# TencentARC/SEED-Story

Measured on AMD Instinct MI355X. Metric: story-steps/sec (text + 1024x1024 image), higher is better.
Workload: dtype bf16

## Files before the change

include/seedstory_hip.h:

```cpp
#ifndef SEEDSTORY_HIP_H_
#define SEEDSTORY_HIP_H_

#include <stddef.h>
#include <stdint.h>

#ifdef __cplusplus
extern "C" {
#endif

#define SS_ABI_VERSION 1

enum { SS_F32 = 0, SS_BF16 = 1, SS_F16 = 2 };
enum { SS_OK = 0, SS_EINVAL = -1, SS_EHIP = -2, SS_ENOMEM = -3, SS_ESTATE = -4 };

enum {
    SS_EPI_NONE = 0,
    SS_EPI_BIAS = 1,
    SS_EPI_GELU = 2,
    SS_EPI_RESIDUAL = 4,
    SS_EPI_SILU_MUL = 8,
    SS_EPI_GEGLU_PAIR = 16
};

const char* ss_last_error(void);
// ... 137 lines not shown
    const void *wqkv, *wo, *wgu, *wdown, *ln1, *ln2;
} ss_llama_layer_weights;

typedef struct ss_llama_weights {
    const void* embed;
    const void* lm_head;
    const void* final_norm;
    const void* rope_cos;
    const void* rope_sin;
    const ss_llama_layer_weights* layers;
} ss_llama_weights;

size_t ss_llama_workspace_bytes(const ss_llama_config* cfg, int64_t max_prefill_rows);
int ss_llama_create(const ss_llama_config* cfg, const ss_llama_weights* w, void* workspace,
                    size_t workspace_bytes, int64_t max_prefill_rows, const int32_t* host_img_ids,
                    ss_llama** out);
void ss_llama_destroy(ss_llama* h);

int ss_llama_select(ss_llama* h, int32_t seq);
int ss_llama_set_stop_id(ss_llama* h, int32_t token_id);

int ss_llama_set_attn_capture(ss_llama* h, void* maps, int64_t n_rows, int64_t ld, int64_t row0, int32_t head,
                              int32_t row_calls);

void* ss_llama_buffer(ss_llama* h, int which);

int ss_llama_set_lengths(ss_llama* h, int64_t kv_len, int64_t pos, void* stream);
int ss_llama_get_lengths(ss_llama* h, int64_t* kv_len, int64_t* pos);
int ss_llama_kv_gather(ss_llama* h, const int32_t* keep_idx_dev, int64_t n_keep, void* stream);

int ss_llama_prefill(ss_llama* h, const void* embeds, int64_t M, const int32_t* pos_ids, void* hidden_out,
                     void* stream);
int ss_llama_prefill_batch(ss_llama* h, const void* embeds, const int64_t* host_rows, void* hidden_out, void* stream);

int ss_llama_generate(ss_llama* h, int64_t n_steps, int32_t last_prompt_id, const int32_t* host_forced,
                      int64_t n_forced, int64_t* host_n_generated, void* stream);

int ss_llama_generate_batch(ss_llama* h, int64_t n_steps, const int32_t* last_prompt_ids,
                            const int32_t* host_forced, int64_t forced_ld, const int64_t* n_forced,
                            const int32_t* active, int64_t* host_n_generated, void* stream);

int ss_llama_profile_decode(ss_llama* h, int64_t n_tokens, float out_ms[8], double out_bytes[4],
                            void* stream);

typedef struct ss_resampler_weights {
    const void* q_in;
    const void* pos_kv;
    const void* kv_proj;
    const void *ln_kv_w, *ln_kv_b;
    const void *in_w, *in_b;
    const void *out_w, *out_b;
    int32_t nq, embed, n_heads, kv_dim, l_kv;
    float ln_eps;
} ss_resampler_weights;
size_t ss_resampler_workspace_bytes(const ss_resampler_weights* w, int64_t batch, int dtype);
int ss_resampler_forward(const ss_resampler_weights* w, const void* x, void* y, int64_t batch, void* workspace,
                         size_t workspace_bytes, int dtype, void* stream);

typedef struct ss_vit_layer_weights {
    const void *ln1_w, *ln1_b, *ln2_w, *ln2_b;
    const void *in_w, *in_b;
    const void *out_w, *out_b;
    const void *fc_w, *fc_b, *proj_w, *proj_b;
} ss_vit_layer_weights;
typedef struct ss_vit_weights {
    const void* conv_w;
    const void* pos;
    const void *ln_pre_w, *ln_pre_b;
    const ss_vit_layer_weights* layers;
    int32_t width, n_layers, n_heads, mlp_width, patch, image, kpad;
    float ln_eps;
} ss_vit_weights;
size_t ss_vit_workspace_bytes(const ss_vit_weights* w, int64_t batch, int dtype);
int ss_vit_forward(const ss_vit_weights* w, const void* img, void* out, int64_t batch, void* workspace,
                   size_t workspace_bytes, int dtype, void* stream);

int ss_vit_blocks(const ss_vit_weights* w, void* x, int64_t batch, int64_t tokens, int64_t layer0, int64_t n_layers,
                  void* workspace, size_t workspace_bytes, int dtype, void* stream);


int ss_conv3x3(const void* x, const void* w, void* y, int64_t batch, int64_t H, int64_t W, int64_t Cin,
               int64_t Cout, int64_t stride, int64_t upsample2x, const void* bias, const void* rowvec,
               int64_t rowvec_stride, const void* residual, int dtype, void* stream);

size_t ss_groupnorm_workspace_bytes(int64_t batch, int64_t hw, int64_t channels, int64_t groups, int dtype);
int ss_groupnorm(const void* x, const void* gamma, const void* beta, void* y, void* stats_ws, int64_t batch,
                 int64_t hw, int64_t channels, int64_t groups, float eps, int fuse_silu, int dtype, void* stream);

size_t ss_loss_workspace_bytes(int64_t n);
int ss_cross_entropy_rows(const void* logits, int64_t ld, const int64_t* labels, int64_t rows, int64_t vocab,
                          int64_t ignore_index, float* row_loss, float* row_valid, int dtype, void* stream);
int ss_cosine_rows(const void* rec, const void* target, int64_t rows, int64_t dim, float* row_val, int dtype, void* stream);
int ss_masked_mean(const float* vals, const float* mask, int64_t n, void* workspace, float* out2, void* stream);
int ss_mse(const void* a, const void* b, int64_t n, void* workspace, float* out2, int dtype, void* stream);

int ss_geglu(const void* in, void* out, int64_t rows, int64_t d, int dtype, void* stream);
int ss_unary(const void* x, void* y, int64_t n, int op, int dtype, void* stream);
int ss_softmax_rows(void* scores, int64_t rows, int64_t cols, float scale, int dtype, void* stream);
int ss_transpose(const void* in, void* out, int64_t rows, int64_t cols, int dtype, void* stream);
int ss_concat_channels(const void* a, const void* b, void* out, int64_t rows, int64_t c1, int64_t c2, int dtype,
                       void* stream);
int ss_layout_nchw_nhwc(const void* in, void* out, int64_t batch, int64_t channels, int64_t hw, int64_t cpad,
                        int to_nhwc, int dtype, void* stream);
int ss_euler_scale_dup(const void* x, void* xin, int64_t n, float sigma, int dtype, void* stream);
int ss_euler_cfg_step(void* x, const void* eps, int64_t n, float guidance, float sigma, float sigma_next,
                      int dtype, void* stream);
#define SS_FILTER_BILINEAR 0
#define SS_FILTER_BICUBIC 1
int ss_resample_ksize(int64_t in_size, int64_t out_size, int filter);
int ss_resample_coeffs(int64_t in_size, int64_t out_size, int filter, int32_t* coef, int32_t* bounds);
int ss_image_preprocess(const void* src_u8_hwc, int64_t H, int64_t W, void* dst_chw, void* dst_u8_hwc, int64_t OH, int64_t OW,
                        int64_t crop_top, int64_t crop_left, int64_t CH, int64_t CW, const int32_t* coef_h,
                        const int32_t* bounds_h, int ksize_h, const int32_t* coef_v, const int32_t* bounds_v, int ksize_v,
                        int64_t first_row, int64_t n_rows, void* tmp_u8, const float mean[3], const float std[3], int dtype,
                        void* stream);
int ss_image_to_u8(const void* in, void* out_u8, int64_t pixels, int64_t cpad, int dtype, void* stream);

int ss_debug_tr_probe(const void* src, void* dst, const void* lane_off, void* stream);

#ifdef __cplusplus
}
#endif
#endif
```

seed-story_amd/csrc/ss_diffusion.hip:

```cpp
#include "ss_common.h"

namespace ss {

__device__ __forceinline__ float silu_d(float g) { return g / (1.0f + expf(-g)); }
__device__ __forceinline__ float gelu_d(float v) { return 0.5f * v * (1.0f + erff(v * 0.70710678118654752440f)); }

__device__ __forceinline__ float silu_fast(float g) {
    return g * __builtin_amdgcn_rcpf(1.0f + __builtin_amdgcn_exp2f(-1.4426950408889634f * g));
}

template <typename T>
__global__ __launch_bounds__(256) void groupnorm_stats_kernel(const T* __restrict__ x, double* __restrict__ part,
                                                              int HW, int C, int G, int rows_per_block) {
    constexpr int V = Tr<T>::kVec;
    extern __shared__ __attribute__((aligned(16))) char smem_raw[];
    float* red = reinterpret_cast<float*>(smem_raw);
    float* chs = red + 256 * 2 * V;
    const int b = blockIdx.y;
    const int cg = C / G, ppr = C / V;
    const int r0 = blockIdx.x * rows_per_block;
    const int r1 = min(HW, r0 + rows_per_block);
    const T* xb = x + ((int64_t)b * HW) * C;
    for (int pc = 0; pc < ppr; pc += 256) {
        const int cw = min(256, ppr - pc);
// ... 9 lines not shown
            for (; r + 3 * rip < r1; r += 4 * rip) {
                uint4 u[4];
#pragma unroll
                for (int q = 0; q < 4; ++q) u[q] = ld16(xp + (int64_t)(r + q * rip) * C);
#pragma unroll
                for (int q = 0; q < 4; ++q) {
                    float f[V];
                    unpack<T>(u[q], f);
#pragma unroll
                    for (int j = 0; j < V; ++j) { s1[j] += f[j]; s2[j] = fmaf(f[j], f[j], s2[j]); }
                }
            }
            for (; r + rip < r1; r += 2 * rip) {
                float f[V], h[V];
                const uint4 u0 = ld16(xp + (int64_t)r * C), u1 = ld16(xp + (int64_t)(r + rip) * C);
                unpack<T>(u0, f);
                unpack<T>(u1, h);
#pragma unroll
                for (int j = 0; j < V; ++j) {
                    s1[j] += f[j]; s2[j] = fmaf(f[j], f[j], s2[j]);
                    s1[j] += h[j]; s2[j] = fmaf(h[j], h[j], s2[j]);
                }
            }
            if (r < r1) {
                float f[V];
                unpack<T>(ld16(xp + (int64_t)r * C), f);
#pragma unroll
                for (int j = 0; j < V; ++j) { s1[j] += f[j]; s2[j] = fmaf(f[j], f[j], s2[j]); }
            }
#pragma unroll
            for (int j = 0; j < V; ++j) { red[threadIdx.x * 2 * V + 2 * j] = s1[j]; red[threadIdx.x * 2 * V + 2 * j + 1] = s2[j]; }
        }
        __syncthreads();
        if (active && ry == 0) {
            for (int k = 1; k < rip; ++k) {
                const float* o = red + (k * cw + (int)threadIdx.x) * 2 * V;
#pragma unroll
                for (int j = 0; j < V; ++j) { s1[j] += o[2 * j]; s2[j] += o[2 * j + 1]; }
            }
#pragma unroll
            for (int j = 0; j < V; ++j) { chs[(p * V + j) * 2] = s1[j]; chs[(p * V + j) * 2 + 1] = s2[j]; }
        }
        __syncthreads();
    }
    double* out = part + (((int64_t)b * gridDim.x + blockIdx.x) * G) * 2;
    for (int g = threadIdx.x; g < G; g += 256) {
        double a1 = 0.0, a2 = 0.0;
        for (int c = g * cg; c < (g + 1) * cg; ++c) { a1 += (double)chs[2 * c]; a2 += (double)chs[2 * c + 1]; }
        out[2 * g] = a1;
        out[2 * g + 1] = a2;
    }
}

__global__ __launch_bounds__(256) void groupnorm_finalize_kernel(const double* __restrict__ part, double* __restrict__ stats,
                                                                 int nblk, int G) {
    __shared__ double sl[256 * 2];
    const int b = blockIdx.x;
    const int gw = G < 256 ? G : 256;
    const int ns = 256 / gw;
    for (int g0 = 0; g0 < G; g0 += gw) {
        const int g = g0 + (int)threadIdx.x % gw, sidx = (int)threadIdx.x / gw;
        double a1 = 0.0, a2 = 0.0;
        if (sidx < ns && g < G) {
            const int per = (nblk + ns - 1) / ns;
            const int k0 = sidx * per, k1 = min(nblk, k0 + per);
            const double2* pp = reinterpret_cast<const double2*>(part) + (int64_t)b * nblk * G + g;
            for (int kb = k0; kb < k1; kb += 8) {
                double2 t[8];
#pragma unroll
                for (int k = 0; k < 8; ++k) t[k] = (kb + k < k1) ? pp[(int64_t)(kb + k) * G] : make_double2(0.0, 0.0);
#pragma unroll
                for (int k = 0; k < 8; ++k) { a1 += t[k].x; a2 += t[k].y; }
            }
        }
        sl[threadIdx.x * 2] = a1;
        sl[threadIdx.x * 2 + 1] = a2;
        __syncthreads();
        if (sidx == 0 && g < G) {
            for (int k = 1; k < ns; ++k) { a1 += sl[(k * gw + (int)threadIdx.x) * 2]; a2 += sl[(k * gw + (int)threadIdx.x) * 2 + 1]; }
            stats[((int64_t)b * G + g) * 2] = a1;
            stats[((int64_t)b * G + g) * 2 + 1] = a2;
        }
        __syncthreads();
    }
}

template <typename T>
__global__ __launch_bounds__(256) void groupnorm_apply_kernel(const T* __restrict__ x, const double* __restrict__ stats,
                                                              const T* __restrict__ gamma, const T* __restrict__ beta,
                                                              T* __restrict__ y, int HW, int C, int G, float eps,
                                                              int silu, int rows_per_block) {
    constexpr int V = Tr<T>::kVec;
    const int b = blockIdx.y;
    const int cg = C / G, ppr = C / V;
    const int r0 = blockIdx.x * rows_per_block;
    const int r1 = min(HW, r0 + rows_per_block);
    const float inv_n = 1.0f / ((float)HW * (float)cg);
    const T* xb = x + ((int64_t)b * HW) * C;
    T* yb = y + ((int64_t)b * HW) * C;
    for (int pc = 0; pc < ppr; pc += 256) {
        const int cw = min(256, ppr - pc);
        const int rip = 256 / cw;
        const int ry = threadIdx.x / cw, p = pc + threadIdx.x % cw;
        if (ry >= rip) continue;
        float sc[V], sh[V], ga[V], be[V];
        unpack<T>(ld16(gamma + p * V), ga);
        unpack<T>(ld16(beta + p * V), be);
#pragma unroll
        for (int j = 0; j < V; ++j) {
            const int g = (p * V + j) / cg;
            const double md = stats[((int64_t)b * G + g) * 2] * (double)inv_n;
            const float mean = (float)md;
            const float var = (float)fmax(stats[((int64_t)b * G + g) * 2 + 1] * (double)inv_n - md * md, 0.0);
            const float rstd = 1.0f / sqrtf(var + eps);
            sc[j] = rstd * ga[j];
            sh[j] = be[j] - mean * sc[j];
        }
        const T* xp = xb + (int64_t)p * V;
        T* yp = yb + (int64_t)p * V;
        auto one = [&](const uint4& u, int r) {
            float f[V];
            unpack<T>(u, f);
#pragma unroll
            for (int j = 0; j < V; ++j) {
                float v = fmaf(f[j], sc[j], sh[j]);
                if (silu) v = silu_fast(Tr<T>::rnd(v));
                f[j] = v;
            }
            st16(yp + (int64_t)r * C, pack<T>(f));
        };
        int r = r0 + ry;
        for (; r + 3 * rip < r1; r += 4 * rip) {
            uint4 u[4];
#pragma unroll
            for (int q = 0; q < 4; ++q) u[q] = ld16(xp + (int64_t)(r + q * rip) * C);
#pragma unroll
            for (int q = 0; q < 4; ++q) one(u[q], r + q * rip);
        }
        for (; r + rip < r1; r += 2 * rip) {
            const uint4 u0 = ld16(xp + (int64_t)r * C), u1 = ld16(xp + (int64_t)(r + rip) * C);
            one(u0, r);
            one(u1, r + rip);
        }
        if (r < r1) one(ld16(xp + (int64_t)r * C), r);
    }
}

static int groupnorm_rows_per_block(int64_t B, int64_t HW, int64_t C, size_t elem) {
    int rows_per_block = (int)((128 * 1024) / (C * elem));
    if (rows_per_block < 16) rows_per_block = 16;
    while (rows_per_block > 16 && B * cdiv(HW, rows_per_block) < 2048) rows_per_block /= 2;
    if (rows_per_block > HW) rows_per_block = (int)HW;
    return rows_per_block;
}

size_t groupnorm_workspace_bytes(int64_t B, int64_t HW, int64_t C, int64_t G, int dtype) {
    if (B * HW == 0) return 0;
    const int rpb = groupnorm_rows_per_block(B, HW, C, dtype_size(dtype));
    return (size_t)B * G * 2 * sizeof(double) * (1 + (size_t)cdiv(HW, rpb));
}

template <typename T>
int groupnorm_launch(const void* x, const void* gamma, const void* beta, void* y, double* ws, int64_t B, int64_t HW,
                     int64_t C, int64_t G, float eps, int silu, hipStream_t s) {
    constexpr int V = Tr<T>::kVec;
    SS_REQUIRE(C % G == 0 && C % V == 0, "groupnorm: C=%lld G=%lld unsupported", (long long)C, (long long)G);
    if (B * HW == 0) return SS_OK;
    const int rows_per_block = groupnorm_rows_per_block(B, HW, C, sizeof(T));
    dim3 grid((unsigned)cdiv(HW, rows_per_block), (unsigned)B);
    double* stats = ws;
    double* part = ws + (size_t)B * G * 2;
    const size_t lds = (size_t)256 * 2 * V * sizeof(float) + (size_t)C * 2 * sizeof(float);
    SS_REQUIRE(lds <= 64 * 1024, "groupnorm: C=%lld too wide", (long long)C);
    hipLaunchKernelGGL(groupnorm_stats_kernel<T>, grid, dim3(256), lds, s, (const T*)x, part, (int)HW, (int)C, (int)G,
                       rows_per_block);
    SS_LAUNCH_CHECK("groupnorm_stats");
    hipLaunchKernelGGL(groupnorm_finalize_kernel, dim3((unsigned)B), dim3(256), 0, s, (const double*)part, stats, (int)grid.x, (int)G);
    SS_LAUNCH_CHECK("groupnorm_finalize");
    hipLaunchKernelGGL(groupnorm_apply_kernel<T>, grid, dim3(256), 0, s, (const T*)x, stats, (const T*)gamma,
                       (const T*)beta, (T*)y, (int)HW, (int)C, (int)G, eps, silu, rows_per_block);
    SS_LAUNCH_CHECK("groupnorm_apply");
    return SS_OK;
}

template <typename T>
__global__ __launch_bounds__(256) void geglu_kernel(const T* __restrict__ in, T* __restrict__ out, int64_t rows, int D) {
    constexpr int V = Tr<T>::kVec;
    const int ppr = D / V;
    const int64_t total = rows * ppr;
    for (int64_t i = blockIdx.x * (int64_t)blockDim.x + threadIdx.x; i < total; i += (int64_t)gridDim.x * blockDim.x) {
        const int64_t r = i / ppr;
        const int p = (int)(i % ppr);
        float a[V], g[V];
        unpack<T>(ld16(in + r * 2 * D + (int64_t)p * V), a);
        unpack<T>(ld16(in + r * 2 * D + D + (int64_t)p * V), g);
#pragma unroll
        for (int j = 0; j < V; ++j) a[j] = a[j] * Tr<T>::rnd(gelu_d(g[j]));
        st16(out + r * D + (int64_t)p * V, pack<T>(a));
    }
}

template <typename T>
__global__ __launch_bounds__(256) void softmax_rows_kernel(T* __restrict__ s, int cols, float scale) {
    constexpr int V = Tr<T>::kVec;
    __shared__ float red[16];
    T* row = s + (int64_t)blockIdx.x * cols;
    const int npack = cols / V;
    float mx = -1e30f;
    for (int p = threadIdx.x; p < npack; p += 256) {
        float f[V];
        unpack<T>(ld16(row + (int64_t)p * V), f);
#pragma unroll
        for (int j = 0; j < V; ++j) mx = fmaxf(mx, f[j] * scale);
    }
    mx = block_max(mx, red);
    float sum = 0.f;
    for (int p = threadIdx.x; p < npack; p += 256) {
        float f[V];
        unpack<T>(ld16(row + (int64_t)p * V), f);
#pragma unroll
        for (int j = 0; j < V; ++j) sum += expf(f[j] * scale - mx);
    }
    sum = block_sum(sum, red);
    const float inv = 1.0f / sum;
    for (int p = threadIdx.x; p < npack; p += 256) {
        float f[V];
        unpack<T>(ld16(row + (int64_t)p * V), f);
#pragma unroll
        for (int j = 0; j < V; ++j) f[j] = expf(f[j] * scale - mx) * inv;
        st16(row + (int64_t)p * V, pack<T>(f));
    }
}

template <typename T>
__global__ __launch_bounds__(256) void transpose_kernel(const T* __restrict__ in, T* __restrict__ out, int R, int Cc) {
    __shared__ T tile[32][33];
    const int c0 = blockIdx.x * 32, r0 = blockIdx.y * 32;
    const int tx = threadIdx.x & 31, ty = threadIdx.x >> 5;
    for (int j = ty; j < 32; j += 8)
        if (r0 + j < R && c0 + tx < Cc) tile[j][tx] = in[(int64_t)(r0 + j) * Cc + c0 + tx];
    __syncthreads();
    for (int j = ty; j < 32; j += 8)
        if (c0 + j < Cc && r0 + tx < R) out[(int64_t)(c0 + j) * R + r0 + tx] = tile[tx][j];
}

template <typename T>
__global__ __launch_bounds__(256) void concat_channels_kernel(const T* __restrict__ a, const T* __restrict__ b,
                                                              T* __restrict__ out, int64_t rows, int C1, int C2) {
    constexpr int V = Tr<T>::kVec;
    const int ppr = (C1 + C2) / V, p1 = C1 / V;
    const int64_t total = rows * ppr;
    for (int64_t i = blockIdx.x * (int64_t)blockDim.x + threadIdx.x; i < total; i += (int64_t)gridDim.x * blockDim.x) {
        const int64_t r = i / ppr;
        const int p = (int)(i % ppr);
        const uint4 v = p < p1 ? ld16(a + r * C1 + (int64_t)p * V) : ld16(b + r * C2 + (int64_t)(p - p1) * V);
        st16(out + r * (C1 + C2) + (int64_t)p * V, v);
    }
}

template <typename T>
__global__ void nchw_to_nhwc_kernel(const T* __restrict__ in, T* __restrict__ out, int64_t B, int C, int HW, int Cpad) {
    const int64_t total = B * HW * Cpad;
    for (int64_t i = blockIdx.x * (int64_t)blockDim.x + threadIdx.x; i < total; i += (int64_t)gridDim.x * blockDim.x) {
        const int c = (int)(i % Cpad);
        const int64_t r = i / Cpad;
        const int64_t b = r / HW, px = r % HW;
        T v;
// ... 64 lines not shown
    SS_LAUNCH_CHECK("geglu");
    return SS_OK;
}
template <typename T>
int unary_launch(const void* x, void* y, int64_t n, int op, hipStream_t s) {
    if (n == 0) return SS_OK;
    hipLaunchKernelGGL(unary_kernel<T>, dim3(egrid(n)), dim3(256), 0, s, (const T*)x, (T*)y, n, op);
    SS_LAUNCH_CHECK("unary");
    return SS_OK;
}
template <typename T>
int softmax_rows_launch(void* sc, int64_t rows, int64_t cols, float scale, hipStream_t s) {
    SS_REQUIRE(cols % Tr<T>::kVec == 0, "softmax_rows: cols %% %d != 0", Tr<T>::kVec);
    if (rows == 0) return SS_OK;
    hipLaunchKernelGGL(softmax_rows_kernel<T>, dim3((unsigned)rows), dim3(256), 0, s, (T*)sc, (int)cols, scale);
    SS_LAUNCH_CHECK("softmax_rows");
    return SS_OK;
}
template <typename T>
int transpose_launch(const void* in, void* out, int64_t R, int64_t Cc, hipStream_t s) {
    if (R * Cc == 0) return SS_OK;
    hipLaunchKernelGGL(transpose_kernel<T>, dim3((unsigned)cdiv(Cc, 32), (unsigned)cdiv(R, 32)), dim3(256), 0, s,
                       (const T*)in, (T*)out, (int)R, (int)Cc);
    SS_LAUNCH_CHECK("transpose");
    return SS_OK;
}
template <typename T>
int concat_channels_launch(const void* a, const void* b, void* out, int64_t rows, int64_t C1, int64_t C2, hipStream_t s) {
    SS_REQUIRE(C1 % Tr<T>::kVec == 0 && C2 % Tr<T>::kVec == 0, "concat_channels: channels %% %d != 0", Tr<T>::kVec);
    if (rows == 0) return SS_OK;
    hipLaunchKernelGGL(concat_channels_kernel<T>, dim3(egrid(rows * (C1 + C2) / Tr<T>::kVec)), dim3(256), 0, s,
                       (const T*)a, (const T*)b, (T*)out, rows, (int)C1, (int)C2);
    SS_LAUNCH_CHECK("concat_channels");
    return SS_OK;
}
template <typename T>
int layout_launch(const void* in, void* out, int64_t B, int64_t C, int64_t HW, int64_t Cpad, int to_nhwc, hipStream_t s) {
    if (B * HW == 0) return SS_OK;
    if (to_nhwc)
        hipLaunchKernelGGL(nchw_to_nhwc_kernel<T>, dim3(egrid(B * HW * Cpad)), dim3(256), 0, s, (const T*)in, (T*)out, B,
                           (int)C, (int)HW, (int)Cpad);
    else
        hipLaunchKernelGGL(nhwc_to_nchw_kernel<T>, dim3(egrid(B * C * HW)), dim3(256), 0, s, (const T*)in, (T*)out, B,
                           (int)C, (int)HW, (int)Cpad);
    SS_LAUNCH_CHECK("layout");
    return SS_OK;
}
template <typename T>
int euler_scale_dup_launch(const void* x, void* xin, int64_t n, float sigma, hipStream_t s) {
    hipLaunchKernelGGL(euler_scale_dup_kernel<T>, dim3(egrid(n)), dim3(256), 0, s, (const T*)x, (T*)xin, n,
                       1.0f / sqrtf(sigma * sigma + 1.0f));
    SS_LAUNCH_CHECK("euler_scale_dup");
    return SS_OK;
}
template <typename T>
int euler_cfg_step_launch(void* x, const void* eps, int64_t n, float guidance, float sigma, float sigma_next, hipStream_t s) {
    hipLaunchKernelGGL(euler_cfg_step_kernel<T>, dim3(egrid(n)), dim3(256), 0, s, (T*)x, (const T*)eps, n, guidance,
                       sigma_next - sigma);
    SS_LAUNCH_CHECK("euler_cfg_step");
    return SS_OK;
}
template <typename T>
int image_to_u8_launch(const void* in, void* out, int64_t pixels, int64_t Cpad, hipStream_t s) {
    hipLaunchKernelGGL(image_to_u8_kernel<T>, dim3(egrid(pixels * 3)), dim3(256), 0, s, (const T*)in, (uint8_t*)out, pixels,
                       (int)Cpad);
    SS_LAUNCH_CHECK("image_to_u8");
    return SS_OK;
}

}

using namespace ss;

extern "C" {

size_t ss_groupnorm_workspace_bytes(int64_t batch, int64_t hw, int64_t channels, int64_t groups, int dtype) {
    return ss::groupnorm_workspace_bytes(batch, hw, channels, groups, dtype);
}

int ss_groupnorm(const void* x, const void* gamma, const void* beta, void* y, void* stats_ws, int64_t batch, int64_t hw,
                 int64_t channels, int64_t groups, float eps, int fuse_silu, int dtype, void* stream) {
    return SS_DISPATCH(dtype, groupnorm_launch, x, gamma, beta, y, (double*)stats_ws, batch, hw, channels, groups, eps,
                       fuse_silu, (hipStream_t)stream);
}
int ss_geglu(const void* in, void* out, int64_t rows, int64_t d, int dtype, void* stream) {
    return SS_DISPATCH(dtype, geglu_launch, in, out, rows, d, (hipStream_t)stream);
}
int ss_unary(const void* x, void* y, int64_t n, int op, int dtype, void* stream) {
    return SS_DISPATCH(dtype, unary_launch, x, y, n, op, (hipStream_t)stream);
}
int ss_softmax_rows(void* scores, int64_t rows, int64_t cols, float scale, int dtype, void* stream) {
    return SS_DISPATCH(dtype, softmax_rows_launch, scores, rows, cols, scale, (hipStream_t)stream);
}
int ss_transpose(const void* in, void* out, int64_t rows, int64_t cols, int dtype, void* stream) {
    return SS_DISPATCH(dtype, transpose_launch, in, out, rows, cols, (hipStream_t)stream);
}
int ss_concat_channels(const void* a, const void* b, void* out, int64_t rows, int64_t c1, int64_t c2, int dtype,
                       void* stream) {
    return SS_DISPATCH(dtype, concat_channels_launch, a, b, out, rows, c1, c2, (hipStream_t)stream);
}
int ss_layout_nchw_nhwc(const void* in, void* out, int64_t batch, int64_t channels, int64_t hw, int64_t cpad,
                        int to_nhwc, int dtype, void* stream) {
    return SS_DISPATCH(dtype, layout_launch, in, out, batch, channels, hw, cpad, to_nhwc, (hipStream_t)stream);
}
int ss_euler_scale_dup(const void* x, void* xin, int64_t n, float sigma, int dtype, void* stream) {
    return SS_DISPATCH(dtype, euler_scale_dup_launch, x, xin, n, sigma, (hipStream_t)stream);
}
int ss_euler_cfg_step(void* x, const void* eps, int64_t n, float guidance, float sigma, float sigma_next, int dtype,
                      void* stream) {
    return SS_DISPATCH(dtype, euler_cfg_step_launch, x, eps, n, guidance, sigma, sigma_next, (hipStream_t)stream);
}
int ss_image_to_u8(const void* in, void* out_u8, int64_t pixels, int64_t cpad, int dtype, void* stream) {
    return SS_DISPATCH(dtype, image_to_u8_launch, in, out_u8, pixels, cpad, (hipStream_t)stream);
}

}

namespace ss {
typedef short v4s_t __attribute__((ext_vector_type(4)));
typedef __attribute__((address_space(3))) v4s_t lds_v4s_t;
__global__ void tr_probe_kernel(const uint16_t* src, uint16_t* dst, const int* lane_off) {
    __shared__ __attribute__((aligned(16))) uint16_t sm[4096];
    for (int i = threadIdx.x; i < 4096; i += 64) sm[i] = src[i];
    __syncthreads();
    const int off = lane_off[threadIdx.x];
    v4s_t r = __builtin_amdgcn_ds_read_tr16_b64_v4i16((lds_v4s_t*)(sm + off));
    for (int j = 0; j < 4; ++j) dst[threadIdx.x * 4 + j] = (uint16_t)r[j];
}
}
extern "C" int ss_debug_tr_probe(const void* src, void* dst, const void* lane_off, void* stream) {
    hipLaunchKernelGGL(ss::tr_probe_kernel, dim3(1), dim3(64), 0, (hipStream_t)stream, (const uint16_t*)src,
                       (uint16_t*)dst, (const int*)lane_off);
    SS_LAUNCH_CHECK("tr_probe");
    return SS_OK;
}
```

seed-story_amd/csrc/ss_gemm.hip:

```cpp
#include <stdio.h>

#include <map>
#include <mutex>

#include "ss_gemm_common.h"

namespace ss {

__device__ __attribute__((aligned(16))) unsigned int g_zero_page[64];

template <typename T, int BM, int BN, int WM, int WN, int KT, bool CONV, bool SPLIT = false>
__global__ __launch_bounds__(64 * WM * WN) void gemm_kernel(const GemmArgs g) {
    static_assert(!SPLIT || Tr<T>::kVec == 4, "SPLIT: fp32 operands");
    constexpr int V = Tr<T>::kVec;
    constexpr int NT = 64 * WM * WN;
    constexpr int PPR = 8 * KT;
    constexpr int BK = PPR * V;
    constexpr int LS = BK + V;
    constexpr int TM = BM / WM, TN = BN / WN;
    constexpr int FM = TM / 16, FN = TN / 16;
    constexpr int PA = (BM * PPR + NT - 1) / NT, PW = (BN * PPR + NT - 1) / NT;
    static_assert(TM % 16 == 0 && TN % 16 == 0, "wave tile must be MFMA-shaped");

    extern __shared__ __attribute__((aligned(16))) char smem_raw[];
// ... 587 lines not shown
                                                               float* __restrict__ part, int part_ld, int tn) {
    const int m = blockIdx.x * 4 + (threadIdx.x >> 6), lane = threadIdx.x & 63;
    if (m >= M) return;
    const T* row = C + (int64_t)m * ldc;
    double t1 = 0.0, t2 = 0.0;
    for (int n0 = 0, strip = 0; n0 < N; n0 += tn, ++strip) {
        float s1 = 0.f, s2 = 0.f;
        const int n1 = n0 + tn < N ? n0 + tn : N;
        for (int n = n0 + lane; n < n1; n += 64) {
            const float v = Tr<T>::ld(row + n);
            s1 += v;
            s2 = fmaf(v, v, s2);
        }
        s1 = wave_sum(s1);
        s2 = wave_sum(s2);
        if (part && lane == 0 && strip < part_ld) {
            part[((int64_t)m * part_ld + strip) * 2] = s1;
            part[((int64_t)m * part_ld + strip) * 2 + 1] = s2;
        }
        t1 += (double)s1;
        t2 += (double)s2;
    }
    if (stat && lane == 0) {
        stat[(int64_t)m * 2] += t1;
        stat[(int64_t)m * 2 + 1] += t2;
    }
}

template <typename T>
int gemm_launch(const void* A, const void* W, void* C, int64_t M, int64_t N, int64_t K, int64_t lda, int64_t ldw,
                int64_t ldc, const void* bias, const void* residual, int64_t ldr, int epi, hipStream_t s,
                double* rowstat_out = nullptr, float* rowpart = nullptr) {
    constexpr int V = Tr<T>::kVec;
    SS_REQUIRE(K % V == 0 && lda % V == 0 && ldw % V == 0, "gemm: K/lda/ldw must be multiples of %d (K=%lld)", V,
               (long long)K);
    SS_REQUIRE(!(epi & SS_EPI_SILU_MUL), "gemm: SILU_MUL is a GEMV epilogue (use ss_silu_mul)");
    SS_REQUIRE(!(epi & SS_EPI_GEGLU_PAIR) || (!(epi & (SS_EPI_GELU | SS_EPI_RESIDUAL)) && N % 2 == 0),
               "gemm: GEGLU_PAIR cannot be combined with GELU/RESIDUAL and needs an even N");
    SS_REQUIRE(!(epi & SS_EPI_BIAS) || bias, "gemm: bias epilogue without bias");
    SS_REQUIRE(!(epi & SS_EPI_RESIDUAL) || residual, "gemm: residual epilogue without residual");
    if (M == 0 || N == 0) return SS_OK;
    GemmArgs g = gemm_args(A, W, C, M, N, K, lda, ldw, ldc, epi, bias, residual, ldr);
    g.swz = knob(K_gemm_xcd_swizzle);
    if (knob(K_gemm_epi_generic)) g.epi |= SS_EPI_INTERNAL_GENERIC;
    if (rowstat_out || rowpart) {
        if constexpr (Tr<T>::kVec != 8) {
            set_error("ss_gemm_rowstat: 16-bit dtypes only");
            return SS_EINVAL;
        } else {
            SS_REQUIRE(K % 64 == 0 && N % 8 == 0 && M > 128, "ss_gemm_rowstat: needs K %% 64 == 0, N %% 8 == 0, M > 128 (M=%lld N=%lld K=%lld)",
                       (long long)M, (long long)N, (long long)K);
            g.rowstat_out = rowstat_out;
            int bn = 0, tn = 0;
            const int cfg = rowstat_cfg<T>(g, &bn, &tn);
            if (rowpart) {
                constexpr size_t A16 = 15;
                SS_REQUIRE(N % bn == 0 && (((size_t)C | (size_t)residual | (size_t)bias) & A16) == 0 && ((ldc | ldr) & 7) == 0,
                           "ss_gemm_rowpart: N %% %d != 0 or operands not 16-byte aligned (N=%lld)", bn, (long long)N);
                g.rowpart = rowpart;
                g.rowpart_ld = (int)(N / tn);
            }
            const bool force_fb = knob(K_gemm_rowstat_fallback) != 0;
            int rc = force_fb ? 1 : gemm_sp_dispatch<T>(cfg + 200, g, s);
            if (rc == 1 && !rowpart && !force_fb) rc = gemm_sp_dispatch<T>(265, g, s);
            if (rc == 1) {
                g.rowstat_out = nullptr;
                g.rowpart = nullptr;
                rc = gemm_dispatch_cfg<T>(lookup_cfg<T>(g), g, s);
                if (rc) return rc;
                hipLaunchKernelGGL(rowstat_fallback_kernel<T>, dim3((unsigned)((M + 3) / 4)), dim3(256), 0, s, (const T*)C, ldc, (int)M,
                                   (int)N, rowstat_out, rowpart, rowpart ? (int)(N / tn) : 0, tn > 0 ? tn : (int)N);
                SS_LAUNCH_CHECK("rowstat_fallback");
                return SS_OK;
            }
            return rc;
        }
    }
    return gemm_dispatch_cfg<T>(lookup_cfg<T>(g), g, s);
}

template <typename T>
int conv3x3_launch(const void* x, const void* w, void* y, int64_t B, int64_t H, int64_t Wd, int64_t Cin, int64_t Cout,
                   int64_t stride, int64_t up, const void* bias, const void* rowvec, int64_t rowvec_ld,
                   const void* residual, int epi, hipStream_t s) {
    constexpr int V = Tr<T>::kVec;
    SS_REQUIRE(Cin % V == 0, "conv3x3: Cin=%lld must be a multiple of %d (pad the channels)", (long long)Cin, V);
    SS_REQUIRE((stride == 1 || stride == 2) && !(up && stride != 1), "conv3x3: unsupported stride/upsample");
    GemmArgs g;
    conv_geometry(g, B, H, Wd, Cin, Cout, stride, up);
    g.A = x; g.W = w; g.C = y; g.bias = bias; g.residual = residual; g.epi = epi;
    g.rowvec = rowvec; g.rowvec_ld = rowvec_ld > 0 ? rowvec_ld : Cout;
    g.swz = knob(K_gemm_xcd_swizzle);
    if (g.M == 0) return SS_OK;
    return gemm_dispatch_cfg<T>(lookup_cfg<T>(g), g, s);
}

template <typename T>
int gemm_tune_launch(int64_t M, int64_t N, int64_t K, int epi, void* ws, size_t ws_bytes, hipStream_t s, float* us) {
    const GemmArgs g = gemm_args(nullptr, nullptr, nullptr, (M + 127) / 128 * 128, N, K, K, K, N, epi, nullptr, nullptr, N);
    return tune_shape<T>(g, ws, ws_bytes, (size_t)g.M * K, s, us);
}
template <typename T>
int conv_tune_launch(int64_t B, int64_t H, int64_t Wd, int64_t Cin, int64_t Cout, int64_t stride, int64_t up, void* ws,
                     size_t ws_bytes, hipStream_t s, float* us) {
    GemmArgs g;
    conv_geometry(g, B, H, Wd, Cin, Cout, stride, up);
    return tune_shape<T>(g, ws, ws_bytes, (size_t)B * H * Wd * Cin, s, us);
}

template <typename T>
int gemm_lnfold_launch(const void* A, const void* Wg, void* C, int64_t M, int64_t N, int64_t K, int64_t ldc, const float* rstd,
                       const float* shift, const float* colsum, const void* bias, int epi, hipStream_t s,
                       const float* ln_part = nullptr, int64_t ln_nstrip = 0, int64_t ln_width = 0, float ln_eps = 0.f) {
    if constexpr (Tr<T>::kVec != 8) {
        set_error("ss_gemm_lnfold: 16-bit dtypes only");
        return SS_EINVAL;
    } else {
        SS_REQUIRE(K % 64 == 0 && N % 16 == 0, "ss_gemm_lnfold: K %% 64 and N %% 16 must be 0 (K=%lld N=%lld)", (long long)K, (long long)N);
        SS_REQUIRE(!(epi & ~(SS_EPI_BIAS | SS_EPI_GELU | SS_EPI_GEGLU_PAIR)), "ss_gemm_lnfold: unsupported epilogue %d", epi);
        SS_REQUIRE(!(epi & SS_EPI_BIAS) || bias, "ss_gemm_lnfold: bias epilogue without bias");
        SS_REQUIRE(((rstd && shift) || (ln_part && ln_nstrip > 0 && ln_width > 0)) && colsum && (((size_t)colsum) & 15) == 0 &&
                   (((size_t)ln_part) & 7) == 0, "ss_gemm_lnfold: row statistics / column vector missing or misaligned");
        if (M == 0 || N == 0) return SS_OK;
        GemmArgs g = gemm_args(A, Wg, C, M, N, K, K, K, ldc, epi, bias);
        g.swz = knob(K_gemm_xcd_swizzle);
        g.scale_a = rstd; g.shift_a = shift; g.scale_w = colsum;
        g.ln_part = ln_part; g.ln_nstrip = (int)ln_nstrip; g.ln_inv_width = ln_width > 0 ? 1.0f / (float)ln_width : 0.f; g.ln_eps = ln_eps;
        int cfg = lookup_cfg<T>(g);
        if (cfg < 60 || cfg > 72) cfg = N % 160 == 0 ? (M >= 2048 ? 62 : 61) : (M * N >= 128 * 128 * 256 ? 65 : 70);
        if (const GemmTile t = sp_tile(cfg); t.WM * t.WN == 4 && !knob(K_lnfold_w4))
            cfg = (t.BN == 160 || N % 160 == 0) ? 62 : 66;
        const int rc = gemm_sp_dispatch<T>(cfg + 100, g, s);
        if (rc == 1) {
            set_error("ss_gemm_lnfold: no kernel for cfg %d / shape [%lld, %lld, %lld]", cfg + 100, (long long)M, (long long)N, (long long)K);
            return SS_EINVAL;
        }
        return rc;
    }
}

template <typename T>
__global__ __launch_bounds__(256) void rowstats_kernel(const T* __restrict__ x, int64_t ld, int rows, int cols, float eps,
                                                       float* __restrict__ rstd, float* __restrict__ shift) {
    constexpr int V = Tr<T>::kVec;
    constexpr int MAXP = 4;
    const int lane = threadIdx.x & 63;
    const int row = blockIdx.x * 4 + (threadIdx.x >> 6);
    if (row >= rows) return;
    const int npack = cols / V;
    const T* xr = x + (int64_t)row * ld;
    uint4 px[MAXP];
    float s1 = 0.f;
#pragma unroll
    for (int i = 0; i < MAXP; ++i) {
        const int p = lane + i * 64;
        if (p < npack) {
            px[i] = *reinterpret_cast<const uint4*>(xr + (int64_t)p * V);
            float f[V];
            unpack<T>(px[i], f);
#pragma unroll
            for (int j = 0; j < V; ++j) s1 += f[j];
        }
    }
    const float mean = wave_sum(s1) / (float)cols;
    float s2 = 0.f;
#pragma unroll
    for (int i = 0; i < MAXP; ++i) {
        const int p = lane + i * 64;
        if (p < npack) {
            float f[V];
            unpack<T>(px[i], f);
#pragma unroll
            for (int j = 0; j < V; ++j) { const float d = f[j] - mean; s2 = fmaf(d, d, s2); }
        }
    }
    const float r = 1.0f / sqrtf(wave_sum(s2) / (float)cols + eps);
    if (lane == 0) { rstd[row] = r; shift[row] = -mean * r; }
// ... 40 lines not shown
    }
    float v[4] = {a.x, a.y, a.z, a.w};
#pragma unroll
    for (int r = 0; r < 4; ++r) {
        if (bias) v[r] += Tr<T>::ld(bias + n + r);
        v[r] = Tr<T>::rnd(v[r]);
        if (res) v[r] += Tr<T>::ld(res + (int64_t)m * ldr + n + r);
        Tr<T>::st(C + (int64_t)m * ldc + n + r, v[r]);
    }
}

static void splitk_plan(int64_t M, int64_t N, int64_t K, int* cfg, int* S) {
    *cfg = 0; *S = 0;
    if (M <= 128 || M > 512 || N % 64 || K % 64 || K < 1024) return;
    const int mt = cdiv(M, 128);
    if (mt * cdiv(N, 128) >= 256) return;
    int c = 301, base = mt * cdiv(N, 64);
    int s = cdiv(2 * 256, base);
    const int kt = (int)(K / 64);
    if (s > kt / 8) s = kt / 8;
    if (s > 8) s = 8;
    if (s < 2) return;
    while (s > 2 && (s - 1) * cdiv(kt, s) >= kt) --s;
    *cfg = c; *S = s;
}

size_t gemm_splitk_workspace_bytes(int64_t M, int64_t N, int64_t K) {
    int cfg, S;
    splitk_plan(M, N, K, &cfg, &S);
    return S ? (size_t)S * M * N * sizeof(float) : 0;
}

template <typename T>
int gemm_splitk_launch(const void* A, const void* W, void* C, int64_t M, int64_t N, int64_t K, const void* bias,
                       const void* residual, void* ws, size_t ws_bytes, hipStream_t s) {
    int cfg = 0, S = 0;
    if constexpr (Tr<T>::kVec == 8) {
        if (knob(K_gemm_splitk)) splitk_plan(M, N, K, &cfg, &S);
    }
    const int force = knob(K_gemm_splitk_s);
    if (S && force >= 2 && force <= 8 && (size_t)force * M * N * sizeof(float) > ws_bytes) S = 0;
    if (!S || !ws || ws_bytes < (size_t)S * M * N * sizeof(float))
        return gemm_launch<T>(A, W, C, M, N, K, K, K, N, bias, residual, N, (bias ? SS_EPI_BIAS : 0) | (residual ? SS_EPI_RESIDUAL : 0), s);
    if constexpr (Tr<T>::kVec == 8) {
        GemmArgs g = gemm_args(A, W, ws, M, N, K, K, K, N, 0, nullptr, nullptr, N);
        g.swz = knob(K_gemm_splitk_swz);
        g.ksplit = S;
        if (force >= 2 && force <= 8 && force <= (int)(K / 64) / 2) g.ksplit = S = force;
        const int rc = gemm_sp_dispatch<T>(cfg, g, s);
        if (rc) {
            if (rc == 1) set_error("gemm_splitk: no kernel for cfg %d", cfg);
            return rc == 1 ? SS_EINVAL : rc;
        }
        const int64_t quads = M * N / 4;
        hipLaunchKernelGGL(splitk_reduce_kernel<T>, dim3((unsigned)((quads + 255) / 256)), dim3(256), 0, s, (const float*)ws, S, (int)M,
                           (int)N, (T*)C, N, (const T*)bias, (const T*)residual, N);
        SS_LAUNCH_CHECK("splitk_reduce");
    }
    return SS_OK;
}

int gemm_splitk_dev(const void* A, const void* W, void* C, int64_t M, int64_t N, int64_t K, const void* bias,
                    const void* residual, void* ws, size_t ws_bytes, int dtype, hipStream_t s) {
    return SS_DISPATCH(dtype, gemm_splitk_launch, A, W, C, M, N, K, bias, residual, ws, ws_bytes, s);
}

int gemm_dev(const void* A, const void* W, void* C, int64_t M, int64_t N, int64_t K, int64_t lda, int64_t ldw,
             int64_t ldc, const void* bias, const void* residual, int64_t ldr, int epi, int dtype, hipStream_t s) {
    return SS_DISPATCH(dtype, gemm_launch, A, W, C, M, N, K, lda, ldw, ldc, bias, residual, ldr, epi, s);
}

}

extern "C" {

int ss_conv3x3(const void* x, const void* w, void* y, int64_t batch, int64_t H, int64_t W_, int64_t Cin,
               int64_t Cout, int64_t stride, int64_t upsample2x, const void* bias, const void* rowvec,
               int64_t rowvec_stride, const void* residual, int dtype, void* stream) {
    const int epi = (bias ? SS_EPI_BIAS : 0) | (residual ? SS_EPI_RESIDUAL : 0);
    return SS_DISPATCH(dtype, ss::conv3x3_launch, x, w, y, batch, H, W_, Cin, Cout, stride, upsample2x, bias, rowvec,
                       rowvec_stride, residual, epi, (hipStream_t)stream);
}

int ss_gemm(const void* A, const void* W, void* C, int64_t M, int64_t N, int64_t K, int64_t lda,
            int64_t ldw, int64_t ldc, const void* bias, const void* residual, int64_t ldr, int epilogue,
            int dtype, void* stream) {
    return ss::gemm_dev(A, W, C, M, N, K, lda, ldw, ldc, bias, residual, ldr, epilogue, dtype, (hipStream_t)stream);
}

int ss_gemm_rowstat(const void* A, const void* W, void* C, int64_t M, int64_t N, int64_t K, int64_t lda, int64_t ldw,
                    int64_t ldc, const void* bias, const void* residual, int64_t ldr, int epilogue, double* rowstat_accum,
                    int dtype, void* stream) {
    SS_REQUIRE(rowstat_accum && (((size_t)rowstat_accum) & 15) == 0, "ss_gemm_rowstat: rowstat_accum missing or not 16-byte aligned");
    SS_REQUIRE(!(epilogue & SS_EPI_GEGLU_PAIR), "ss_gemm_rowstat: not defined for the GEGLU epilogue");
    return SS_DISPATCH(dtype, ss::gemm_launch, A, W, C, M, N, K, lda, ldw, ldc, bias, residual, ldr, epilogue,
                       (hipStream_t)stream, rowstat_accum);
}

size_t ss_gemm_splitk_workspace_bytes(int64_t M, int64_t N, int64_t K) { return ss::gemm_splitk_workspace_bytes(M, N, K); }

int ss_gemm_splitk(const void* A, const void* W, void* C, int64_t M, int64_t N, int64_t K, const void* bias, const void* residual,
                   void* workspace, size_t workspace_bytes, int dtype, void* stream) {
    SS_REQUIRE(A && W && C && M > 0 && N > 0 && K > 0, "ss_gemm_splitk: bad arguments");
    return ss::gemm_splitk_dev(A, W, C, M, N, K, bias, residual, workspace, workspace_bytes, dtype, (hipStream_t)stream);
}

int ss_rowstat_finalize(double* rowstat, int64_t M, int64_t width, float eps, float* rstd_out, float* shift_out, void* stream) {
    SS_REQUIRE(rowstat && rstd_out && shift_out && M > 0 && width > 0 && (((size_t)rowstat) & 15) == 0, "ss_rowstat_finalize: bad arguments");
    hipLaunchKernelGGL(ss::rowstat_finalize_kernel, dim3((unsigned)((M + 255) / 256)), dim3(256), 0, (hipStream_t)stream, rowstat,
                       (int)M, 1.0 / (double)width, eps, rstd_out, shift_out);
    SS_LAUNCH_CHECK("rowstat_finalize");
    return SS_OK;
}

int ss_rowstats(const void* x, int64_t ld, int64_t M, int64_t K, float eps, float* rstd_out, float* shift_out, int dtype, void* stream) {
    SS_REQUIRE(x && rstd_out && shift_out && M > 0 && K > 0 && ld >= K, "ss_rowstats: bad arguments");
    return SS_DISPATCH(dtype, ss::rowstats_launch, x, ld, M, K, eps, rstd_out, shift_out, (hipStream_t)stream);
}

int64_t ss_gemm_rowpart_strips(int64_t M, int64_t N, int64_t K, int dtype) {
    if (dtype != SS_BF16 && dtype != SS_F16) return 0;
    ss::GemmArgs g;
    g.M = (int)M; g.N = (int)N; g.K = (int)K;
    int bn = 0, tn = 0;
    if (dtype == SS_BF16) ss::rowstat_cfg<ss::bf16_t>(g, &bn, &tn); else ss::rowstat_cfg<ss::f16_t>(g, &bn, &tn);
    return (N % bn == 0) ? N / tn : 0;
}

int ss_gemm_rowpart(const void* A, const void* W, void* C, int64_t M, int64_t N, int64_t K, int64_t lda, int64_t ldw,
                    int64_t ldc, const void* bias, const void* residual, int64_t ldr, int epilogue, float* rowpart,
                    int dtype, void* stream) {
    SS_REQUIRE(rowpart && (((size_t)rowpart) & 7) == 0, "ss_gemm_rowpart: rowpart missing or not 8-byte aligned");
    SS_REQUIRE(!(epilogue & SS_EPI_GEGLU_PAIR), "ss_gemm_rowpart: not defined for the GEGLU epilogue");
    return SS_DISPATCH(dtype, ss::gemm_launch, A, W, C, M, N, K, lda, ldw, ldc, bias, residual, ldr, epilogue,
                       (hipStream_t)stream, nullptr, rowpart);
}

int ss_gemm_lnfold_part(const void* A, const void* Wg, void* C, int64_t M, int64_t N, int64_t K, int64_t ldc, const float* rowpart,
                        int64_t strips, int64_t width, float eps, const float* colsum, const void* bias, int epilogue, int dtype,
                        void* stream) {
    SS_REQUIRE(A && Wg && C && rowpart && strips > 0 && width > 0, "ss_gemm_lnfold_part: bad arguments");
    return SS_DISPATCH(dtype, ss::gemm_lnfold_launch, A, Wg, C, M, N, K, ldc, nullptr, nullptr, colsum, bias, epilogue, (hipStream_t)stream,
                       rowpart, strips, width, eps);
}

int ss_gemm_lnfold(const void* A, const void* Wg, void* C, int64_t M, int64_t N, int64_t K, int64_t ldc, const float* rstd,
                   const float* shift, const float* colsum, const void* bias, int epilogue, int dtype, void* stream) {
    SS_REQUIRE(A && Wg && C, "ss_gemm_lnfold: NULL argument");
    return SS_DISPATCH(dtype, ss::gemm_lnfold_launch, A, Wg, C, M, N, K, ldc, rstd, shift, colsum, bias, epilogue, (hipStream_t)stream);
}

size_t ss_gemm_tune_workspace_bytes(int64_t M, int64_t N, int64_t K, int dtype) {
    const size_t e = ss::dtype_size(dtype);
    const size_t Mk = (size_t)((M + 127) / 128 * 128);
    return (Mk * K + Mk * N) * e + ss::tune_rot_bytes((size_t)N * K * e) + 1024;
}

int ss_gemm_tune(int64_t M, int64_t N, int64_t K, int epilogue, int dtype, void* workspace, size_t workspace_bytes,
                 void* stream, float* best_us_host) {
    SS_REQUIRE(M > 0 && N > 0 && K > 0 && K % 8 == 0, "gemm_tune: bad shape");
    return SS_DISPATCH(dtype, ss::gemm_tune_launch, M, N, K, epilogue, workspace, workspace_bytes, (hipStream_t)stream,
                       best_us_host);
}

size_t ss_conv3x3_tune_workspace_bytes(int64_t batch, int64_t H, int64_t W_, int64_t Cin, int64_t Cout, int64_t stride,
                                       int64_t upsample2x, int dtype) {
// ... 63 lines not shown
```

seed-story_amd/csrc/ss_gemm_common.h:

```cpp
#pragma once
#include <type_traits>
#include <utility>

#include "ss_common.h"

namespace ss {

typedef __attribute__((ext_vector_type(4))) uint32_t u32x4_t;
typedef __attribute__((ext_vector_type(8))) uint32_t u32x8_t;
template <int NV> struct Frag { uint4 v[NV]; };
template <typename T> struct OutT { using type = T; };
template <> struct OutT<fp8_t> { using type = bf16_t; };
template <typename T> struct Mma;
template <> struct Mma<bf16_t> {
    static constexpr int kK = 32;
    static constexpr int kEB = 2;
    static constexpr int kNV = 1;
    static __device__ __forceinline__ f32x4_t run(const uint4& a, const uint4& b, f32x4_t c) {
        return __builtin_amdgcn_mfma_f32_16x16x32_bf16(__builtin_bit_cast(bf16x8_t, a),
                                                       __builtin_bit_cast(bf16x8_t, b), c, 0, 0, 0);
    }
    static __device__ __forceinline__ void run_inplace(const uint4& a, const uint4& b, f32x4_t& c) {
        asm volatile("v_mfma_f32_16x16x32_bf16 %0, %1, %2, %0"
                     : "+v"(c)
// ... 383 lines not shown
                    if constexpr (EM == 1) t *= sa * swv[i][r];
                    if constexpr (EM == 2) t = fmaf(t, sa, sh * swv[i][r]);
                    t += bv[i][r];
                    if (do_gelu) t = gelu_for<T>(Tr<T>::rnd(t));
                    v[r] = Tr<T>::rnd(t);
                    if (do_rowvec) v[r] = Tr<T>::rnd(v[r] + rv[i][r]);
                }
                if (geglu) {
                    const float o0 = v[0] * Tr<T>::rnd(gelu_for<T>(v[1])), o1 = v[2] * Tr<T>::rnd(gelu_for<T>(v[3]));
                    float pk[8] = {o0, o1, 0.f, 0.f, 0.f, 0.f, 0.f, 0.f};
                    *reinterpret_cast<uint32_t*>(rowp + (i * 8 + grp * 2) * 2) = pack<T>(pk).x;
                } else {
                    float pk[8] = {v[0], v[1], v[2], v[3], 0.f, 0.f, 0.f, 0.f};
                    const uint4 u = pack<T>(pk);
                    *reinterpret_cast<uint2*>(rowp + (i * 16 + grp * 4) * 2) = make_uint2(u.x, u.y);
                }
            }
        }
        auto readback = [&](auto lpr_tag) {
            constexpr int LPR = decltype(lpr_tag)::value;
            const int n_out0 = geglu ? (n_base >> 1) : n_base;
#pragma unroll
            for (int k = 0; k < (CR * LPR + 63) / 64; ++k) {
                const int idx = lane + k * 64;
                const int row = idx / LPR, c16 = idx - row * LPR;
                const int m = m_base + c * CR + row;
                if (idx < CR * LPR && m < M) {
                    uint4 u = *reinterpret_cast<const uint4*>(stg + row * RS + c16 * 16);
                    if (g.epi & SS_EPI_RESIDUAL) {
                        const uint4 rr = *reinterpret_cast<const uint4*>(res + (int64_t)m * g.ldr + n_base + c16 * 8);
                        float a[8], b[8];
                        unpack<T>(u, a);
                        unpack<T>(rr, b);
#pragma unroll
                        for (int e = 0; e < 8; ++e) a[e] += b[e];
                        u = pack<T>(a);
                    }
                    *reinterpret_cast<uint4*>(C + (int64_t)m * g.ldc + n_out0 + c16 * 8) = u;
                    if constexpr (RSTAT) {
                        if (g.rowstat_out || g.rowpart) {
                            float a[8];
                            unpack<T>(u, a);
                            float sv = 0.f, qv = 0.f;
#pragma unroll
                            for (int e = 0; e < 8; ++e) { sv += a[e]; qv = fmaf(a[e], a[e], qv); }
                            *reinterpret_cast<float2*>(stg + row * RS + c16 * 16) = make_float2(sv, qv);
                        }
                    }
                }
            }
            if constexpr (RSTAT) {
                if (g.rowstat_out || g.rowpart) {
                    const int m = m_base + c * CR + lane;
                    if (lane < CR && m < M) {
                        float sv = 0.f, qv = 0.f;
#pragma unroll
                        for (int q = 0; q < LPR; ++q) {
                            const float2 t = *reinterpret_cast<const float2*>(stg + lane * RS + q * 16);
                            sv += t.x; qv += t.y;
                        }
                        if (g.rowpart) {
                            *reinterpret_cast<float2*>(g.rowpart + ((int64_t)m * g.rowpart_ld + n_base / TN) * 2) = make_float2(sv, qv);
                        } else {
                            unsafeAtomicAdd(g.rowstat_out + 2 * (int64_t)m, (double)sv);
                            unsafeAtomicAdd(g.rowstat_out + 2 * (int64_t)m + 1, (double)qv);
                        }
                    }
                }
            }
        };
        if (geglu) readback(std::integral_constant<int, TN / 16>{});
        else readback(std::integral_constant<int, TN / 8>{});
    }
}

template <typename T> __device__ __forceinline__ uint32_t pack2(float a, float b) {
    if constexpr (std::is_same<T, bf16_t>::value) return f32x2_to_bf16x2_bits(a, b);
    else return f32_to_f16_bits(a) | (f32_to_f16_bits(b) << 16);
}
template <typename T> __device__ __forceinline__ void unpack2(uint32_t w, float& lo, float& hi) {
    if constexpr (std::is_same<T, bf16_t>::value) { lo = __uint_as_float(w << 16); hi = __uint_as_float(w & 0xffff0000u); }
    else { lo = f16_bits_to_f32(w & 0xffffu); hi = f16_bits_to_f32(w >> 16); }
}
template <typename T, int FM, int FN, int EV, bool RES, bool WHOLE>
__device__ __forceinline__ void gemm_epilogue_staged_pipe(const GemmArgs& g, f32x4_t (&acc)[FN][FM], int m_base, int n_base,
                                                          int lane, char* stg) {
    static_assert(Tr<T>::kVec == 8, "16-bit outputs only");
    static_assert(EV >= 1 && EV <= 4, "compile-time variants only");
    constexpr int TN = FN * 16, RS = TN * 2 + 16;
    constexpr bool GEGLU = EV == 4;
    constexpr int LPR = GEGLU ? TN / 16 : TN / 8;
    constexpr int NPC = 16 * LPR;
    constexpr int NP = (NPC + 63) / 64;
    const int l15 = lane & 15, grp = lane >> 4;
    const int M = g.M;
    constexpr bool has_res = RES;
    const T* bias = (const T*)g.bias;

    float bv[FN][4];
    {
        uint2 braw[FN];
        const bool hb = (g.epi & SS_EPI_BIAS) != 0;
#pragma unroll
        for (int i = 0; i < FN; ++i) braw[i] = hb ? *reinterpret_cast<const uint2*>(bias + n_base + i * 16 + grp * 4) : make_uint2(0u, 0u);
#pragma unroll
        for (int i = 0; i < FN; ++i) {
            float f[8];
            unpack<T>(make_uint4(braw[i].x, braw[i].y, 0u, 0u), f);
            bv[i][0] = f[0]; bv[i][1] = f[1]; bv[i][2] = f[2]; bv[i][3] = f[3];
        }
    }
    uint2 rvp[EV == 3 ? FN : 1];
    int rv_b = -1;
    auto load_rv = [&](int c) {
        if constexpr (EV == 3) {
            const int bidx = (m_base + c * 16) / g.rows_per_batch;
            if (bidx != rv_b) {
                rv_b = bidx;
                const T* rp = (const T*)g.rowvec + (int64_t)bidx * g.rowvec_ld + n_base + grp * 4;
#pragma unroll
                for (int i = 0; i < FN; ++i) rvp[i] = *reinterpret_cast<const uint2*>(rp + i * 16);
            }
        }
    };

    uint32_t loff[NP], goff[NP], roff[NP];
    bool pv[NP];
    int prow[NP];
#pragma unroll
    for (int k = 0; k < NP; ++k) {
        const int idx = lane + k * 64;
        const int row = idx / LPR, c16 = idx - row * LPR;
        pv[k] = (NPC % 64 == 0 || k + 1 < NP) ? true : idx < NPC;
        prow[k] = row;
        loff[k] = pv[k] ? (uint32_t)(row * RS + c16 * 16) : 0u;
        goff[k] = (uint32_t)row * (uint32_t)(g.ldc * 2) + (uint32_t)(c16 * 16);
        roff[k] = pv[k] ? (uint32_t)row * (uint32_t)(g.ldr * 2) + (uint32_t)(c16 * 16) : 0u;
    }
    const int n_out0 = GEGLU ? (n_base >> 1) : n_base;
    char* Cb = reinterpret_cast<char*>((T*)g.C + (int64_t)m_base * g.ldc + n_out0);
    const char* Rb = reinterpret_cast<const char*>((const T*)g.residual + (int64_t)m_base * g.ldr + n_base);
    const int64_t cstep = 32 * g.ldc, rstep = 32 * g.ldr;
    char* wrow = stg + l15 * RS + (GEGLU ? grp * 4 : grp * 8);

    auto stage = [&](int c) {
        load_rv(c);
#pragma unroll
        for (int i = 0; i < FN; ++i) {
            float t[4];
#pragma unroll
            for (int r = 0; r < 4; ++r) t[r] = acc[i][c][r] + bv[i][r];
            if constexpr (EV == 2) {
#pragma unroll
                for (int r = 0; r < 4; ++r) t[r] = gelu_for<T>(Tr<T>::rnd(t[r]));
            }
            if constexpr (EV == 3) {
                float rv[8];
                asm volatile("" : "+v"(rvp[i].x), "+v"(rvp[i].y));
                unpack<T>(make_uint4(rvp[i].x, rvp[i].y, 0u, 0u), rv);
#pragma unroll
                for (int r = 0; r < 4; ++r) t[r] = Tr<T>::rnd(t[r]) + rv[r];
            }
            if constexpr (GEGLU) {
                float v0, v1, v2, v3;
                unpack2<T>(pack2<T>(t[0], t[1]), v0, v1);
                unpack2<T>(pack2<T>(t[2], t[3]), v2, v3);
                const float o0 = v0 * Tr<T>::rnd(gelu_for<T>(v1)), o1 = v2 * Tr<T>::rnd(gelu_for<T>(v3));
                *reinterpret_cast<uint32_t*>(wrow + i * 16) = pack2<T>(o0, o1);
            } else {
                *reinterpret_cast<uint2*>(wrow + i * 32) = make_uint2(pack2<T>(t[0], t[1]), pack2<T>(t[2], t[3]));
            }
        }
    };
    uint4 u[NP];
    auto readback = [&]() {
#pragma unroll
        for (int k = 0; k < NP; ++k) u[k] = *reinterpret_cast<const uint4*>(stg + loff[k]);
    };

    constexpr int RD = 2;
    uint4 rr[FM][NP];
    auto row_ok = [&](int c, int k) { return pv[k] && (WHOLE || m_base + c * 16 + prow[k] < M); };
    auto load_res = [&](int c) {
        const gmem_char_t* Rc = uniform_gptr(Rb + c * rstep);
#pragma unroll
        for (int k = 0; k < NP; ++k) {
            if constexpr (WHOLE) rr[c][k] = gmem_ld16(Rc + roff[k]);
            else rr[c][k] = row_ok(c, k) ? gmem_ld16(Rc + roff[k]) : make_uint4(0u, 0u, 0u, 0u);
        }
    };
    load_rv(0);
    if (has_res) {
#pragma unroll
        for (int c = 0; c < RD && c < FM; ++c) load_res(c);
    }
    __builtin_amdgcn_sched_barrier(0);
    stage(0);
    __builtin_amdgcn_sched_barrier(0);
    readback();
#pragma unroll
    for (int c = 0; c < FM; ++c) {
        if (has_res && c + RD < FM) load_res(c + RD);
        __builtin_amdgcn_sched_barrier(0);
        if (c + 1 < FM) stage(c + 1);
        __builtin_amdgcn_sched_barrier(0);
        gmem_char_t* Cc = uniform_gptr(Cb + c * cstep);
#pragma unroll
        for (int k = 0; k < NP; ++k) {
            uint4 o = u[k];
            if (has_res) {
                float a[8], b[8];
                unpack<T>(o, a);
                unpack<T>(rr[c][k], b);
#pragma unroll
                for (int e = 0; e < 8; ++e) a[e] += b[e];
                o = pack<T>(a);
            }
            if (row_ok(c, k)) gmem_st16(Cc + goff[k], o);
        }
        __builtin_amdgcn_sched_barrier(0);
        if (c + 1 < FM) readback();
    }
}

#define SS_SP_TILES(X) \
    X(20, 128, 128, 2, 2, 1, 2,  0, 0) \
    X(21, 128,  64, 2, 2, 1, 2,  0, 0) \
    X(22,  64,  64, 2, 2, 1, 2,  0, 0) \
    X(23, 256, 128, 4, 2, 1, 2,  0, 0) \
    X(24, 256, 256, 2, 4, 2, 2,  0, 0)    \
    X(26, 128, 160, 2, 2, 1, 2,  0, 0)    \
    X(28, 128, 320, 2, 4, 1, 2,  0, 0)    \
    X(29,  64, 160, 2, 2, 1, 2,  0, 0)    \
    X(30, 256, 160, 4, 2, 1, 2,  0, 0)    \
    X(31, 256, 160, 4, 2, 1, 3,  0, 0)    \
    X(32, 256, 160, 4, 2, 1, 3,  1, 0)    \
    X(33, 256, 160, 4, 2, 1, 3,  3, 0)    \
    X(34, 256, 256, 2, 4, 2, 2,  1, 0)    \
    X(35, 256, 256, 2, 4, 2, 2,  2, 0)    \
    X(36, 256, 256, 2, 4, 2, 2,  3, 0)    \
    X(37, 128, 160, 2, 2, 1, 2,  1, 0)    \
    X(38, 256, 160, 4, 2, 1, 2,  2, 0)    \
    X(39, 128, 320, 2, 4, 1, 2,  2, 0)    \
    X(40, 256, 256, 2, 4, 2, 2,  6, 0)    \
    X(41, 128, 160, 2, 2, 1, 2,  4, 0)    \
    X(42, 256, 160, 4, 2, 1, 3,  4, 0)    \
    X(43, 256, 160, 4, 2, 1, 2,  6, 0)    \
    X(44, 128, 320, 2, 4, 1, 2,  4, 0)    \
    X(45, 256, 128, 4, 2, 1, 2,  4, 0)    \
    X(46, 128, 128, 2, 2, 1, 2,  4, 0)    \
    X(60, 256, 256, 2, 4, 2, 2, 11, 1)    \
    X(61, 128, 160, 2, 2, 1, 2,  8, 3)    \
    X(62, 256, 160, 4, 2, 1, 3, 12, 3)    \
    X(63, 128, 320, 2, 4, 1, 2,  8, 3)    \
    X(64, 256, 160, 4, 2, 1, 2, 10, 3)    \
    X(65, 128, 128, 2, 2, 1, 2,  8, 3)    \
    X(66, 256, 128, 4, 2, 1, 2,  8, 1)    \
    X(67,  64, 160, 2, 2, 1, 2,  8, 3)    \
    X(68, 128,  64, 2, 2, 1, 2,  8, 1)    \
    X(69, 256, 256, 2, 4, 2, 2,  8, 1)    \
    X(70,  64,  64, 2, 2, 1, 2,  8, 1)    \
    X(71, 256, 160, 4, 2, 1, 2,  8, 3)    \
    X(72, 128, 320, 2, 4, 1, 2, 10, 3)
#define SS_SP_SPLITK_TILES(X) \
    X(300, 128, 128, 2, 2, 1, 2, 64, 0) \
    X(301, 128,  64, 2, 2, 1, 2, 64, 0)
#define SS_SP_FP8_TILES(X) \
    X(80, 128, 128, 2, 2, 2, 2, 8, 0)     \
    X(81, 128, 160, 2, 2, 2, 2, 8, 0)     \
    X(82, 256, 160, 4, 2, 2, 2, 8, 0)     \
    X(85,  64, 160, 2, 2, 1, 2, 8, 0)     \
    X(86,  64,  64, 2, 2, 1, 2, 8, 0) \
    X(88, 128, 160, 2, 2, 2, 2, 0, 0)
#define SS_W4_FP8_TILES(X) \
    X(95, 256, 256, 2, 2, 16, 0, 2, 0)    \
    X(96, 256, 256, 2, 2, 16, 0, 0, 0)

struct GemmTile { int id, BM, BN, WM, WN, NH, NS, FLAGS, variants; };
#define SS_TILE_ROW(id, BM, BN, WM, WN, NH, NS, FLAGS, VAR) {id, BM, BN, WM, WN, NH, NS, FLAGS, VAR},
constexpr GemmTile kSpTiles[] = {SS_SP_TILES(SS_TILE_ROW)};
constexpr GemmTile kFp8Tiles[] = {SS_SP_FP8_TILES(SS_TILE_ROW) SS_W4_FP8_TILES(SS_TILE_ROW)};
template <int N> constexpr GemmTile find_tile(const GemmTile (&t)[N], int id) {
    for (int i = 0; i < N; ++i) if (t[i].id == id) return t[i];
    return GemmTile{};
}
constexpr GemmTile sp_tile(int id) { return find_tile(kSpTiles, id); }
constexpr GemmTile fp8_tile(int id) { return find_tile(kFp8Tiles, id); }

template <int N> constexpr bool tiles_well_formed(const GemmTile (&t)[N]) {
    for (int i = 0; i < N; ++i) {
        for (int j = 0; j < i; ++j) if (t[j].id == t[i].id) return false;
        if (t[i].id < 1 || t[i].id >= 100 || (t[i].variants && !(t[i].FLAGS & 8))) return false;
    }
    return true;
}
static_assert(tiles_well_formed(kSpTiles) && tiles_well_formed(kFp8Tiles),
              "tile lists: duplicate id, base id outside 1 .. 99, or a variant on a tile without the staged epilogue");

template <typename T> int gemm_sp_dispatch(int cfg, const GemmArgs& g, hipStream_t s);
template <typename T> int gemm_sp_dispatch_conv(int cfg, const GemmArgs& g, hipStream_t s);
template <typename T> int gemm_pp_dispatch(int cfg, const GemmArgs& g, hipStream_t s);
template <typename T> int gemm_pp_dispatch_conv(int cfg, const GemmArgs& g, hipStream_t s);
template <typename T> int gemm_w4_dispatch(int cfg, const GemmArgs& g, hipStream_t s);
template <typename T> int gemm_w4_dispatch_conv(int cfg, const GemmArgs& g, hipStream_t s);
int gemm_sp_dispatch_fp8(int cfg, const GemmArgs& g, hipStream_t s);
int gemm_w4_dispatch_fp8(int cfg, const GemmArgs& g, hipStream_t s);
template <typename T> static int gemm_sp_run(int cfg, const GemmArgs& g, hipStream_t s) {
    return g.conv_Cin > 0 ? gemm_sp_dispatch_conv<T>(cfg, g, s) : gemm_sp_dispatch<T>(cfg, g, s);
}
template <typename T> static int gemm_pp_run(int cfg, const GemmArgs& g, hipStream_t s) {
    return g.conv_Cin > 0 ? gemm_pp_dispatch_conv<T>(cfg, g, s) : gemm_pp_dispatch<T>(cfg, g, s);
}
template <typename T> static int gemm_w4_run(int cfg, const GemmArgs& g, hipStream_t s) {
    return g.conv_Cin > 0 ? gemm_w4_dispatch_conv<T>(cfg, g, s) : gemm_w4_dispatch<T>(cfg, g, s);
}

static inline int num_cus() {
    static int n = 0;
    if (!n) {
        int dev = 0;
        hipDeviceProp_t p;
        if (hipGetDevice(&dev) == hipSuccess && hipGetDeviceProperties(&p, dev) == hipSuccess) n = p.multiProcessorCount;
        if (n <= 0) n = 256;
    }
    return n;
}
template <auto KERN> static int launch_tiles(const char* name, const GemmArgs& g, int total, int cap, int threads, size_t lds, hipStream_t s) {
    const int grid = cap > 0 && total > cap ? cap : total;
    if (lds > 64 * 1024) SS_DYN_LDS(KERN, lds);
    hipLaunchKernelGGL(KERN, dim3((unsigned)grid, (unsigned)g.ksplit), dim3(threads), lds, s, g, total);
    SS_LAUNCH_CHECK(name);
    return SS_OK;
}

}
```

seed-story_amd/csrc/ss_gemm_pp.inc:

```

namespace ss {

template <int BN, int FLAGS>
struct PpLds {
    static constexpr int FN = BN / 64, FN0 = (FN + 1) / 2, FN1 = FN / 2, TN = FN * 16;
    static constexpr int HA = 128 * 128, HB0 = 4 * FN0 * 16 * 128, HB1 = 4 * FN1 * 16 * 128;
    static constexpr int BUF = 2 * HA + HB0 + HB1;
    static constexpr int STG_CR = 16, STG_WAVE = STG_CR * (TN * 2 + 16);
    static constexpr bool STG_IN_RING = 2 * BUF + 8 * STG_WAVE > 163840;
    static constexpr int BYTES = 2 * BUF + ((FLAGS & 8) != 0 && !STG_IN_RING ? 8 * STG_WAVE : 0);
};

static __device__ __attribute__((aligned(4096))) unsigned int g_pp_zero_page[1024];

__device__ __forceinline__ void dma16v(const char* gsrc, uint32_t lds_base) {
    asm volatile(
        "s_mov_b32 m0, %1\n\t"
        "s_nop 0\n\t"
        "global_load_lds_dwordx4 %0, off"
        :
        : "v"(gsrc), "s"(lds_base)
        : "memory");
}

template <typename T, int BN, int FLAGS, bool CONV>
__global__ __launch_bounds__(512) void gemm_pp_kernel(const GemmArgs g, const int total_tiles) {
    using Lds = PpLds<BN, FLAGS>;
    constexpr int BM = 256, FN = Lds::FN, FN0 = Lds::FN0, FN1 = Lds::FN1, TM = 128, TN = Lds::TN, FM = 8;
    static_assert(BN == 256 || BN == 320, "tile widths");
    constexpr bool EXACT = BN == 320 || CONV;
    constexpr bool PRIO = (FLAGS & 1) != 0, PERSIST = (FLAGS & 2) != 0, TWO = (FLAGS & 4) != 0, STAGED = (FLAGS & 8) != 0, RSTAT = (FLAGS & 32) != 0;
    constexpr int EM = ((FLAGS & 16) != 0) ? 2 : 0;
    constexpr int HA = Lds::HA, HB0 = Lds::HB0, HB1 = Lds::HB1, BUF = Lds::BUF;
    constexpr int OFF_A0 = 0, OFF_A1 = HA, OFF_B0 = 2 * HA, OFF_B1 = 2 * HA + HB0;
    constexpr int NP0 = FN0, NP1 = FN1;
    constexpr int FLY = NP0 + 2 + NP1;
    constexpr int STG_CR = Lds::STG_CR, STG_WAVE = Lds::STG_WAVE;
    constexpr bool STG_IN_RING = Lds::STG_IN_RING;
    static_assert(!(PERSIST && STG_IN_RING), "persistent tiles prefetch under the epilogue: the strips need their own LDS");
    static_assert(Mma<T>::kEB == 2, "16-bit operands");
    using TO = T;
    extern __shared__ __attribute__((aligned(16))) char smem_raw[];

    const int tid = threadIdx.x, lane = tid & 63;
    const int wid = __builtin_amdgcn_readfirstlane(tid >> 6);
    const int wm = wid >> 2, wn = wid & 3;
    const int l15 = lane & 15, grp = lane >> 4;
    const int M = g.M, N = g.N;
    const int MT = (M + BM - 1) / BM, NT = (N + BN - 1) / BN;
    const int ntiles = g.K / 64;
    const int tpt = CONV ? g.conv_Cin / 64 : 1;
    const uint32_t tpt_inv = CONV ? (65536u + (uint32_t)tpt - 1u) / (uint32_t)tpt : 0u;
    const int lw = CONV ? __builtin_ctz((unsigned)g.conv_W) : 0;
    const uint32_t lds0 = __builtin_amdgcn_readfirstlane((uint32_t)(size_t)(lds_void_t*)smem_raw);

    const int srow = lane >> 3;
    const int schunk = (lane & 7) ^ srow;
    auto b_col = [&](int h, int i) {
        const int RH = (h ? FN1 : FN0) * 16;
        const int r8 = (wid + 8 * i) * 8;
        return (r8 / RH) * TN + (h ? FN0 * 16 : 0) + r8 % RH + srow;
    };
    int m_blk = 0, n_blk = 0;
    uint32_t voffA[EXACT ? 1 : 2][EXACT ? 1 : 2], voffW[EXACT ? 1 : 2][EXACT ? 1 : 3];
    const char* sbaseA = nullptr;
    const char* sbaseW = nullptr;
    auto setup_tile = [&](int vid) {
        int mt_, nt_;
        xcd_tile_id(g.swz, MT, NT, vid, mt_, nt_);
        m_blk = mt_ * BM; n_blk = nt_ * BN;
        if constexpr (CONV) {
            voffA[0][0] = (uint32_t)(srow * g.conv_Cin * 2 + schunk * 16);
            voffW[0][0] = (uint32_t)((int64_t)srow * g.ldw * 2 + schunk * 16);
        } else if constexpr (EXACT) {
            voffA[0][0] = (uint32_t)((int64_t)srow * g.lda * 2 + schunk * 16);
            voffW[0][0] = (uint32_t)((int64_t)srow * g.ldw * 2 + schunk * 16);
        } else {
#pragma unroll
            for (int h = 0; h < 2; ++h) {
#pragma unroll
                for (int i = 0; i < 2; ++i) {
                    int m = m_blk + i * 128 + h * 64 + wid * 8 + srow;
                    m = m < M ? m : M - 1;
                    voffA[h][i] = (uint32_t)((int64_t)(m - m_blk) * g.lda * 2 + schunk * 16);
                }
#pragma unroll
                for (int i = 0; i < (h ? NP1 : NP0); ++i) {
                    int n = n_blk + b_col(h, i);
                    n = n < N ? n : N - 1;
                    voffW[h][i] = (uint32_t)((int64_t)(n - n_blk) * g.ldw * 2 + schunk * 16);
                }
            }
        }
        sbaseA = uniform_ptr((const char*)g.A + (CONV ? (int64_t)0 : (int64_t)m_blk * g.lda * 2));
        sbaseW = uniform_ptr((const char*)g.W + (int64_t)n_blk * g.ldw * 2);
    };
    struct Cur { const char* src; int dy, dx, c, tap; };
    auto cur_set_tap = [&](Cur& k) {
        const int t3 = (k.tap * 11) >> 5;
        k.dy = t3 - 1; k.dx = k.tap - 3 * t3 - 1;
        k.src = (const char*)g.A + ((int64_t)(k.dy * g.conv_W + k.dx) * g.conv_Cin + k.c * 64) * 2;
    };
    auto cur_make = [&](int t) {
        Cur k;
        k.tap = (int)(((uint32_t)t * tpt_inv) >> 16);
        k.c = t - k.tap * tpt;
        cur_set_tap(k);
        return k;
    };
    auto cur_next = [&](Cur& k) {
        k.c += 1; k.src += 128;
        if (k.c == tpt) { k.c = 0; k.tap += 1; cur_set_tap(k); }
    };
    auto stage_conv = [&](const Cur& k, int b, int h) {
        const uint32_t keep = m0_save();
// ... 156 lines not shown
            asm volatile("s_waitcnt lgkmcnt(0)" ::: "memory");
            pin();
            mma(1, H1);
            pin();
            bar();
            if (s2) { stage(t + 2, b, 3); wait_vmcnt<FLY>(); } else { wait_vmcnt<0>(); }
            bar();
            pin();
            mma(1, H0);
            pin();
            bar();
            if constexpr (CONV) { P1 = P2; cur_next(P2); }
        };
        auto tile2 = [&](int t, auto btag) {
            constexpr int b = decltype(btag)::value;
            const char* L = smem_raw + b * BUF;
            const bool s1 = t + 1 < ntiles, s2 = t + 2 < ntiles;
            read_w0(L + OFF_B0);
            read_w1(L + OFF_B1);
            read_a(L + OFF_A0);
            pin();
            if (s1) {
                stage(t + 1, b ^ 1, 3);
                if constexpr (CONV) stage_conv(P1, b ^ 1, 1); else stage(t + 1, b ^ 1, 1);
                wait_vmcnt<4 + NP0 + NP1>();
            } else {
                wait_vmcnt<0>();
            }
            asm volatile("s_waitcnt lgkmcnt(0)" ::: "memory");
            bar();
            pin();
            mma(0, H0);
            mma(0, H1);
            pin();
            bar();
            read_a(L + OFF_A1);
            pin();
            if (s2) {
                if constexpr (CONV) stage_conv(P2, b, 0); else stage(t + 2, b, 0);
                stage(t + 2, b, 2);
                wait_vmcnt<4 + NP0>();
            } else if (s1) {
                wait_vmcnt<2>();
            } else {
                wait_vmcnt<0>();
            }
            asm volatile("s_waitcnt lgkmcnt(0)" ::: "memory");
            bar();
            pin();
            mma(1, H1);
            mma(1, H0);
            pin();
            bar();
            if constexpr (CONV) { P1 = P2; cur_next(P2); }
        };
        int t = 0;
        for (; t + 1 < ntiles; t += 2) {
            if constexpr (TWO) { tile2(t, std::integral_constant<int, 0>{}); tile2(t + 1, std::integral_constant<int, 1>{}); }
            else { tile(t, std::integral_constant<int, 0>{}); tile(t + 1, std::integral_constant<int, 1>{}); }
        }
        if (t < ntiles) { if constexpr (TWO) tile2(t, std::integral_constant<int, 0>{}); else tile(t, std::integral_constant<int, 0>{}); }
        if (wm == 0) bar();

        if (has_next) {
            setup_tile(vnext);
            prologue();
        }
        asm volatile("s_nop 15\n\ts_nop 15" ::: "memory");
#pragma unroll
        for (int i = 0; i < FN; ++i)
#pragma unroll
            for (int j = 0; j < FM; ++j) asm volatile("" : "+v"(acc[i][j]));

        bool staged = false;
        if constexpr (STAGED) {
            constexpr size_t A16 = 15;
            staged = (n_cur + wn * TN + TN <= N) && (((size_t)g.C | (size_t)g.residual | (size_t)g.bias | (size_t)g.rowvec) & A16) == 0 &&
                     ((g.ldc | g.ldr | g.rowvec_ld) & 7) == 0 && (EM == 0 || ((size_t)g.scale_w & A16) == 0);
            if (staged) {
                char* strip = smem_raw + (STG_IN_RING ? 0 : 2 * BUF) + wid * STG_WAVE;
                const int mb = m_cur + wm * TM, nb = n_cur + wn * TN;
                const bool o_gelu = (g.epi & SS_EPI_GELU) != 0, o_geglu = (g.epi & SS_EPI_GEGLU_PAIR) != 0;
                const bool o_rv = g.rowvec != nullptr || (!CONV && (g.epi & SS_EPI_INTERNAL_GENERIC) != 0);
                if constexpr (EM == 0 && !RSTAT) {
                    const bool o_res = (g.epi & SS_EPI_RESIDUAL) != 0;
                    if (!o_gelu && !o_geglu && !o_rv && !o_res) gemm_epilogue_staged_pipe<TO, FM, FN, 1, false, EXACT>(g, acc, mb, nb, lane, strip);
                    else if (!o_gelu && !o_geglu && !o_rv) gemm_epilogue_staged_pipe<TO, FM, FN, 1, true, EXACT>(g, acc, mb, nb, lane, strip);
                    else if (CONV && !o_gelu && !o_geglu && !o_res && (g.rows_per_batch & 15) == 0) gemm_epilogue_staged_pipe<TO, FM, FN, 3, false, EXACT>(g, acc, mb, nb, lane, strip);
                    else if (!CONV && o_geglu && !o_gelu && !o_rv && !o_res) gemm_epilogue_staged_pipe<TO, FM, FN, 4, false, EXACT>(g, acc, mb, nb, lane, strip);
                    else if (!CONV && o_gelu && !o_geglu && !o_rv && !o_res) gemm_epilogue_staged_pipe<TO, FM, FN, 2, false, EXACT>(g, acc, mb, nb, lane, strip);
                    else gemm_epilogue_staged<TO, FM, FN, STG_CR, EM, RSTAT, 0>(g, acc, mb, nb, lane, strip);
                } else {
                if (!o_gelu && !o_geglu && !o_rv) gemm_epilogue_staged<TO, FM, FN, STG_CR, EM, RSTAT, 1>(g, acc, mb, nb, lane, strip);
                else if constexpr (CONV) gemm_epilogue_staged<TO, FM, FN, STG_CR, EM, RSTAT, 3>(g, acc, mb, nb, lane, strip);
                else if (o_geglu && !o_gelu && !o_rv) gemm_epilogue_staged<TO, FM, FN, STG_CR, EM, RSTAT, 4>(g, acc, mb, nb, lane, strip);
                else if (o_gelu && !o_geglu && !o_rv) gemm_epilogue_staged<TO, FM, FN, STG_CR, EM, RSTAT, 2>(g, acc, mb, nb, lane, strip);
                else gemm_epilogue_staged<TO, FM, FN, STG_CR, EM, RSTAT, 0>(g, acc, mb, nb, lane, strip);
                }
            }
        }
        if (!staged) gemm_epilogue<TO, FM, FN, EM, RSTAT>(g, acc, m_cur + wm * TM, n_cur + wn * TN, l15, grp);
        if (!has_next) break;
        vid = vnext;
        asm volatile("" : "+s"(vid));
        setup_tile(vid);
    }
}

template <typename T, int BN, int FLAGS>
static int pp_launch(const GemmArgs& g, hipStream_t s) {
    constexpr bool CONV = SS_PP_CONV != 0;
    const bool conv = g.conv_Cin > 0;
    if (conv != CONV || g.ksplit > 1) return 1;
    bool ok = (g.K % 64 == 0) && g.K >= 64 && (int64_t)BN * g.ldw * 2 < (1ll << 31);
    if (conv) {
        ok = ok && g.conv_stride == 1 && !g.conv_up && g.conv_Cin % 64 == 0 && g.conv_Cin <= 4096 && g.conv_W >= 8 &&
             (g.conv_W & (g.conv_W - 1)) == 0 && (g.conv_H & (g.conv_H - 1)) == 0 && g.M % 256 == 0 && g.N % BN == 0 &&
             (int64_t)g.M * g.conv_Cin * 2 < (1ll << 31);
    } else {
        ok = ok && (int64_t)256 * g.lda * 2 < (1ll << 31);
        if (BN == 320 && (g.M % 256 != 0 || g.N % 320 != 0)) ok = false;
    }
    if (!ok) return 1;
    if ((g.rowstat_out || g.rowpart) && !(FLAGS & 32)) return 1;
    return launch_tiles<gemm_pp_kernel<T, BN, FLAGS, CONV>>("gemm_pp", g, cdiv(g.M, 256) * cdiv(g.N, BN), (FLAGS & 2) ? num_cus() : 0, 512,
                                                            PpLds<BN, FLAGS>::BYTES, s);
}

#if SS_PP_CONV
template <typename T> int gemm_pp_dispatch_conv(int cfg, const GemmArgs& g, hipStream_t s) {
#else
template <typename T> int gemm_pp_dispatch(int cfg, const GemmArgs& g, hipStream_t s) {
#endif
    switch (cfg) {
        case 54: return pp_launch<T, 256, 8>(g, s);
        case 55: return pp_launch<T, 256, 10>(g, s);
        case 56: return pp_launch<T, 320, 8>(g, s);
        case 57: return pp_launch<T, 256, 12>(g, s);
#if !SS_PP_CONV
        case 58: return pp_launch<T, 320, 12>(g, s);
#endif
        default: return 1;
    }
}
#if SS_PP_CONV
template int gemm_pp_dispatch_conv<SS_PP_T>(int, const GemmArgs&, hipStream_t);
#else
template int gemm_pp_dispatch<SS_PP_T>(int, const GemmArgs&, hipStream_t);
#endif

}
```

seed-story_amd/seedstory/_lib.py:

```python
import ctypes as C
import os

_HERE = os.path.dirname(os.path.abspath(__file__))
LIB_PATH = os.environ.get("SEEDSTORY_HIP_LIB", os.path.join(os.path.dirname(_HERE), "lib", "libseedstory_hip.so"))

SS_F32, SS_BF16, SS_F16 = 0, 1, 2
SS_FILTER_BILINEAR, SS_FILTER_BICUBIC = 0, 1
EPI_NONE, EPI_BIAS, EPI_GELU, EPI_RESIDUAL, EPI_SILU_MUL, EPI_GEGLU_PAIR = 0, 1, 2, 4, 8, 16

vp, i64, i32, f32, sz = C.c_void_p, C.c_int64, C.c_int32, C.c_float, C.c_size_t
i32p = C.POINTER(C.c_int32)


class SSError(RuntimeError):
    pass


class LlamaConfig(C.Structure):
    _fields_ = [("hidden", i32), ("n_heads", i32), ("n_layers", i32), ("inter", i32), ("vocab", i32),
                ("max_pos", i32), ("rms_eps", f32), ("dtype", i32), ("cache_cap", i32), ("max_new", i32),
                ("n_img_ids", i32), ("eos_id", i32), ("n_seq", i32)]


class LlamaLayerWeights(C.Structure):
# ... 17 lines not shown


class VitWeights(C.Structure):
    _fields_ = [("conv_w", vp), ("pos", vp), ("ln_pre_w", vp), ("ln_pre_b", vp),
                ("layers", C.POINTER(VitLayerWeights)), ("width", i32), ("n_layers", i32), ("n_heads", i32),
                ("mlp_width", i32), ("patch", i32), ("image", i32), ("kpad", i32), ("ln_eps", f32)]


PROTOTYPES = {
    "ss_last_error": (C.c_char_p, []),
    "ss_abi_version": (C.c_int, []),
    "ss_device_info": (C.c_int, [i32p]),
    "ss_rowstats": (C.c_int, [vp, i64, i64, i64, f32, vp, vp, C.c_int, vp]),
    "ss_gemm_lnfold": (C.c_int, [vp, vp, vp, i64, i64, i64, i64, vp, vp, vp, vp, C.c_int, C.c_int, vp]),
    "ss_gemm_rowstat": (C.c_int, [vp, vp, vp, i64, i64, i64, i64, i64, i64, vp, vp, i64, C.c_int, vp, C.c_int, vp]),
    "ss_gemm_rowpart_strips": (i64, [i64, i64, i64, C.c_int]),
    "ss_gemm_rowpart": (C.c_int, [vp, vp, vp, i64, i64, i64, i64, i64, i64, vp, vp, i64, C.c_int, vp, C.c_int, vp]),
    "ss_gemm_lnfold_part": (C.c_int, [vp, vp, vp, i64, i64, i64, i64, vp, i64, i64, f32, vp, vp, C.c_int, C.c_int, vp]),
    "ss_rowstat_finalize": (C.c_int, [vp, i64, i64, f32, vp, vp, vp]),
    "ss_gemm_splitk_workspace_bytes": (C.c_size_t, [i64, i64, i64]),
    "ss_gemm_splitk": (C.c_int, [vp, vp, vp, i64, i64, i64, vp, vp, vp, C.c_size_t, C.c_int, vp]),
    "ss_quantize_rows_fp8": (C.c_int, [vp, i64, i64, i64, vp, vp, vp, vp, f32, C.c_int, vp]),
    "ss_gemm_fp8": (C.c_int, [vp, vp, vp, vp, vp, i64, i64, i64, i64, vp, vp, i64, C.c_int, vp]),
    "ss_create": (C.c_int, [C.c_int, C.POINTER(vp)]),
    "ss_context_info": (C.c_int, [vp, C.POINTER(i64)]),
    "ss_destroy": (None, [vp]),
    "ss_rccl_unique_id": (C.c_int, [vp]),
    "ss_rccl_init": (C.c_int, [vp, C.c_int, C.c_int, C.POINTER(vp)]),
    "ss_rccl_destroy": (None, [vp]),
    "ss_rccl_send": (C.c_int, [vp, vp, i64, C.c_int, C.c_int, vp]),
    "ss_rccl_recv": (C.c_int, [vp, vp, i64, C.c_int, C.c_int, vp]),
    "ss_rccl_bcast": (C.c_int, [vp, vp, i64, C.c_int, C.c_int, vp]),
    "ss_set_tuning": (C.c_int, [C.c_char_p, C.c_int]),
    "ss_get_tuning": (C.c_int, [C.c_char_p, C.c_int]),
    "ss_rmsnorm": (C.c_int, [vp, vp, vp, i64, i64, f32, C.c_int, vp]),
    "ss_layernorm": (C.c_int, [vp, vp, vp, vp, i64, i64, f32, C.c_int, vp]),
    "ss_add_bcast": (C.c_int, [vp, vp, vp, i64, i64, i64, i64, C.c_int, vp]),
    "ss_silu_mul": (C.c_int, [vp, vp, i64, i64, C.c_int, vp]),
    "ss_gather_rows": (C.c_int, [vp, vp, vp, i64, i64, C.c_int, vp]),
    "ss_scatter_rows": (C.c_int, [vp, vp, vp, i64, i64, C.c_int, vp]),
    "ss_im2col_patch": (C.c_int, [vp, vp, i64, i64, i64, i64, C.c_int, vp]),
    "ss_l2normalize_dim1": (C.c_int, [vp, vp, i64, i64, i64, C.c_int, vp]),
    "ss_rope_kv_append": (C.c_int, [vp, vp, vp, vp, vp, vp, vp, i64, i64, i64, i64, i64, i64, C.c_int, vp]),
    "ss_attention": (C.c_int, [vp, vp, vp, vp] + [i64] * 17 + [f32, C.c_int, C.c_int, vp]),
    "ss_attention_ragged": (C.c_int, [vp, vp, vp, vp] + [i64] * 3 + [vp] + [i64] * 13 + [f32, C.c_int, C.c_int, vp]),
    "ss_attn_decode_workspace_bytes": (sz, [i64, i64]),
    "ss_attn_decode": (C.c_int, [vp, vp, vp, vp, vp, vp, i64, i64, i64, C.c_int, vp]),
    "ss_attn_scores": (C.c_int, [vp, i64, vp, i64, vp, i64, i64, i64, i64, C.c_int, C.c_int, vp]),
    "ss_gemm": (C.c_int, [vp, vp, vp, i64, i64, i64, i64, i64, i64, vp, vp, i64, C.c_int, C.c_int, vp]),
    "ss_gemm_tune_workspace_bytes": (sz, [i64, i64, i64, C.c_int]),
    "ss_gemm_tune": (C.c_int, [i64, i64, i64, C.c_int, C.c_int, vp, sz, vp, C.POINTER(f32)]),
    "ss_conv3x3_tune_workspace_bytes": (sz, [i64, i64, i64, i64, i64, i64, i64, C.c_int]),
    "ss_conv3x3_tune": (C.c_int, [i64, i64, i64, i64, i64, i64, i64, C.c_int, vp, sz, vp, C.POINTER(f32)]),
    "ss_tune_lookup": (C.c_int, [i64, i64, i64, i64, i64, i64, i64, i64, C.c_int, i32p]),
    "ss_tune_export": (i64, [i32p, i64]),
    "ss_tune_import": (C.c_int, [i32p, i64]),
    "ss_tune_clear": (C.c_int, []),
    "ss_gemv": (C.c_int, [vp, vp, vp, i64, i64, vp, f32, vp, vp, C.c_int, C.c_int, vp]),
    "ss_gemv_batched": (C.c_int, [vp, vp, vp, i64, i64, i64, vp, f32, vp, vp, C.c_int, C.c_int, vp]),
    "ss_gemv_plan": (C.c_int, [i64, i64, i64, C.c_int, C.c_int, C.c_int, C.c_int, i32p, i64]),
    "ss_imgproc_argmax": (C.c_int, [vp, i64, vp, vp, i64, vp, C.c_int, vp]),
    "ss_llama_workspace_bytes": (sz, [C.POINTER(LlamaConfig), i64]),
    "ss_llama_create": (C.c_int, [C.POINTER(LlamaConfig), C.POINTER(LlamaWeights), vp, sz, i64, i32p,
                                  C.POINTER(vp)]),
    "ss_llama_destroy": (None, [vp]),
    "ss_llama_select": (C.c_int, [vp, i32]),
    "ss_llama_set_stop_id": (C.c_int, [vp, i32]),
    "ss_llama_set_attn_capture": (C.c_int, [vp, vp, i64, i64, i64, i32, i32]),
    "ss_llama_buffer": (vp, [vp, C.c_int]),
    "ss_llama_set_lengths": (C.c_int, [vp, i64, i64, vp]),
    "ss_llama_get_lengths": (C.c_int, [vp, C.POINTER(i64), C.POINTER(i64)]),
    "ss_llama_kv_gather": (C.c_int, [vp, vp, i64, vp]),
    "ss_llama_prefill": (C.c_int, [vp, vp, i64, vp, vp, vp]),
    "ss_llama_prefill_batch": (C.c_int, [vp, vp, C.POINTER(i64), vp, vp]),
    "ss_llama_generate": (C.c_int, [vp, i64, i32, i32p, i64, C.POINTER(i64), vp]),
    "ss_llama_generate_batch": (C.c_int, [vp, i64, i32p, i32p, i64, C.POINTER(i64), i32p, C.POINTER(i64), vp]),
    "ss_llama_profile_decode": (C.c_int, [vp, i64, C.POINTER(f32), C.POINTER(C.c_double), vp]),
    "ss_resampler_workspace_bytes": (sz, [C.POINTER(ResamplerWeights), i64, C.c_int]),
    "ss_resampler_forward": (C.c_int, [C.POINTER(ResamplerWeights), vp, vp, i64, vp, sz, C.c_int, vp]),
    "ss_vit_workspace_bytes": (sz, [C.POINTER(VitWeights), i64, C.c_int]),
    "ss_vit_forward": (C.c_int, [C.POINTER(VitWeights), vp, vp, i64, vp, sz, C.c_int, vp]),
    "ss_vit_blocks": (C.c_int, [C.POINTER(VitWeights), vp, i64, i64, i64, i64, vp, sz, C.c_int, vp]),
    "ss_conv3x3": (C.c_int, [vp, vp, vp, i64, i64, i64, i64, i64, i64, i64, vp, vp, i64, vp, C.c_int, vp]),
    "ss_loss_workspace_bytes": (C.c_size_t, [i64]),
    "ss_cross_entropy_rows": (C.c_int, [vp, i64, vp, i64, i64, i64, vp, vp, C.c_int, vp]),
    "ss_cosine_rows": (C.c_int, [vp, vp, i64, i64, vp, C.c_int, vp]),
    "ss_masked_mean": (C.c_int, [vp, vp, i64, vp, vp, vp]),
    "ss_mse": (C.c_int, [vp, vp, i64, vp, vp, C.c_int, vp]),
    "ss_groupnorm_workspace_bytes": (C.c_size_t, [i64, i64, i64, i64, C.c_int]),
    "ss_groupnorm": (C.c_int, [vp, vp, vp, vp, vp, i64, i64, i64, i64, f32, C.c_int, C.c_int, vp]),
    "ss_geglu": (C.c_int, [vp, vp, i64, i64, C.c_int, vp]),
    "ss_unary": (C.c_int, [vp, vp, i64, C.c_int, C.c_int, vp]),
    "ss_softmax_rows": (C.c_int, [vp, i64, i64, f32, C.c_int, vp]),
    "ss_transpose": (C.c_int, [vp, vp, i64, i64, C.c_int, vp]),
    "ss_concat_channels": (C.c_int, [vp, vp, vp, i64, i64, i64, C.c_int, vp]),
    "ss_layout_nchw_nhwc": (C.c_int, [vp, vp, i64, i64, i64, i64, C.c_int, C.c_int, vp]),
    "ss_euler_scale_dup": (C.c_int, [vp, vp, i64, f32, C.c_int, vp]),
    "ss_euler_cfg_step": (C.c_int, [vp, vp, i64, f32, f32, f32, C.c_int, vp]),
    "ss_resample_ksize": (C.c_int, [i64, i64, C.c_int]),
    "ss_resample_coeffs": (C.c_int, [i64, i64, C.c_int, i32p, i32p]),
    "ss_image_preprocess": (C.c_int, [vp, i64, i64, vp, vp, i64, i64, i64, i64, i64, i64, vp, vp, C.c_int, vp, vp, C.c_int,
                                      i64, i64, vp, C.POINTER(f32), C.POINTER(f32), C.c_int, vp]),
    "ss_image_to_u8": (C.c_int, [vp, vp, i64, i64, C.c_int, vp]),
    "ss_debug_tr_probe": (C.c_int, [vp, vp, vp, vp]),
}

_lib = None


def lib():
    global _lib
    if _lib is None:
        if not os.path.exists(LIB_PATH):
            raise SSError("libseedstory_hip.so not found at %s — build it first (seed-story_amd/csrc/Makefile); "
                          "there is no CPU fallback" % LIB_PATH)
        import torch
        l = C.CDLL(LIB_PATH)
        for name, (res, args) in PROTOTYPES.items():
            fn = getattr(l, name)
            fn.restype = res
            fn.argtypes = args
        if l.ss_abi_version() != 1:
            raise SSError("ABI version mismatch")
        _lib = l
        from . import tune
        tune.load_default_table()
    return _lib


def check(rc, what=""):
    if rc != 0:
        msg = lib().ss_last_error()
        raise SSError("%s failed (%d): %s" % (what or "seedstory call", rc, msg.decode() if msg else "?"))


_tuning_gen = 0


def set_tuning(key: str, value: int):
    global _tuning_gen
    check(lib().ss_set_tuning(key.encode(), int(value)), "ss_set_tuning")
    _tuning_gen += 1


def tuning_generation() -> int:
    return _tuning_gen


def get_tuning(key: str, default: int = 0) -> int:
    return int(lib().ss_get_tuning(key.encode(), int(default)))
```

seed-story_amd/seedstory/diffusion.py:

```python
import json
import math
import os

import numpy as np
import torch
from torch import nn

from . import _lib, ops

SDXL_BASE_UNET = dict(in_channels=4, out_channels=4, block_out_channels=(320, 640, 1280), layers_per_block=2,
                      transformer_layers=(0, 2, 10), num_heads=(5, 10, 20), cross_attention_dim=2048,
                      addition_time_embed_dim=256, pooled_dim=1280, norm_groups=32)
SDXL_BASE_VAE = dict(latent_channels=4, out_channels=3, block_out_channels=(128, 256, 512, 512), layers_per_block=2,
                     norm_groups=32, scaling_factor=0.13025)



def _unet_shapes(c):
    s = {}
    boc = c["block_out_channels"]
    temb = boc[0] * 4
    xdim = c["cross_attention_dim"]

    def lin(n, o, i, bias=True):
# ... 175 lines not shown
    def config(self):
        return self.cfg

    @classmethod
    def from_pretrained(cls, path, subfolder=None, torch_dtype=None, **kw):
        folder = os.path.join(path, subfolder) if subfolder else path
        with open(os.path.join(folder, "config.json")) as f:
            jc = json.load(f)
        tl = jc.get("transformer_layers_per_block", 1)
        boc = tuple(jc["block_out_channels"])
        types = jc.get("down_block_types", ())
        tl = tuple(tl) if isinstance(tl, (list, tuple)) else (tl,) * len(boc)
        tl = tuple(t if "CrossAttn" in types[i] else 0 for i, t in enumerate(tl)) if types else tl
        heads = jc.get("attention_head_dim", 8)
        heads = tuple(heads) if isinstance(heads, (list, tuple)) else (heads,) * len(boc)
        cfg = dict(in_channels=jc.get("in_channels", 4), out_channels=jc.get("out_channels", 4), block_out_channels=boc,
                   layers_per_block=jc.get("layers_per_block", 2), transformer_layers=tl, num_heads=heads,
                   cross_attention_dim=jc.get("cross_attention_dim", 2048),
                   addition_time_embed_dim=jc.get("addition_time_embed_dim", 256),
                   pooled_dim=jc.get("projection_class_embeddings_input_dim", 2816) - 6 * jc.get("addition_time_embed_dim", 256),
                   norm_groups=jc.get("norm_num_groups", 32))
        m = cls(cfg)
        from safetensors.torch import load_file
        sd = {}
        for fn in sorted(os.listdir(folder)):
            if fn.endswith(".safetensors") and "fp16" not in fn or fn == "diffusion_pytorch_model.fp16.safetensors" and not sd:
                sd.update(load_file(os.path.join(folder, fn)))
        from . import ckpt as _ckpt
        _ckpt.load_checked(m, sd, "unet:")
        return m.to(torch_dtype) if torch_dtype is not None else m

    def init_synthetic(self, seed=0):
        _init_synthetic(self, seed)
        self._prep = None
        return self

    def _prepare(self):
        sig = _sig(self)
        if self._prep is not None and self._prep_sig == sig:
            return self._prep
        sd = {k: v.data for k, v in self.named_parameters()}
        P = {}
        for k, v in sd.items():
            if v.dim() == 4 and v.shape[-1] == 3:
                cpad = 8 if v.shape[1] < 8 else None
                P[k] = _conv_w(v, cpad)
            elif v.dim() == 4:
                P[k] = v.reshape(v.shape[0], v.shape[1]).contiguous()
            else:
                P[k] = v
        for k in list(sd.keys()):
            if k.endswith("attn1.to_q.weight"):
                b = k[:-len("to_q.weight")]
                P[b + "qkv"] = torch.cat([sd[b + "to_q.weight"], sd[b + "to_k.weight"], sd[b + "to_v.weight"]], 0).contiguous()
            if k.endswith("ff.net.0.proj.weight"):
                b = k[:-len("weight")]
                w, bb = sd[k], sd[b + "bias"]
                d = w.shape[0] // 2
                P[b + "pairs.weight"] = torch.stack([w[:d], w[d:]], dim=1).reshape(2 * d, w.shape[1]).contiguous()
                P[b + "pairs.bias"] = torch.stack([bb[:d], bb[d:]], dim=1).reshape(2 * d).contiguous()
            if k.endswith("attn2.to_k.weight"):
                b = k[:-len("to_k.weight")]
                P[b + "kv"] = torch.cat([sd[b + "to_k.weight"], sd[b + "to_v.weight"]], 0).contiguous()
        names = [k[:-len(".time_emb_proj.weight")] for k in sd if k.endswith(".time_emb_proj.weight")]
        if names:
            P["temb_all.weight"] = torch.cat([sd[n + ".time_emb_proj.weight"] for n in names], 0).contiguous()
            P["temb_all.bias"] = torch.cat([sd[n + ".time_emb_proj.bias"] for n in names], 0).contiguous()
            off = 0
            P["temb_all.offsets"] = {}
            for n in names:
                P["temb_all.offsets"][n] = off
                off += sd[n + ".time_emb_proj.weight"].shape[0]
        if getattr(self, "_lnfold", False) and sd[next(iter(sd))].dtype in (torch.bfloat16, torch.float16):
            self._prepare_lnfold(P)
        if getattr(self, "_fp8", False):
            if sd[next(iter(sd))].dtype != torch.bfloat16:
                raise _lib.SSError("the fp8 UNet path produces bf16 activations: move the module to bf16 first")
            self._prepare_fp8(P)
        self._prep, self._prep_sig = P, sig
        self._prep_gen = getattr(self, "_prep_gen", 0) + 1
        return P

    def _resnet(self, P, n, x, B, H, W, temb_act, groups, eps=1e-5):
        h = ops.groupnorm(x, P[n + ".norm1.weight"], P[n + ".norm1.bias"], B, groups, eps, silu=True)
        tp, tld = None, 0
        if temb_act is not None:
            off = P["temb_all.offsets"][n]
            tld = temb_act.shape[1]
            tp = temb_act[:, off:]
        h, _, _ = ops.conv3x3(h, P[n + ".conv1.weight"], B, H, W, bias=P[n + ".conv1.bias"], rowvec=tp, rowvec_stride=tld)
        h = ops.groupnorm(h, P[n + ".norm2.weight"], P[n + ".norm2.bias"], B, groups, eps, silu=True)
        sc = x
        if (n + ".conv_shortcut.weight") in P:
            sc = ops.gemm(x, P[n + ".conv_shortcut.weight"], bias=P[n + ".conv_shortcut.bias"])
        h, _, _ = ops.conv3x3(h, P[n + ".conv2.weight"], B, H, W, bias=P[n + ".conv2.bias"], residual=sc)
        return h

    def enable_fp8(self, on=True):
        if bool(on) != getattr(self, "_fp8", False):
            self._fp8 = bool(on)
            self._prep = None
        return self

    def enable_lnfold(self, on=True):
        if bool(on) != getattr(self, "_lnfold", False):
            self._lnfold = bool(on)
            self._prep = None
        return self

    def _prepare_lnfold(self, P):
        for k in list(P.keys()):
            if not k.endswith(".norm1.weight") or ".transformer_blocks." not in k:
                continue
            b = k[:-len(".norm1.weight")]
            for norm, wkey, bkey in ((".norm1", ".attn1.qkv", None), (".norm2", ".attn2.to_q.weight", None),
                                     (".norm3", ".ff.net.0.proj.pairs.weight", ".ff.net.0.proj.pairs.bias")):
                W = P[b + wkey]
                if W.shape[1] % 64 or W.shape[0] % 16:
                    continue
                gamma, beta = P[b + norm + ".weight"].float(), P[b + norm + ".bias"].float()
                wg = (W.float() * gamma[None, :]).to(W.dtype).contiguous()
                c = wg.float().sum(dim=1).contiguous()
                d = W.float() @ beta
                if bkey is not None:
                    d = d + P[b + bkey].float()
                P[b + wkey + ".lnf"] = (wg, c, d.to(W.dtype).contiguous())

    def _prepare_fp8(self, P):
        for k in list(P.keys()):
            v = P[k]
            if not (isinstance(v, torch.Tensor) and v.dim() == 2 and ".attentions." in k):
                continue
            if k.endswith(("attn1.qkv", "pairs.weight", "to_out.0.weight", "attn2.to_q.weight", "ff.net.2.weight",
                           "proj_in.weight", "proj_out.weight")) and v.shape[1] % 128 == 0:
                P[k + ".fp8"] = ops.quantize_rows_fp8(v.contiguous())

    def _lin(self, P, name, x, *, ln=None, bias=None, residual=None, geglu=False, rowstat=None):
        f8 = P.get(name + ".fp8") if getattr(self, "_fp8", False) else None
        if f8 is None:
            if ln is not None:
                x = ops.layernorm(x, ln[0], ln[1], ln[2])
            if geglu:
                return ops.gemm_geglu(x, P[name], bias)
            part = None
            if rowstat is not None:
                M, K = x.shape
                N = P[name].shape[0]
                strips = ops.rowpart_strips(M, N, K, x.dtype)
                part = rowstat["buf"][:M * strips * 2].view(M, strips, 2)
                rowstat["cur"] = part
            return ops.gemm(x, P[name], bias=bias, residual=residual, rowpart=part)
        assert rowstat is None
        x8, sx = ops.quantize_rows_fp8(x, ln=ln)
        return ops.gemm_fp8(x8, sx, f8[0], f8[1], bias=bias, residual=residual, geglu=geglu)

    def _lnfold_on(self):
        return getattr(self, "_lnfold", False) and not getattr(self, "_fp8", False)

    def _lin_ln(self, P, name, x, ln, bias=None, geglu=False, rowstat=None):
        lnf = P.get(name + ".lnf") if self._lnfold_on() else None
        if lnf is None:
            assert rowstat is None
            return self._lin(P, name, x, ln=ln, bias=bias, geglu=geglu)
        if rowstat is not None:
            return ops.gemm_lnfold_part(x, lnf[0], rowstat["cur"], x.shape[1], ln[2], lnf[1], bias_d=lnf[2], geglu=geglu)
        rstd, shift = ops.rowstats(x, ln[2])
        return ops.gemm_lnfold(x, lnf[0], rstd, shift, lnf[1], bias_d=lnf[2], geglu=geglu)

    def _rs_new(self, rows, width, device):
        bufs = self.__dict__.setdefault("_rs_bufs", {})
        key = (rows, width, str(device))
        b = bufs.get(key)
        if b is None:
            b = bufs[key] = torch.empty(rows * ((width + 63) // 64) * 2, dtype=torch.float32, device=device)
            self._kv_gen = getattr(self, "_kv_gen", 0) + 1
        return {"buf": b, "cur": None}

    def _transformer(self, P, n, x, B, HW, ctx2d, Lctx, heads, layers, groups):
        h = ops.groupnorm(x, P[n + ".norm.weight"], P[n + ".norm.bias"], B, groups, 1e-6, silu=False)
        rs = None
        if self._lnfold_on() and h.shape[0] > 128 and all(
                (n + ".transformer_blocks.%d%s.lnf" % (k, w)) in P for k in range(layers)
                for w in (".attn1.qkv", ".attn2.to_q.weight", ".ff.net.0.proj.pairs.weight")):
            width = P[n + ".proj_in.weight"].shape[0]
            if all(ops.rowpart_strips(h.shape[0], width, kk, h.dtype) > 0 for kk in (h.shape[1], width, 4 * width)):
                rs = self._rs_new(h.shape[0], width, h.device)
        h = self._lin(P, n + ".proj_in.weight", h, bias=P[n + ".proj_in.bias"], rowstat=rs)
        for k in range(layers):
            b = n + ".transformer_blocks.%d" % k
            qkv = self._lin_ln(P, b + ".attn1.qkv", h, (P[b + ".norm1.weight"], P[b + ".norm1.bias"], 1e-5), rowstat=rs)
            a = ops.attention_qkv_packed(qkv, B, HW, heads)
            h = self._lin(P, b + ".attn1.to_out.0.weight", a, bias=P[b + ".attn1.to_out.0.bias"], residual=h, rowstat=rs)
            q = self._lin_ln(P, b + ".attn2.to_q.weight", h, (P[b + ".norm2.weight"], P[b + ".norm2.bias"], 1e-5), rowstat=rs)
            kv = self._ctx_kv.get(b)
            if kv is None:
                w = P[b + ".attn2.kv"]
                buf = self._ctx_kv_buf.get(b) if hasattr(self, "_ctx_kv_buf") else None
                if buf is None or buf.shape != (ctx2d.shape[0], w.shape[0]) or buf.dtype != ctx2d.dtype:
                    if not hasattr(self, "_ctx_kv_buf"):
                        self._ctx_kv_buf = {}
                    buf = self._ctx_kv_buf[b] = torch.empty(ctx2d.shape[0], w.shape[0], dtype=ctx2d.dtype, device=ctx2d.device)
                    self._kv_gen = getattr(self, "_kv_gen", 0) + 1
                kv = self._ctx_kv[b] = ops.gemm(ctx2d, w, out=buf)
            a = ops.attention_q_kvpacked(q, kv, B, HW, Lctx, heads)
            h = self._lin(P, b + ".attn2.to_out.0.weight", a, bias=P[b + ".attn2.to_out.0.bias"], residual=h, rowstat=rs)
            u = self._lin_ln(P, b + ".ff.net.0.proj.pairs.weight", h, (P[b + ".norm3.weight"], P[b + ".norm3.bias"], 1e-5),
                             bias=P[b + ".ff.net.0.proj.pairs.bias"], geglu=True, rowstat=rs)
            h = self._lin(P, b + ".ff.net.2.weight", u, bias=P[b + ".ff.net.2.bias"], residual=h,
                          rowstat=rs if k + 1 < layers else None)
        return self._lin(P, n + ".proj_out.weight", h, bias=P[n + ".proj_out.bias"], residual=x)

    @torch.no_grad()
    def forward(self, sample, timestep, encoder_hidden_states, added_cond_kwargs=None, return_dict=True, **kw):
        c = self.cfg
        P = self._prepare()
        dt, dev = sample.dtype, sample.device
        B, _, H, W = sample.shape
        boc, G, L = c["block_out_channels"], c["norm_groups"], c["layers_per_block"]
        temb = kw.get("temb_in")
        if temb is None:
            t = torch.as_tensor(timestep, dtype=torch.float32).reshape(-1).expand(B)
            temb = timestep_embedding(t, boc[0]).to(device=dev, dtype=dt)
        emb = ops.gemm(ops.silu(ops.gemm(temb, P["time_embedding.linear_1.weight"], bias=P["time_embedding.linear_1.bias"])),
                       P["time_embedding.linear_2.weight"], bias=P["time_embedding.linear_2.bias"])
        tids = added_cond_kwargs["time_ids"]
        tkey = (tuple(tids.flatten().tolist()), dt, str(dev)) if tids.device.type == "cpu" else None
        tid = self._tid_cache.get(tkey) if tkey is not None and hasattr(self, "_tid_cache") else None
        if tid is None:
            tid = timestep_embedding(tids.flatten().cpu(), c["addition_time_embed_dim"]).reshape(B, -1).to(device=dev, dtype=dt)
            if tkey is not None:
                self._tid_cache = {tkey: tid}
        add = torch.cat([added_cond_kwargs["text_embeds"].to(dt), tid], dim=-1).contiguous()
        emb = ops.gemm(ops.silu(ops.gemm(add, P["add_embedding.linear_1.weight"], bias=P["add_embedding.linear_1.bias"])),
                       P["add_embedding.linear_2.weight"], bias=P["add_embedding.linear_2.bias"], residual=emb)
        temb_act = ops.silu(emb)
        temb_act = ops.gemm(temb_act, P["temb_all.weight"], bias=P["temb_all.bias"])
        ctx = encoder_hidden_states.to(dt).contiguous()
        Lctx = ctx.shape[1]
        ctx2d = ctx.view(B * Lctx, -1)
        ckey = (encoder_hidden_states.data_ptr(), encoder_hidden_states._version, tuple(ctx.shape), dt, id(P))
        if getattr(self, "_ctx_key", None) != ckey:
            self._ctx_key, self._ctx_kv = ckey, {}

        x = ops.nchw_to_nhwc(sample.contiguous(), 8)
        h, _, _ = ops.conv3x3(x, P["conv_in.weight"], B, H, W, bias=P["conv_in.bias"])
        skips = [(h, H, W)]
        for i in range(len(boc)):
            for j in range(L):
                h = self._resnet(P, "down_blocks.%d.resnets.%d" % (i, j), h, B, H, W, temb_act, G)
                if c["transformer_layers"][i]:
                    h = self._transformer(P, "down_blocks.%d.attentions.%d" % (i, j), h, B, H * W, ctx2d, Lctx,
                                          c["num_heads"][i], c["transformer_layers"][i], G)
                skips.append((h, H, W))
            if i < len(boc) - 1:
                n = "down_blocks.%d.downsamplers.0.conv" % i
                h, H, W = ops.conv3x3(h, P[n + ".weight"], B, H, W, stride=2, bias=P[n + ".bias"])
                skips.append((h, H, W))
        h = self._resnet(P, "mid_block.resnets.0", h, B, H, W, temb_act, G)
        h = self._transformer(P, "mid_block.attentions.0", h, B, H * W, ctx2d, Lctx, c["num_heads"][-1],
                              c["transformer_layers"][-1], G)
        h = self._resnet(P, "mid_block.resnets.1", h, B, H, W, temb_act, G)
        for i in range(len(boc)):
            ri = len(boc) - 1 - i
            for j in range(L + 1):
                sk, _, _ = skips.pop()
                h = ops.concat_channels(h, sk)
                h = self._resnet(P, "up_blocks.%d.resnets.%d" % (i, j), h, B, H, W, temb_act, G)
                if c["transformer_layers"][ri]:
                    h = self._transformer(P, "up_blocks.%d.attentions.%d" % (i, j), h, B, H * W, ctx2d, Lctx,
                                          c["num_heads"][ri], c["transformer_layers"][ri], G)
            if i < len(boc) - 1:
                n = "up_blocks.%d.upsamplers.0.conv" % i
                h, H, W = ops.conv3x3(h, P[n + ".weight"], B, H, W, upsample=True, bias=P[n + ".bias"])
        h = ops.groupnorm(h, P["conv_norm_out.weight"], P["conv_norm_out.bias"], B, G, 1e-5, silu=True)
        o, _, _ = ops.conv3x3(h, P["conv_out.weight"], B, H, W, bias=P["conv_out.bias"])
        out = ops.nhwc_to_nchw(o, B, c["out_channels"], H, W)
        return _Sample(out) if return_dict else (out,)



class _VaeConfig:
    def __init__(self, scaling_factor, force_upcast=False):
        self.scaling_factor = scaling_factor
        self.force_upcast = force_upcast


class AutoencoderKL(nn.Module):

    def __init__(self, config=None):
        super().__init__()
        self.cfg = dict(SDXL_BASE_VAE if config is None else config)
        _grow(self, _vae_shapes(self.cfg))
        self.config = _VaeConfig(self.cfg["scaling_factor"], bool(self.cfg.get("force_upcast", True)))
        self._prep = None
        self._prep_sig = None

    @classmethod
    def from_pretrained(cls, path, subfolder=None, torch_dtype=None, **kw):
        folder = os.path.join(path, subfolder) if subfolder else path
        with open(os.path.join(folder, "config.json")) as f:
            jc = json.load(f)
        cfg = dict(latent_channels=jc.get("latent_channels", 4), out_channels=jc.get("out_channels", 3),
                   block_out_channels=tuple(jc["block_out_channels"]), layers_per_block=jc.get("layers_per_block", 2),
                   norm_groups=jc.get("norm_num_groups", 32), scaling_factor=jc.get("scaling_factor", 0.13025),
                   force_upcast=jc.get("force_upcast", True))
        m = cls(cfg)
        from safetensors.torch import load_file
        sd = {}
        for fn in sorted(os.listdir(folder)):
            if fn.endswith(".safetensors") and not sd:
                sd.update(load_file(os.path.join(folder, fn)))
        ren = {".query.": ".to_q.", ".key.": ".to_k.", ".value.": ".to_v.", ".proj_attn.": ".to_out.0."}
        sd = {_rename(k, ren): v for k, v in sd.items()}
        from . import ckpt as _ckpt
        _ckpt.load_checked(m, sd, "vae:", expect_unexpected=("encoder.", "quant_conv."))
        return m.to(torch_dtype) if torch_dtype is not None else m

    def init_synthetic(self, seed=0):
        _init_synthetic(self, seed)
        self._prep = None
        return self

    def decode_dtype(self):
        p0 = next(self.parameters()).dtype
        if _lib.get_tuning("vae_fp32", 0):
            return torch.float32
        if p0 == torch.float16 and self.config.force_upcast:
            return torch.bfloat16 if _lib.get_tuning("vae_bf16", 0) else torch.float32
        return p0

    def _prepare(self, run_dtype=None):
        run_dtype = self.decode_dtype() if run_dtype is None else run_dtype
        sig = _sig(self) + (run_dtype,)
        if self._prep is not None and self._prep_sig == sig:
            return self._prep
        P = {}
        for k, v in self.named_parameters():
            v = v.data.to(run_dtype)
            if v.dim() == 4 and v.shape[-1] == 3:
                P[k] = _conv_w(v, 8 if v.shape[1] < 8 else None)
            elif v.dim() == 4:
                P[k] = v.reshape(v.shape[0], v.shape[1]).contiguous()
            else:
                P[k] = v
        w = P["post_quant_conv.weight"]
        wp = torch.zeros(8, 8, dtype=w.dtype, device=w.device)
        wp[:w.shape[0], :w.shape[1]] = w
        bp = torch.zeros(8, dtype=w.dtype, device=w.device)
        bp[:w.shape[0]] = P["post_quant_conv.bias"]
        P["post_quant_conv.weight"], P["post_quant_conv.bias"] = wp, bp
        self._prep, self._prep_sig = P, sig
        return P

    def _resnet(self, P, n, x, B, H, W, G):
        h = ops.groupnorm(x, P[n + ".norm1.weight"], P[n + ".norm1.bias"], B, G, 1e-6, silu=True)
        h, _, _ = ops.conv3x3(h, P[n + ".conv1.weight"], B, H, W, bias=P[n + ".conv1.bias"])
        h = ops.groupnorm(h, P[n + ".norm2.weight"], P[n + ".norm2.bias"], B, G, 1e-6, silu=True)
# ... 209 lines not shown
```

seed-story_amd/seedstory/ops.py:

```python
import math

import torch

from . import _lib, tune
from ._lib import EPI_BIAS, EPI_GELU, EPI_NONE, EPI_RESIDUAL, EPI_SILU_MUL, check, lib

_DT = {torch.float32: _lib.SS_F32, torch.bfloat16: _lib.SS_BF16, torch.float16: _lib.SS_F16}


def dt(t):
    try:
        return _DT[t.dtype if isinstance(t, torch.Tensor) else t]
    except KeyError:
        raise _lib.SSError("unsupported dtype %s" % (t.dtype if isinstance(t, torch.Tensor) else t))


def stream():
    return torch.cuda.current_stream().cuda_stream


def p(t):
    return None if t is None else t.data_ptr()


# ... 76 lines not shown
def l2normalize_dim1(x):
    _req(x)
    B, L, Cc = x.shape
    y = torch.empty_like(x)
    check(lib().ss_l2normalize_dim1(p(x), p(y), B, L, Cc, dt(x), stream()), "ss_l2normalize_dim1")
    return y


def rope_kv_append(qkv, kcache, vcache, cos, sin, n_heads, kv_start, pos_ids=None, pos_start=0):
    _req(qkv); _req(kcache); _req(vcache)
    M = qkv.shape[0]
    E = qkv.shape[1] // 3
    hd = E // n_heads
    q = torch.empty(M, E, dtype=qkv.dtype, device=qkv.device)
    pid = None if pos_ids is None else pos_ids.to(device=qkv.device, dtype=torch.int32).contiguous()
    check(lib().ss_rope_kv_append(p(qkv), p(q), p(kcache), p(vcache), p(cos), p(sin), p(pid), pos_start, M, n_heads,
                                  hd, kv_start, kcache.shape[1], dt(qkv), stream()), "ss_rope_kv_append")
    return q


def attention(q, k, v, n_heads, scale=None, causal_br=False, out=None):
    _req(q); _req(k); _req(v)
    B, Lq, E = q.shape
    Lk = k.shape[1]
    hd = E // n_heads
    out = _out(out, q.shape, q, "attention")
    scale = 1.0 / math.sqrt(hd) if scale is None else scale
    kb = 0 if k.shape[0] == 1 and B > 1 else Lk * E
    check(lib().ss_attention(p(q), p(k), p(v), p(out), B, n_heads, Lq, Lk, hd, Lq * E, hd, E, kb, hd, E, kb, hd, E,
                             Lq * E, hd, E, scale, int(causal_br), dt(q), stream()), "ss_attention")
    return out


def attention_cache(q, kcache, vcache, kv_len, causal_br=True, out=None):
    _req(q); _req(kcache)
    M, E = q.shape
    n_heads, cap, hd = kcache.shape
    out = _out(out, q.shape, q, "attention_cache")
    check(lib().ss_attention(p(q), p(kcache), p(vcache), p(out), 1, n_heads, M, kv_len, hd, 0, hd, E, 0, cap * hd, hd,
                             0, cap * hd, hd, 0, hd, E, 1.0 / math.sqrt(hd), int(causal_br), dt(q), stream()),
          "ss_attention")
    return out


def attention_cache_slots(q, kcache, vcache, kv_lens, causal_br=True, out=None):
    import ctypes
    _req(q); _req(kcache)
    S, n_heads, cap, hd = kcache.shape
    E = n_heads * hd
    M = q.shape[0] // S
    out = _out(out, q.shape, q, "attention_cache_slots")
    lens = (ctypes.c_int32 * S)(*[int(x) for x in kv_lens])
    check(lib().ss_attention_ragged(p(q), p(kcache), p(vcache), p(out), S, n_heads, M, ctypes.cast(lens, ctypes.c_void_p), hd,
                                    M * E, hd, E, n_heads * cap * hd, cap * hd, hd, n_heads * cap * hd, cap * hd, hd, M * E, hd, E,
                                    1.0 / math.sqrt(hd), int(causal_br), dt(q), stream()), "ss_attention_ragged")
    return out


def attn_decode(q, kcache, vcache, kv_len_dev, out=None):
    _req(q); _req(kcache)
    n_heads, cap, hd = kcache.shape
    ws = torch.empty(lib().ss_attn_decode_workspace_bytes(n_heads, hd), dtype=torch.uint8, device=q.device)
    out = _out(out, q.shape, q, "attn_decode")
    check(lib().ss_attn_decode(p(q), p(kcache), p(vcache), p(out), p(ws), p(kv_len_dev), n_heads, hd, cap, dt(q),
                               stream()), "ss_attn_decode")
    return out


def attn_scores(q, k, out, row_calls=False):
    for t, name in ((q, "q"), (k, "k"), (out, "out")):
        if not t.is_cuda:
            raise _lib.SSError("%s must live on the GPU (there is no CPU path)" % name)
        if t.dim() != 2 or t.stride(1) != 1 or t.dtype != q.dtype:
            raise _lib.SSError("%s must be a 2-D view with unit inner stride, in q's dtype" % name)
    M, hd = q.shape
    kv = k.shape[0]
    if k.shape[1] != hd or out.shape[0] != M or out.shape[1] < kv:
        raise _lib.SSError("attn_scores: q %s, k %s, out %s do not fit" % (tuple(q.shape), tuple(k.shape), tuple(out.shape)))
    check(lib().ss_attn_scores(p(q), q.stride(0), p(k), k.stride(0), p(out), out.stride(0), M, kv, hd, 1 if row_calls else 0,
                               dt(q), stream()), "ss_attn_scores")
    return out


def gemm(a, w, bias=None, residual=None, gelu=False, out=None, rowstat=None, rowpart=None):
    _req(a); _req(w)
    M, K = a.shape
    N = w.shape[0]
    out = _out(out, (M, N), a, "gemm")
    epi = (EPI_BIAS if bias is not None else 0) | (EPI_GELU if gelu else 0) | (EPI_RESIDUAL if residual is not None else 0)
    tune.ensure_gemm(M, N, K, dt(a), epi, a.device)
    if rowstat is not None:
        assert rowstat.dtype == torch.float64 and rowstat.is_contiguous() and rowstat.numel() == 2 * M
        check(lib().ss_gemm_rowstat(p(a), p(w), p(out), M, N, K, K, w.stride(0), N, p(bias), p(residual), N, epi, p(rowstat),
                                    dt(a), stream()), "ss_gemm_rowstat")
        return out
    if rowpart is not None:
        assert rowpart.dtype == torch.float32 and rowpart.is_contiguous() and rowpart.shape[0] == M
        if rowpart.shape[1] != rowpart_strips(M, N, K, a.dtype):
            raise _lib.SSError("gemm(rowpart=): buffer has %d strips, this shape's tile writes %d"
                               % (rowpart.shape[1], rowpart_strips(M, N, K, a.dtype)))
        check(lib().ss_gemm_rowpart(p(a), p(w), p(out), M, N, K, K, w.stride(0), N, p(bias), p(residual), N, epi, p(rowpart),
                                    dt(a), stream()), "ss_gemm_rowpart")
        return out
    check(lib().ss_gemm(p(a), p(w), p(out), M, N, K, K, w.stride(0), N, p(bias), p(residual), N, epi, dt(a), stream()),
          "ss_gemm")
    return out


def gemm_splitk(a, w, bias=None, residual=None, out=None):
    _req(a); _req(w)
    M, K = a.shape
    N = w.shape[0]
    out = _out(out, (M, N), a, "gemm_splitk")
    nbytes = lib().ss_gemm_splitk_workspace_bytes(M, N, K)
    ws = torch.empty(max(nbytes, 16), dtype=torch.uint8, device=a.device)
    check(lib().ss_gemm_splitk(p(a), p(w), p(out), M, N, K, p(bias), p(residual), p(ws), nbytes, dt(a), stream()), "ss_gemm_splitk")
    return out


def gemm_geglu(a, w_pairs, bias_pairs, out=None):
    _req(a); _req(w_pairs)
    M, K = a.shape
    N = w_pairs.shape[0]
    out = _out(out, (M, N // 2), a, "gemm_geglu")
    tune.ensure_gemm(M, N, K, dt(a), _lib.EPI_GEGLU_PAIR, a.device)
    check(lib().ss_gemm(p(a), p(w_pairs), p(out), M, N, K, K, K, N // 2, p(bias_pairs), None, 0,
                        _lib.EPI_BIAS | _lib.EPI_GEGLU_PAIR, dt(a), stream()), "ss_gemm(geglu)")
    return out


def rowstats(x, eps):
    _req(x)
    M, K = x.shape
    st = torch.empty(2, M, dtype=torch.float32, device=x.device)
    check(lib().ss_rowstats(p(x), x.stride(0), M, K, float(eps), p(st[0]), p(st[1]), dt(x), stream()), "ss_rowstats")
    return st[0], st[1]


def gemm_lnfold(x, wg, rstd, shift, colsum, bias_d=None, gelu=False, geglu=False):
    _req(x); _req(wg)
    M, K = x.shape
    N = wg.shape[0]
    No = N // 2 if geglu else N
    out = torch.empty(M, No, dtype=x.dtype, device=x.device)
    epi = (EPI_BIAS if bias_d is not None else 0) | (EPI_GELU if gelu else 0) | (_lib.EPI_GEGLU_PAIR if geglu else 0)
    tune.ensure_gemm(M, N, K, dt(x), epi, x.device)
    check(lib().ss_gemm_lnfold(p(x), p(wg), p(out), M, N, K, No, p(rstd), p(shift), p(colsum), p(bias_d), epi, dt(x), stream()),
          "ss_gemm_lnfold")
    return out


def rowpart_strips(M, N, K, dtype):
    tune.ensure_gemm(M, N, K, dt(dtype), 0, None)
    return int(lib().ss_gemm_rowpart_strips(M, N, K, dt(dtype)))


def gemm_lnfold_part(x, wg, rowpart, width, eps, colsum, bias_d=None, gelu=False, geglu=False):
    _req(x); _req(wg); _req(rowpart)
    M, K = x.shape
    N = wg.shape[0]
    No = N // 2 if geglu else N
    out = torch.empty(M, No, dtype=x.dtype, device=x.device)
    epi = (EPI_BIAS if bias_d is not None else 0) | (EPI_GELU if gelu else 0) | (_lib.EPI_GEGLU_PAIR if geglu else 0)
    tune.ensure_gemm(M, N, K, dt(x), epi, x.device)
    check(lib().ss_gemm_lnfold_part(p(x), p(wg), p(out), M, N, K, No, p(rowpart), rowpart.shape[1], int(width), float(eps),
                                    p(colsum), p(bias_d), epi, dt(x), stream()), "ss_gemm_lnfold_part")
    return out


def rowstat_finalize(rowstat, width, eps, out=None):
    M = rowstat.shape[0]
    st = torch.empty(2, M, dtype=torch.float32, device=rowstat.device) if out is None else out
    check(lib().ss_rowstat_finalize(p(rowstat), M, int(width), float(eps), p(st[0]), p(st[1]), stream()), "ss_rowstat_finalize")
    return st[0], st[1]


def quantize_rows_fp8(x, ln=None):
    _req(x)
    M, K = x.shape
    q = torch.empty(M, K, dtype=torch.uint8, device=x.device)
    sc = torch.empty(M, dtype=torch.float32, device=x.device)
    g, b, eps = ln if ln is not None else (None, None, 0.0)
    check(lib().ss_quantize_rows_fp8(p(x), x.stride(0), M, K, p(q), p(sc), p(g), p(b), float(eps), dt(x), stream()),
          "ss_quantize_rows_fp8")
    return q, sc


def gemm_fp8(a8, sa, w8, sw, bias=None, residual=None, gelu=False, geglu=False, out=None):
    M, K = a8.shape
    N = w8.shape[0]
    No = N // 2 if geglu else N
    if out is None:
        out = torch.empty(M, No, dtype=torch.bfloat16, device=a8.device)
    epi = (EPI_BIAS if bias is not None else 0) | (EPI_GELU if gelu else 0) | (EPI_RESIDUAL if residual is not None else 0) | \
        (_lib.EPI_GEGLU_PAIR if geglu else 0)
    check(lib().ss_gemm_fp8(p(a8), p(sa), p(w8), p(sw), p(out), M, N, K, No, p(bias), p(residual), No, epi, stream()), "ss_gemm_fp8")
    return out


def gemv(w, x, norm_w=None, eps=0.0, bias=None, residual=None, silu_mul=False, out=None):
    _req(w); _req(x)
    N, K = w.shape
    if silu_mul:
        N //= 2
    y = _out(out, (N,), x, "gemv")
    epi = (EPI_BIAS if bias is not None else 0) | (EPI_RESIDUAL if residual is not None else 0) | \
          (EPI_SILU_MUL if silu_mul else 0)
    check(lib().ss_gemv(p(w), p(x), p(y), N, K, p(norm_w), eps, p(bias), p(residual), epi, dt(x), stream()), "ss_gemv")
    return y


def gemv_batched(w, x, norm_w=None, eps=0.0, bias=None, residual=None, silu_mul=False, out=None):
    _req(w); _req(x)
    N, K = w.shape
    if silu_mul:
        N //= 2
    nb = x.shape[0]
    y = _out(out, (nb, N), x, "gemv_batched")
    epi = (EPI_BIAS if bias is not None else 0) | (EPI_RESIDUAL if residual is not None else 0) | \
          (EPI_SILU_MUL if silu_mul else 0)
    check(lib().ss_gemv_batched(p(w), p(x), p(y), N, K, nb, p(norm_w), eps, p(bias), p(residual), epi, dt(x),
                                stream()), "ss_gemv_batched")
    return y


def imgproc_argmax(logits, last_id, img_ids):
    _req(logits)
    dev = logits.device
    last = torch.tensor([last_id], dtype=torch.int32, device=dev)
    ids = torch.as_tensor(list(img_ids), dtype=torch.int32, device=dev)
    tok = torch.zeros(1, dtype=torch.int32, device=dev)
    check(lib().ss_imgproc_argmax(p(logits), logits.numel(), p(last), p(ids), ids.numel(), p(tok), dt(logits),
                                  stream()), "ss_imgproc_argmax")
    return tok


def conv3x3(x, w, B, H, W, stride=1, upsample=False, bias=None, rowvec=None, residual=None, rowvec_stride=0, out=None):
    _req(x); _req(w)
    Cin = x.shape[-1]
    Cout = w.shape[0]
    Hin, Win = (2 * H, 2 * W) if upsample else (H, W)
    Ho, Wo = (Hin + 2 - 3) // stride + 1, (Win + 2 - 3) // stride + 1
    y = _out(out, (B * Ho * Wo, Cout), x, "conv3x3")
    tune.ensure_conv(B, H, W, Cin, Cout, stride, upsample, dt(x), x.device)
    check(lib().ss_conv3x3(p(x), p(w), p(y), B, H, W, Cin, Cout, stride, int(upsample), p(bias), p(rowvec),
                           rowvec_stride, p(residual), dt(x), stream()), "ss_conv3x3")
    return y, Ho, Wo


def groupnorm(x, gamma, beta, B, groups, eps, silu=False):
    _req(x)
    C = x.shape[-1]
    HW = x.shape[0] // B
    y = torch.empty_like(x)
    nb = int(lib().ss_groupnorm_workspace_bytes(B, HW, C, groups, dt(x)))
    ws = torch.empty(max(nb // 8, 1), dtype=torch.float64, device=x.device)
    check(lib().ss_groupnorm(p(x), p(gamma), p(beta), p(y), p(ws), B, HW, C, groups, eps, int(silu), dt(x), stream()),
          "ss_groupnorm")
    return y


def _mean2(vals, mask):
    n = vals.numel()
    ws = torch.empty(max(int(lib().ss_loss_workspace_bytes(n)) // 8, 1), dtype=torch.float64, device=vals.device)
    out = torch.empty(2, dtype=torch.float32, device=vals.device)
    check(lib().ss_masked_mean(p(vals), p(mask) if mask is not None else None, n, p(ws), p(out), stream()), "ss_masked_mean")
    return out


def cross_entropy(logits, labels, ignore_index=-100):
    _req(logits)
    R, V = logits.shape
    labels = labels.to(device=logits.device, dtype=torch.int64).contiguous()
    assert labels.numel() == R and logits.stride(1) == 1
    row = torch.empty(R, dtype=torch.float32, device=logits.device)
    valid = torch.empty(R, dtype=torch.float32, device=logits.device)
    check(lib().ss_cross_entropy_rows(p(logits), logits.stride(0), p(labels), R, V, ignore_index, p(row), p(valid), dt(logits),
                                      stream()), "ss_cross_entropy_rows")
    out = _mean2(row, valid)
    return out[0], out[1]


def cosine_loss(rec, target):
    _req(rec)
    _req(target)
    assert rec.shape == target.shape and rec.dtype == target.dtype
    dim = rec.shape[-1]
    r2, t2 = rec.reshape(-1, dim).contiguous(), target.reshape(-1, dim).contiguous()
    val = torch.empty(r2.shape[0], dtype=torch.float32, device=rec.device)
    check(lib().ss_cosine_rows(p(r2), p(t2), r2.shape[0], dim, p(val), dt(rec), stream()), "ss_cosine_rows")
    return _mean2(val, None)[0]


def mse_loss(a, b):
    _req(a)
    _req(b)
    assert a.shape == b.shape and a.dtype == b.dtype
    a2, b2 = a.contiguous(), b.contiguous()
    n = a2.numel()
    ws = torch.empty(max(int(lib().ss_loss_workspace_bytes(n)) // 8, 1), dtype=torch.float64, device=a.device)
    out = torch.empty(2, dtype=torch.float32, device=a.device)
    check(lib().ss_mse(p(a2), p(b2), n, p(ws), p(out), dt(a), stream()), "ss_mse")
    return out[0]


def geglu(x):
    _req(x)
    rows, two_d = x.shape
    out = torch.empty(rows, two_d // 2, dtype=x.dtype, device=x.device)
    check(lib().ss_geglu(p(x), p(out), rows, two_d // 2, dt(x), stream()), "ss_geglu")
    return out


def silu(x):
    _req(x)
    y = torch.empty_like(x)
    check(lib().ss_unary(p(x), p(y), x.numel(), 0, dt(x), stream()), "ss_unary")
    return y


def attention_qkv_packed(qkv, B, L, n_heads, out=None):
    _req(qkv)
    E = qkv.shape[1] // 3
    hd = E // n_heads
    out = _out(out, (B * L, E), qkv, "attention_qkv_packed")
    esz = qkv.element_size()
    base = qkv.data_ptr()
    check(lib().ss_attention(base, base + E * esz, base + 2 * E * esz, p(out), B, n_heads, L, L, hd, L * 3 * E, hd, 3 * E,
                             L * 3 * E, hd, 3 * E, L * 3 * E, hd, 3 * E, L * E, hd, E, 1.0 / math.sqrt(hd), 0, dt(qkv),
                             stream()), "ss_attention")
    return out


def attention_q_kvpacked(q, kv, B, Lq, Lk, n_heads, out=None):
    _req(q); _req(kv)
    E = q.shape[1]
    hd = E // n_heads
    out = _out(out, q.shape, q, "attention_q_kvpacked")
    esz = q.element_size()
    kb = kv.data_ptr()
    check(lib().ss_attention(p(q), kb, kb + E * esz, p(out), B, n_heads, Lq, Lk, hd, Lq * E, hd, E, Lk * 2 * E, hd, 2 * E,
                             Lk * 2 * E, hd, 2 * E, Lq * E, hd, E, 1.0 / math.sqrt(hd), 0, dt(q), stream()), "ss_attention")
    return out


def softmax_rows_(s, scale):
    _req(s)
    check(lib().ss_softmax_rows(p(s), s.shape[0], s.shape[1], scale, dt(s), stream()), "ss_softmax_rows")
    return s


def transpose(x):
    _req(x)
    R, Cc = x.shape
    out = torch.empty(Cc, R, dtype=x.dtype, device=x.device)
    check(lib().ss_transpose(p(x), p(out), R, Cc, dt(x), stream()), "ss_transpose")
    return out


def concat_channels(a, b):
    _req(a); _req(b)
    rows = a.shape[0]
    out = torch.empty(rows, a.shape[1] + b.shape[1], dtype=a.dtype, device=a.device)
    check(lib().ss_concat_channels(p(a), p(b), p(out), rows, a.shape[1], b.shape[1], dt(a), stream()),
          "ss_concat_channels")
    return out


def nchw_to_nhwc(x, cpad):
    _req(x)
    B, Cc = x.shape[0], x.shape[1]
    HW = x[0, 0].numel()
    out = torch.empty(B * HW, cpad, dtype=x.dtype, device=x.device)
    check(lib().ss_layout_nchw_nhwc(p(x), p(out), B, Cc, HW, cpad, 1, dt(x), stream()), "ss_layout_nchw_nhwc")
    return out


def nhwc_to_nchw(x, B, C, H, W):
    _req(x)
    out = torch.empty(B, C, H, W, dtype=x.dtype, device=x.device)
    check(lib().ss_layout_nchw_nhwc(p(x), p(out), B, C, H * W, x.shape[-1], 0, dt(x), stream()), "ss_layout_nchw_nhwc")
    return out


def euler_scale_dup(x, sigma):
    _req(x)
    xin = torch.empty((2,) + tuple(x.shape), dtype=x.dtype, device=x.device)
    check(lib().ss_euler_scale_dup(p(x), p(xin), x.numel(), float(sigma), dt(x), stream()), "ss_euler_scale_dup")
    return xin


def euler_cfg_step_(x, eps, guidance, sigma, sigma_next):
    _req(x); _req(eps)
    check(lib().ss_euler_cfg_step(p(x), p(eps), x.numel(), float(guidance), float(sigma), float(sigma_next), dt(x),
                                  stream()), "ss_euler_cfg_step")
    return x


def image_to_u8(x, pixels):
    _req(x)
    out = torch.empty(pixels, 3, dtype=torch.uint8, device=x.device)
    check(lib().ss_image_to_u8(p(x), p(out), pixels, x.shape[-1], dt(x), stream()), "ss_image_to_u8")
    return out
```

Measured before the change: 2.325.

## Fuse GroupNorm statistics into conv/GEMM epilogues and skip-concat writes in UNet

Conv3x3 and GEMM epilogues now emit per-column partial sums into a colpart buffer, so the following GroupNorm only finalizes and applies instead of rereading the activation for statistics. Up-block outputs are written directly into the left half of the concat buffer via a leading dimension. A concat_skip kernel copies the skip half while accumulating its channel statistics for the next GroupNorm. This removes full-tensor reads and separate concat copies in the UNet, at the cost of more code paths, dependence on specific GEMM configs and HW%128 constraints, and fallbacks when those do not hold.

```diff
diff --git a/include/seedstory_hip.h b/include/seedstory_hip.h
--- a/include/seedstory_hip.h
+++ b/include/seedstory_hip.h
@@ -243,10 +243,29 @@
 int ss_conv3x3(const void* x, const void* w, void* y, int64_t batch, int64_t H, int64_t W, int64_t Cin,
                int64_t Cout, int64_t stride, int64_t upsample2x, const void* bias, const void* rowvec,
                int64_t rowvec_stride, const void* residual, int dtype, void* stream);
+int ss_conv3x3_ld(const void* x, const void* w, void* y, int64_t ldy, int64_t batch, int64_t H, int64_t W, int64_t Cin,
+                  int64_t Cout, int64_t stride, int64_t upsample2x, const void* bias, const void* rowvec,
+                  int64_t rowvec_stride, const void* residual, int dtype, void* stream);
 
 size_t ss_groupnorm_workspace_bytes(int64_t batch, int64_t hw, int64_t channels, int64_t groups, int dtype);
 int ss_groupnorm(const void* x, const void* gamma, const void* beta, void* y, void* stats_ws, int64_t batch,
                  int64_t hw, int64_t channels, int64_t groups, float eps, int fuse_silu, int dtype, void* stream);
+
+int ss_conv3x3_colpart(const void* x, const void* w, void* y, int64_t ldy, int64_t batch, int64_t H, int64_t W, int64_t Cin,
+                       int64_t Cout, const void* bias, const void* rowvec, int64_t rowvec_stride, const void* residual,
+                       void* colpart, int force, int dtype, void* stream);
+int ss_gemm_colpart(const void* A, const void* W, void* C, int64_t M, int64_t N, int64_t K, int64_t ldc, const void* bias,
+                    const void* residual, int64_t ldr, int64_t hw, void* colpart, int force, int dtype, void* stream);
+int ss_groupnorm_colpart(const void* x, const void* gamma, const void* beta, void* y, void* stats_ws, const void* colpart,
+                         int64_t batch, int64_t hw, int64_t channels, int64_t groups, float eps, int fuse_silu, int dtype,
+                         void* stream);
+
+size_t ss_concat_skip_part_bytes(int64_t batch, int64_t hw, int64_t c1, int64_t c2, int dtype);
+int ss_concat_skip(const void* skip, void* out, void* chpart, int64_t batch, int64_t hw, int64_t c1, int64_t c2, int dtype,
+                   void* stream);
+int ss_groupnorm_cat(const void* x, const void* gamma, const void* beta, void* y, void* stats_ws, const void* chpart,
+                     int64_t batch, int64_t hw, int64_t channels, int64_t c1, int64_t groups, float eps, int fuse_silu, int dtype,
+                     void* stream);
 
 size_t ss_loss_workspace_bytes(int64_t n);
 int ss_cross_entropy_rows(const void* logits, int64_t ld, const int64_t* labels, int64_t rows, int64_t vocab,
diff --git a/seed-story_amd/csrc/ss_diffusion.hip b/seed-story_amd/csrc/ss_diffusion.hip
--- a/seed-story_amd/csrc/ss_diffusion.hip
+++ b/seed-story_amd/csrc/ss_diffusion.hip
@@ -115,6 +115,85 @@
             stats[((int64_t)b * G + g) * 2 + 1] = a2;
         }
         __syncthreads();
+    }
+}
+
+template <typename T, bool COPY>
+__global__ __launch_bounds__(256) void groupnorm_stats_cols_kernel(T* __restrict__ x, const T* __restrict__ skip,
+                                                                   float* __restrict__ chpart, double* __restrict__ part,
+                                                                   int HW, int C, int C1, int G, int rows_per_block) {
+    constexpr int V = Tr<T>::kVec;
+    extern __shared__ __attribute__((aligned(16))) char smem_raw[];
+    float* red = reinterpret_cast<float*>(smem_raw);
+    float* chs = red + 256 * 2 * V;
+    const int b = blockIdx.y;
+    const int cg = C / G, ppr = C / V, p1 = C1 / V, C2 = C - C1;
+    const int r0 = blockIdx.x * rows_per_block;
+    const int r1 = min(HW, r0 + rows_per_block);
+    T* xb = x + ((int64_t)b * HW) * C;
+    const T* sb = COPY ? skip + ((int64_t)b * HW) * C2 : nullptr;
+    float* cp = chpart + (((int64_t)b * gridDim.x + blockIdx.x) * C2) * 2;
+    for (int pc = 0; pc < ppr; pc += 256) {
+        const int cw = min(256, ppr - pc);
+        if (COPY ? pc + cw <= p1 : pc >= p1) continue;
+        const int rip = 256 / cw;
+        const int ry = threadIdx.x / cw, p = pc + threadIdx.x % cw;
+        const bool active = ry < rip && (COPY ? p >= p1 : p < p1);
+        float s1[V], s2[V];
+#pragma unroll
+        for (int j = 0; j < V; ++j) { s1[j] = 0.f; s2[j] = 0.f; }
+        if (active) {
+            const T* src = COPY ? sb + (int64_t)(p - p1) * V : xb + (int64_t)p * V;
+            const int64_t ld = COPY ? C2 : C;
+            T* dst = xb + (int64_t)p * V;
+            int r = r0 + ry;
+            for (; r + 3 * rip < r1; r += 4 * rip) {
+                uint4 u[4];
+#pragma unroll
+                for (int q = 0; q < 4; ++q) u[q] = ld16(src + (int64_t)(r + q * rip) * ld);
+#pragma unroll
+                for (int q = 0; q < 4; ++q) {
+                    float f[V];
+                    if constexpr (COPY) st16(dst + (int64_t)(r + q * rip) * C, u[q]);
+                    unpack<T>(u[q], f);
+#pragma unroll
+                    for (int j = 0; j < V; ++j) { s1[j] += f[j]; s2[j] = fmaf(f[j], f[j], s2[j]); }
+                }
+            }
+            for (; r < r1; r += rip) {
+                float f[V];
+                const uint4 u0 = ld16(src + (int64_t)r * ld);
+                if constexpr (COPY) st16(dst + (int64_t)r * C, u0);
+                unpack<T>(u0, f);
+#pragma unroll
+                for (int j = 0; j < V; ++j) { s1[j] += f[j]; s2[j] = fmaf(f[j], f[j], s2[j]); }
+            }
+#pragma unroll
+            for (int j = 0; j < V; ++j) { red[threadIdx.x * 2 * V + 2 * j] = s1[j]; red[threadIdx.x * 2 * V + 2 * j + 1] = s2[j]; }
+        }
+        __syncthreads();
+        if (active && ry == 0) {
+            for (int k = 1; k < rip; ++k) {
+                const float* o = red + (k * cw + (int)threadIdx.x) * 2 * V;
+#pragma unroll
+                for (int j = 0; j < V; ++j) { s1[j] += o[2 * j]; s2[j] += o[2 * j + 1]; }
+            }
+            float* o = COPY ? cp + (int64_t)(p - p1) * V * 2 : chs + (int64_t)p * V * 2;
+#pragma unroll
+            for (int j = 0; j < V; ++j) { o[2 * j] = s1[j]; o[2 * j + 1] = s2[j]; }
+        }
+        __syncthreads();
+    }
+    if constexpr (!COPY) {
+        for (int i = threadIdx.x; i < 2 * C2; i += 256) chs[2 * C1 + i] = cp[i];
+        __syncthreads();
+        double* out = part + (((int64_t)b * gridDim.x + blockIdx.x) * G) * 2;
+        for (int g = threadIdx.x; g < G; g += 256) {
+            double a1 = 0.0, a2 = 0.0;
+            for (int c = g * cg; c < (g + 1) * cg; ++c) { a1 += (double)chs[2 * c]; a2 += (double)chs[2 * c + 1]; }
+            out[2 * g] = a1;
+            out[2 * g + 1] = a2;
+        }
     }
 }
 
@@ -216,6 +295,107 @@
     return SS_OK;
 }
 
+__global__ __launch_bounds__(256) void groupnorm_colpart_finalize_kernel(const float* __restrict__ colpart, double* __restrict__ stats,
+                                                                         int nslot, int C, int G) {
+    __shared__ double sl[256 * 2];
+    const int g = blockIdx.x, b = blockIdx.y;
+    const int cg = C / G;
+    const int ns = 256 / cg;
+    const int ch = (int)threadIdx.x % cg, sidx = (int)threadIdx.x / cg;
+    double a1 = 0.0, a2 = 0.0;
+    if (sidx < ns) {
+        const int per = (nslot + ns - 1) / ns;
+        const int k0 = sidx * per, k1 = min(nslot, k0 + per);
+        const float2* pp = reinterpret_cast<const float2*>(colpart) + ((int64_t)b * nslot) * C + g * cg + ch;
+        for (int kb = k0; kb < k1; kb += 8) {
+            float2 t[8];
+#pragma unroll
+            for (int k = 0; k < 8; ++k) t[k] = (kb + k < k1) ? pp[(int64_t)(kb + k) * C] : make_float2(0.f, 0.f);
+#pragma unroll
+            for (int k = 0; k < 8; ++k) { a1 += (double)t[k].x; a2 += (double)t[k].y; }
+        }
+    }
+    sl[threadIdx.x * 2] = a1;
+    sl[threadIdx.x * 2 + 1] = a2;
+    __syncthreads();
+    if ((int)threadIdx.x < cg) {
+        for (int k = 1; k < ns; ++k) { a1 += sl[(k * cg + ch) * 2]; a2 += sl[(k * cg + ch) * 2 + 1]; }
+    }
+    __syncthreads();
+    if ((int)threadIdx.x < cg) { sl[ch * 2] = a1; sl[ch * 2 + 1] = a2; }
+    __syncthreads();
+    if (threadIdx.x == 0) {
+        double s1 = 0.0, s2 = 0.0;
+        for (int c = 0; c < cg; ++c) { s1 += sl[c * 2]; s2 += sl[c * 2 + 1]; }
+        stats[((int64_t)b * G + g) * 2] = s1;
+        stats[((int64_t)b * G + g) * 2 + 1] = s2;
+    }
+}
+
+template <typename T>
+int groupnorm_colpart_launch(const void* x, const void* gamma, const void* beta, void* y, double* ws, const float* colpart,
+                             int64_t B, int64_t HW, int64_t C, int64_t G, float eps, int silu, hipStream_t s) {
+    constexpr int V = Tr<T>::kVec;
+    SS_REQUIRE(C % G == 0 && C % V == 0 && C / G <= 256, "groupnorm_colpart: C=%lld G=%lld unsupported", (long long)C, (long long)G);
+    SS_REQUIRE(colpart && HW % 128 == 0, "groupnorm_colpart: partials missing or HW=%lld %% 128 != 0", (long long)HW);
+    if (B * HW == 0) return SS_OK;
+    const int rows_per_block = groupnorm_rows_per_block(B, HW, C, sizeof(T));
+    double* stats = ws;
+    hipLaunchKernelGGL(groupnorm_colpart_finalize_kernel, dim3((unsigned)G, (unsigned)B), dim3(256), 0, s, colpart, stats,
+                       (int)(HW / 128), (int)C, (int)G);
+    SS_LAUNCH_CHECK("groupnorm_colpart_finalize");
+    hipLaunchKernelGGL(groupnorm_apply_kernel<T>, dim3((unsigned)cdiv(HW, rows_per_block), (unsigned)B), dim3(256), 0, s, (const T*)x,
+                       stats, (const T*)gamma, (const T*)beta, (T*)y, (int)HW, (int)C, (int)G, eps, silu, rows_per_block);
+    SS_LAUNCH_CHECK("groupnorm_apply");
+    return SS_OK;
+}
+
+size_t concat_skip_part_bytes(int64_t B, int64_t HW, int64_t C1, int64_t C2, int dtype) {
+    if (B * HW == 0) return 0;
+    const int rpb = groupnorm_rows_per_block(B, HW, C1 + C2, dtype_size(dtype));
+    return (size_t)B * cdiv(HW, rpb) * C2 * 2 * sizeof(float);
+}
+
+template <typename T>
+int concat_skip_launch(const void* skip, void* x, float* chpart, int64_t B, int64_t HW, int64_t C1, int64_t C2, hipStream_t s) {
+    constexpr int V = Tr<T>::kVec;
+    SS_REQUIRE(C1 % V == 0 && C2 % V == 0 && C1 > 0 && C2 > 0, "concat_skip: channels %% %d != 0", V);
+    SS_REQUIRE(chpart, "concat_skip: chpart == NULL");
+    if (B * HW == 0) return SS_OK;
+    const int64_t C = C1 + C2;
+    const int rows_per_block = groupnorm_rows_per_block(B, HW, C, sizeof(T));
+    dim3 grid((unsigned)cdiv(HW, rows_per_block), (unsigned)B);
+    hipLaunchKernelGGL((groupnorm_stats_cols_kernel<T, true>), grid, dim3(256), (size_t)256 * 2 * V * sizeof(float), s, (T*)x,
+                       (const T*)skip, chpart, (double*)nullptr, (int)HW, (int)C, (int)C1, 1, rows_per_block);
+    SS_LAUNCH_CHECK("concat_skip");
+    return SS_OK;
+}
+
+template <typename T>
+int groupnorm_cat_launch(const void* x, const void* gamma, const void* beta, void* y, double* ws, const float* chpart, int64_t B,
+                         int64_t HW, int64_t C, int64_t C1, int64_t G, float eps, int silu, hipStream_t s) {
+    constexpr int V = Tr<T>::kVec;
+    SS_REQUIRE(C % G == 0 && C % V == 0 && C1 % V == 0 && C1 > 0 && C1 < C, "groupnorm_cat: C=%lld C1=%lld G=%lld unsupported",
+               (long long)C, (long long)C1, (long long)G);
+    SS_REQUIRE(chpart, "groupnorm_cat: chpart == NULL");
+    if (B * HW == 0) return SS_OK;
+    const int rows_per_block = groupnorm_rows_per_block(B, HW, C, sizeof(T));
+    dim3 grid((unsigned)cdiv(HW, rows_per_block), (unsigned)B);
+    double* stats = ws;
+    double* part = ws + (size_t)B * G * 2;
+    const size_t lds = (size_t)256 * 2 * V * sizeof(float) + (size_t)C * 2 * sizeof(float);
+    SS_REQUIRE(lds <= 64 * 1024, "groupnorm_cat: C=%lld too wide", (long long)C);
+    hipLaunchKernelGGL((groupnorm_stats_cols_kernel<T, false>), grid, dim3(256), lds, s, (T*)const_cast<void*>(x), (const T*)nullptr,
+                       const_cast<float*>(chpart), part, (int)HW, (int)C, (int)C1, (int)G, rows_per_block);
+    SS_LAUNCH_CHECK("groupnorm_stats_cols");
+    hipLaunchKernelGGL(groupnorm_finalize_kernel, dim3((unsigned)B), dim3(256), 0, s, (const double*)part, stats, (int)grid.x, (int)G);
+    SS_LAUNCH_CHECK("groupnorm_finalize");
+    hipLaunchKernelGGL(groupnorm_apply_kernel<T>, grid, dim3(256), 0, s, (const T*)x, stats, (const T*)gamma,
+                       (const T*)beta, (T*)y, (int)HW, (int)C, (int)G, eps, silu, rows_per_block);
+    SS_LAUNCH_CHECK("groupnorm_apply");
+    return SS_OK;
+}
+
 template <typename T>
 __global__ __launch_bounds__(256) void geglu_kernel(const T* __restrict__ in, T* __restrict__ out, int64_t rows, int D) {
     constexpr int V = Tr<T>::kVec;
@@ -446,6 +626,25 @@
                  int64_t channels, int64_t groups, float eps, int fuse_silu, int dtype, void* stream) {
     return SS_DISPATCH(dtype, groupnorm_launch, x, gamma, beta, y, (double*)stats_ws, batch, hw, channels, groups, eps,
                        fuse_silu, (hipStream_t)stream);
+}
+int ss_groupnorm_colpart(const void* x, const void* gamma, const void* beta, void* y, void* stats_ws, const void* colpart,
+                         int64_t batch, int64_t hw, int64_t channels, int64_t groups, float eps, int fuse_silu, int dtype,
+                         void* stream) {
+    return SS_DISPATCH(dtype, groupnorm_colpart_launch, x, gamma, beta, y, (double*)stats_ws, (const float*)colpart, batch, hw,
+                       channels, groups, eps, fuse_silu, (hipStream_t)stream);
+}
+size_t ss_concat_skip_part_bytes(int64_t batch, int64_t hw, int64_t c1, int64_t c2, int dtype) {
+    return ss::concat_skip_part_bytes(batch, hw, c1, c2, dtype);
+}
+int ss_concat_skip(const void* skip, void* out, void* chpart, int64_t batch, int64_t hw, int64_t c1, int64_t c2, int dtype,
+                   void* stream) {
+    return SS_DISPATCH(dtype, concat_skip_launch, skip, out, (float*)chpart, batch, hw, c1, c2, (hipStream_t)stream);
+}
+int ss_groupnorm_cat(const void* x, const void* gamma, const void* beta, void* y, void* stats_ws, const void* chpart,
+                     int64_t batch, int64_t hw, int64_t channels, int64_t c1, int64_t groups, float eps, int fuse_silu, int dtype,
+                     void* stream) {
+    return SS_DISPATCH(dtype, groupnorm_cat_launch, x, gamma, beta, y, (double*)stats_ws, (const float*)chpart, batch, hw,
+                       channels, c1, groups, eps, fuse_silu, (hipStream_t)stream);
 }
 int ss_geglu(const void* in, void* out, int64_t rows, int64_t d, int dtype, void* stream) {
     return SS_DISPATCH(dtype, geglu_launch, in, out, rows, d, (hipStream_t)stream);
diff --git a/seed-story_amd/csrc/ss_gemm.hip b/seed-story_amd/csrc/ss_gemm.hip
--- a/seed-story_amd/csrc/ss_gemm.hip
+++ b/seed-story_amd/csrc/ss_gemm.hip
@@ -693,17 +693,66 @@
 template <typename T>
 int conv3x3_launch(const void* x, const void* w, void* y, int64_t B, int64_t H, int64_t Wd, int64_t Cin, int64_t Cout,
                    int64_t stride, int64_t up, const void* bias, const void* rowvec, int64_t rowvec_ld,
-                   const void* residual, int epi, hipStream_t s) {
+                   const void* residual, int epi, hipStream_t s, int64_t ldc = 0) {
     constexpr int V = Tr<T>::kVec;
     SS_REQUIRE(Cin % V == 0, "conv3x3: Cin=%lld must be a multiple of %d (pad the channels)", (long long)Cin, V);
+    SS_REQUIRE(ldc == 0 || ldc >= Cout, "conv3x3: ldc=%lld < Cout=%lld", (long long)ldc, (long long)Cout);
     SS_REQUIRE((stride == 1 || stride == 2) && !(up && stride != 1), "conv3x3: unsupported stride/upsample");
     GemmArgs g;
     conv_geometry(g, B, H, Wd, Cin, Cout, stride, up);
     g.A = x; g.W = w; g.C = y; g.bias = bias; g.residual = residual; g.epi = epi;
     g.rowvec = rowvec; g.rowvec_ld = rowvec_ld > 0 ? rowvec_ld : Cout;
+    if (ldc > 0) g.ldc = ldc;
     g.swz = knob(K_gemm_xcd_swizzle);
     if (g.M == 0) return SS_OK;
     return gemm_dispatch_cfg<T>(lookup_cfg<T>(g), g, s);
+}
+
+template <typename T>
+int colpart_launch(GemmArgs g, int64_t hw, float* colpart, int force, hipStream_t s) {
+    if constexpr (Tr<T>::kVec != 8) {
+        return 1;
+    } else {
+        constexpr size_t A16 = 15;
+        if (!colpart || hw <= 0 || hw % 128 != 0 || g.M % hw != 0 || g.M % 128 != 0) return 1;
+        if ((((size_t)g.C | (size_t)g.residual | (size_t)g.bias | (size_t)g.rowvec | (size_t)colpart) & A16) != 0 ||
+            ((g.ldc | g.ldr | g.rowvec_ld) & 7) != 0)
+            return 1;
+        int cfg = lookup_cfg<T>(g);
+        if (cfg == 55) cfg = 54;
+        if (cfg != 54 && cfg != 56 && cfg != 57 && cfg != 58) {
+            if (!force) return 1;
+            cfg = (g.N % 320 == 0 && g.M % 256 == 0) ? 56 : 54;
+        }
+        g.rowpart = colpart;
+        return g.conv_Cin > 0 ? gemm_ppc_dispatch_conv<T>(cfg, g, s) : gemm_ppc_dispatch<T>(cfg, g, s);
+    }
+}
+
+template <typename T>
+int conv3x3_colpart_launch(const void* x, const void* w, void* y, int64_t ldy, int64_t B, int64_t H, int64_t Wd, int64_t Cin,
+                           int64_t Cout, const void* bias, const void* rowvec, int64_t rowvec_ld, const void* residual,
+                           float* colpart, int force, hipStream_t s) {
+    if (Cin % Tr<T>::kVec != 0 || (ldy != 0 && ldy < Cout)) return 1;
+    GemmArgs g;
+    conv_geometry(g, B, H, Wd, Cin, Cout, 1, 0);
+    g.A = x; g.W = w; g.C = y; g.bias = bias; g.residual = residual;
+    g.epi = (bias ? SS_EPI_BIAS : 0) | (residual ? SS_EPI_RESIDUAL : 0);
+    g.rowvec = rowvec; g.rowvec_ld = rowvec_ld > 0 ? rowvec_ld : Cout;
+    if (ldy > 0) g.ldc = ldy;
+    g.swz = knob(K_gemm_xcd_swizzle);
+    if (g.M == 0) return 1;
+    return colpart_launch<T>(g, H * Wd, colpart, force, s);
+}
+
+template <typename T>
+int gemm_colpart_launch(const void* A, const void* W, void* C, int64_t M, int64_t N, int64_t K, int64_t ldc, const void* bias,
+                        const void* residual, int64_t ldr, int64_t hw, float* colpart, int force, hipStream_t s) {
+    if (M == 0 || N == 0 || K % 64 != 0) return 1;
+    GemmArgs g = gemm_args(A, W, C, M, N, K, K, K, ldc, (bias ? SS_EPI_BIAS : 0) | (residual ? SS_EPI_RESIDUAL : 0), bias, residual, ldr);
+    g.swz = knob(K_gemm_xcd_swizzle);
+    if (knob(K_gemm_epi_generic)) return 1;
+    return colpart_launch<T>(g, hw, colpart, force, s);
 }
 
 template <typename T>
@@ -910,6 +959,27 @@
                        rowvec_stride, residual, epi, (hipStream_t)stream);
 }
 
+int ss_conv3x3_colpart(const void* x, const void* w, void* y, int64_t ldy, int64_t batch, int64_t H, int64_t W_, int64_t Cin,
+                       int64_t Cout, const void* bias, const void* rowvec, int64_t rowvec_stride, const void* residual,
+                       void* colpart, int force, int dtype, void* stream) {
+    return SS_DISPATCH(dtype, ss::conv3x3_colpart_launch, x, w, y, ldy, batch, H, W_, Cin, Cout, bias, rowvec, rowvec_stride,
+                       residual, (float*)colpart, force, (hipStream_t)stream);
+}
+
+int ss_gemm_colpart(const void* A, const void* W, void* C, int64_t M, int64_t N, int64_t K, int64_t ldc, const void* bias,
+                    const void* residual, int64_t ldr, int64_t hw, void* colpart, int force, int dtype, void* stream) {
+    return SS_DISPATCH(dtype, ss::gemm_colpart_launch, A, W, C, M, N, K, ldc, bias, residual, ldr, hw, (float*)colpart, force,
+                       (hipStream_t)stream);
+}
+
+int ss_conv3x3_ld(const void* x, const void* w, void* y, int64_t ldy, int64_t batch, int64_t H, int64_t W_, int64_t Cin,
+                  int64_t Cout, int64_t stride, int64_t upsample2x, const void* bias, const void* rowvec,
+                  int64_t rowvec_stride, const void* residual, int dtype, void* stream) {
+    const int epi = (bias ? SS_EPI_BIAS : 0) | (residual ? SS_EPI_RESIDUAL : 0);
+    return SS_DISPATCH(dtype, ss::conv3x3_launch, x, w, y, batch, H, W_, Cin, Cout, stride, upsample2x, bias, rowvec,
+                       rowvec_stride, residual, epi, (hipStream_t)stream, ldy);
+}
+
 int ss_gemm(const void* A, const void* W, void* C, int64_t M, int64_t N, int64_t K, int64_t lda,
             int64_t ldw, int64_t ldc, const void* bias, const void* residual, int64_t ldr, int epilogue,
             int dtype, void* stream) {
diff --git a/seed-story_amd/csrc/ss_gemm_common.h b/seed-story_amd/csrc/ss_gemm_common.h
--- a/seed-story_amd/csrc/ss_gemm_common.h
+++ b/seed-story_amd/csrc/ss_gemm_common.h
@@ -489,11 +489,12 @@
     if constexpr (std::is_same<T, bf16_t>::value) { lo = __uint_as_float(w << 16); hi = __uint_as_float(w & 0xffff0000u); }
     else { lo = f16_bits_to_f32(w & 0xffffu); hi = f16_bits_to_f32(w >> 16); }
 }
-template <typename T, int FM, int FN, int EV, bool RES, bool WHOLE>
+template <typename T, int FM, int FN, int EV, bool RES, bool WHOLE, bool COLP = false>
 __device__ __forceinline__ void gemm_epilogue_staged_pipe(const GemmArgs& g, f32x4_t (&acc)[FN][FM], int m_base, int n_base,
-                                                          int lane, char* stg) {
+                                                          int lane, char* stg, char* fin = nullptr) {
     static_assert(Tr<T>::kVec == 8, "16-bit outputs only");
     static_assert(EV >= 1 && EV <= 4, "compile-time variants only");
+    static_assert(!COLP || EV == 1 || EV == 3, "column partials: plain / rowvec epilogues");
     constexpr int TN = FN * 16, RS = TN * 2 + 16;
     constexpr bool GEGLU = EV == 4;
     constexpr int LPR = GEGLU ? TN / 16 : TN / 8;
@@ -596,6 +597,8 @@
             else rr[c][k] = row_ok(c, k) ? gmem_ld16(Rc + roff[k]) : make_uint4(0u, 0u, 0u, 0u);
         }
     };
+    float cs[2] = {0.f, 0.f};
+    double cq[2] = {0.0, 0.0};
     load_rv(0);
     if (has_res) {
 #pragma unroll
@@ -624,9 +627,32 @@
                 o = pack<T>(a);
             }
             if (row_ok(c, k)) gmem_st16(Cc + goff[k], o);
+            if constexpr (COLP) {
+                if (pv[k]) *reinterpret_cast<uint4*>(fin + loff[k]) = o;
+            }
+        }
+        if constexpr (COLP) {
+            asm volatile("" ::: "memory");
+            if (lane < TN / 2) {
+                const char* cp = fin + lane * 4;
+#pragma unroll
+                for (int r = 0; r < 16; ++r) {
+                    float a, b;
+                    unpack2<T>(*reinterpret_cast<const uint32_t*>(cp + r * RS), a, b);
+                    const double da = (double)a, db = (double)b;
+                    cs[0] += a; cq[0] = fma(da, da, cq[0]);
+                    cs[1] += b; cq[1] = fma(db, db, cq[1]);
+                }
+            }
+            asm volatile("" ::: "memory");
         }
         __builtin_amdgcn_sched_barrier(0);
         if (c + 1 < FM) readback();
+    }
+    if constexpr (COLP) {
+        if (lane < TN / 2 && m_base < M)
+            *reinterpret_cast<float4*>(g.rowpart + ((int64_t)(m_base >> 7) * g.N + n_base + 2 * lane) * 2) =
+                make_float4(cs[0], (float)cq[0], cs[1], (float)cq[1]);
     }
 }
 
@@ -708,6 +734,8 @@
 template <typename T> int gemm_sp_dispatch_conv(int cfg, const GemmArgs& g, hipStream_t s);
 template <typename T> int gemm_pp_dispatch(int cfg, const GemmArgs& g, hipStream_t s);
 template <typename T> int gemm_pp_dispatch_conv(int cfg, const GemmArgs& g, hipStream_t s);
+template <typename T> int gemm_ppc_dispatch(int cfg, const GemmArgs& g, hipStream_t s);
+template <typename T> int gemm_ppc_dispatch_conv(int cfg, const GemmArgs& g, hipStream_t s);
 template <typename T> int gemm_w4_dispatch(int cfg, const GemmArgs& g, hipStream_t s);
 template <typename T> int gemm_w4_dispatch_conv(int cfg, const GemmArgs& g, hipStream_t s);
 int gemm_sp_dispatch_fp8(int cfg, const GemmArgs& g, hipStream_t s);
diff --git a/seed-story_amd/csrc/ss_gemm_pp.inc b/seed-story_amd/csrc/ss_gemm_pp.inc
--- a/seed-story_amd/csrc/ss_gemm_pp.inc
+++ b/seed-story_amd/csrc/ss_gemm_pp.inc
@@ -1,3 +1,7 @@
+
+#ifndef SS_PP_COLPART
+#define SS_PP_COLPART 0
+#endif
 
 namespace ss {
 
@@ -31,6 +35,8 @@
     constexpr bool EXACT = BN == 320 || CONV;
     constexpr bool PRIO = (FLAGS & 1) != 0, PERSIST = (FLAGS & 2) != 0, TWO = (FLAGS & 4) != 0, STAGED = (FLAGS & 8) != 0, RSTAT = (FLAGS & 32) != 0;
     constexpr int EM = ((FLAGS & 16) != 0) ? 2 : 0;
+    constexpr bool COLP = (FLAGS & 64) != 0;
+    static_assert(!COLP || (STAGED && !PERSIST && (FLAGS & 48) == 0), "column partials: staged, non-persistent, plain epilogue");
     constexpr int HA = Lds::HA, HB0 = Lds::HB0, HB1 = Lds::HB1, BUF = Lds::BUF;
     constexpr int OFF_A0 = 0, OFF_A1 = HA, OFF_B0 = 2 * HA, OFF_B1 = 2 * HA + HB0;
     constexpr int NP0 = FN0, NP1 = FN1;
@@ -353,6 +359,14 @@
                 const int mb = m_cur + wm * TM, nb = n_cur + wn * TN;
                 const bool o_gelu = (g.epi & SS_EPI_GELU) != 0, o_geglu = (g.epi & SS_EPI_GEGLU_PAIR) != 0;
                 const bool o_rv = g.rowvec != nullptr || (!CONV && (g.epi & SS_EPI_INTERNAL_GENERIC) != 0);
+                if constexpr (COLP) {
+                    char* fin = smem_raw + (STG_IN_RING ? 8 * STG_WAVE : 0) + wid * STG_WAVE;
+                    static_assert((STG_IN_RING ? 16 : 8) * STG_WAVE <= BUF, "second strips fit ring buffer 0");
+                    const bool o_res = (g.epi & SS_EPI_RESIDUAL) != 0;
+                    if (!o_rv && !o_res) gemm_epilogue_staged_pipe<TO, FM, FN, 1, false, EXACT, true>(g, acc, mb, nb, lane, strip, fin);
+                    else if (!o_rv) gemm_epilogue_staged_pipe<TO, FM, FN, 1, true, EXACT, true>(g, acc, mb, nb, lane, strip, fin);
+                    else if constexpr (CONV) gemm_epilogue_staged_pipe<TO, FM, FN, 3, false, EXACT, true>(g, acc, mb, nb, lane, strip, fin);
+                } else
                 if constexpr (EM == 0 && !RSTAT) {
                     const bool o_res = (g.epi & SS_EPI_RESIDUAL) != 0;
                     if (!o_gelu && !o_geglu && !o_rv && !o_res) gemm_epilogue_staged_pipe<TO, FM, FN, 1, false, EXACT>(g, acc, mb, nb, lane, strip);
@@ -393,11 +407,39 @@
         if (BN == 320 && (g.M % 256 != 0 || g.N % 320 != 0)) ok = false;
     }
     if (!ok) return 1;
-    if ((g.rowstat_out || g.rowpart) && !(FLAGS & 32)) return 1;
+    if ((g.rowstat_out || g.rowpart) && !(FLAGS & (32 | 64))) return 1;
+    if (FLAGS & 64) {
+        const bool rv = g.rowvec != nullptr;
+        if (!g.rowpart || g.rowstat_out || g.N % BN != 0 || g.M % 128 != 0 || (g.epi & ~(SS_EPI_BIAS | SS_EPI_RESIDUAL)) ||
+            (rv && (!conv || (g.epi & SS_EPI_RESIDUAL) || (g.rows_per_batch & 15))))
+            return 1;
+    }
     return launch_tiles<gemm_pp_kernel<T, BN, FLAGS, CONV>>("gemm_pp", g, cdiv(g.M, 256) * cdiv(g.N, BN), (FLAGS & 2) ? num_cus() : 0, 512,
                                                             PpLds<BN, FLAGS>::BYTES, s);
 }
 
+#if SS_PP_COLPART
+#if SS_PP_CONV
+template <typename T> int gemm_ppc_dispatch_conv(int cfg, const GemmArgs& g, hipStream_t s) {
+#else
+template <typename T> int gemm_ppc_dispatch(int cfg, const GemmArgs& g, hipStream_t s) {
+#endif
+    switch (cfg) {
+        case 54: return pp_launch<T, 256, 8 | 64>(g, s);
+        case 56: return pp_launch<T, 320, 8 | 64>(g, s);
+        case 57: return pp_launch<T, 256, 12 | 64>(g, s);
+#if !SS_PP_CONV
+        case 58: return pp_launch<T, 320, 12 | 64>(g, s);
+#endif
+        default: return 1;
+    }
+}
+#if SS_PP_CONV
+template int gemm_ppc_dispatch_conv<SS_PP_T>(int, const GemmArgs&, hipStream_t);
+#else
+template int gemm_ppc_dispatch<SS_PP_T>(int, const GemmArgs&, hipStream_t);
+#endif
+#else
 #if SS_PP_CONV
 template <typename T> int gemm_pp_dispatch_conv(int cfg, const GemmArgs& g, hipStream_t s) {
 #else
@@ -419,5 +461,6 @@
 #else
 template int gemm_pp_dispatch<SS_PP_T>(int, const GemmArgs&, hipStream_t);
 #endif
-
-}
+#endif
+
+}
diff --git a/seed-story_amd/csrc/ss_gemm_ppc_bf16.hip b/seed-story_amd/csrc/ss_gemm_ppc_bf16.hip
--- /dev/null
+++ b/seed-story_amd/csrc/ss_gemm_ppc_bf16.hip
@@ -0,0 +1,5 @@
+#include "ss_gemm_common.h"
+#define SS_PP_T ::ss::bf16_t
+#define SS_PP_CONV 0
+#define SS_PP_COLPART 1
+#include "ss_gemm_pp.inc"
diff --git a/seed-story_amd/csrc/ss_gemm_ppc_bf16_conv.hip b/seed-story_amd/csrc/ss_gemm_ppc_bf16_conv.hip
--- /dev/null
+++ b/seed-story_amd/csrc/ss_gemm_ppc_bf16_conv.hip
@@ -0,0 +1,5 @@
+#include "ss_gemm_common.h"
+#define SS_PP_T ::ss::bf16_t
+#define SS_PP_CONV 1
+#define SS_PP_COLPART 1
+#include "ss_gemm_pp.inc"
diff --git a/seed-story_amd/csrc/ss_gemm_ppc_f16.hip b/seed-story_amd/csrc/ss_gemm_ppc_f16.hip
--- /dev/null
+++ b/seed-story_amd/csrc/ss_gemm_ppc_f16.hip
@@ -0,0 +1,5 @@
+#include "ss_gemm_common.h"
+#define SS_PP_T ::ss::f16_t
+#define SS_PP_CONV 0
+#define SS_PP_COLPART 1
+#include "ss_gemm_pp.inc"
diff --git a/seed-story_amd/csrc/ss_gemm_ppc_f16_conv.hip b/seed-story_amd/csrc/ss_gemm_ppc_f16_conv.hip
--- /dev/null
+++ b/seed-story_amd/csrc/ss_gemm_ppc_f16_conv.hip
@@ -0,0 +1,5 @@
+#include "ss_gemm_common.h"
+#define SS_PP_T ::ss::f16_t
+#define SS_PP_CONV 1
+#define SS_PP_COLPART 1
+#include "ss_gemm_pp.inc"
diff --git a/seed-story_amd/seedstory/_lib.py b/seed-story_amd/seedstory/_lib.py
--- a/seed-story_amd/seedstory/_lib.py
+++ b/seed-story_amd/seedstory/_lib.py
@@ -123,6 +123,7 @@
     "ss_vit_forward": (C.c_int, [C.POINTER(VitWeights), vp, vp, i64, vp, sz, C.c_int, vp]),
     "ss_vit_blocks": (C.c_int, [C.POINTER(VitWeights), vp, i64, i64, i64, i64, vp, sz, C.c_int, vp]),
     "ss_conv3x3": (C.c_int, [vp, vp, vp, i64, i64, i64, i64, i64, i64, i64, vp, vp, i64, vp, C.c_int, vp]),
+    "ss_conv3x3_ld": (C.c_int, [vp, vp, vp, i64, i64, i64, i64, i64, i64, i64, i64, vp, vp, i64, vp, C.c_int, vp]),
     "ss_loss_workspace_bytes": (C.c_size_t, [i64]),
     "ss_cross_entropy_rows": (C.c_int, [vp, i64, vp, i64, i64, i64, vp, vp, C.c_int, vp]),
     "ss_cosine_rows": (C.c_int, [vp, vp, i64, i64, vp, C.c_int, vp]),
@@ -130,6 +131,12 @@
     "ss_mse": (C.c_int, [vp, vp, i64, vp, vp, C.c_int, vp]),
     "ss_groupnorm_workspace_bytes": (C.c_size_t, [i64, i64, i64, i64, C.c_int]),
     "ss_groupnorm": (C.c_int, [vp, vp, vp, vp, vp, i64, i64, i64, i64, f32, C.c_int, C.c_int, vp]),
+    "ss_conv3x3_colpart": (C.c_int, [vp, vp, vp, i64, i64, i64, i64, i64, i64, vp, vp, i64, vp, vp, C.c_int, C.c_int, vp]),
+    "ss_gemm_colpart": (C.c_int, [vp, vp, vp, i64, i64, i64, i64, vp, vp, i64, i64, vp, C.c_int, C.c_int, vp]),
+    "ss_groupnorm_colpart": (C.c_int, [vp, vp, vp, vp, vp, vp, i64, i64, i64, i64, f32, C.c_int, C.c_int, vp]),
+    "ss_concat_skip_part_bytes": (C.c_size_t, [i64, i64, i64, i64, C.c_int]),
+    "ss_concat_skip": (C.c_int, [vp, vp, vp, i64, i64, i64, i64, C.c_int, vp]),
+    "ss_groupnorm_cat": (C.c_int, [vp, vp, vp, vp, vp, vp, i64, i64, i64, i64, i64, f32, C.c_int, C.c_int, vp]),
     "ss_geglu": (C.c_int, [vp, vp, i64, i64, C.c_int, vp]),
     "ss_unary": (C.c_int, [vp, vp, i64, C.c_int, C.c_int, vp]),
     "ss_softmax_rows": (C.c_int, [vp, i64, i64, f32, C.c_int, vp]),
diff --git a/seed-story_amd/seedstory/diffusion.py b/seed-story_amd/seedstory/diffusion.py
--- a/seed-story_amd/seedstory/diffusion.py
+++ b/seed-story_amd/seedstory/diffusion.py
@@ -281,23 +281,45 @@
         return P
 
     def _resnet(self, P, n, x, B, H, W, temb_act, groups, eps=1e-5):
-        h = ops.groupnorm(x, P[n + ".norm1.weight"], P[n + ".norm1.bias"], B, groups, eps, silu=True)
+        return self._resnet_p(P, n, x, B, H, W, temb_act, groups, eps)[0]
+
+    def _resnet_p(self, P, n, x, B, H, W, temb_act, groups, eps=1e-5, cat=None, out_cat=None, x_part=None, want_part=False):
+        h = ops.groupnorm(x, P[n + ".norm1.weight"], P[n + ".norm1.bias"], B, groups, eps, silu=True, cat=cat, colpart=x_part)
         tp, tld = None, 0
         if temb_act is not None:
             off = P["temb_all.offsets"][n]
             tld = temb_act.shape[1]
             tp = temb_act[:, off:]
-        h, _, _ = ops.conv3x3(h, P[n + ".conv1.weight"], B, H, W, bias=P[n + ".conv1.bias"], rowvec=tp, rowvec_stride=tld)
-        h = ops.groupnorm(h, P[n + ".norm2.weight"], P[n + ".norm2.bias"], B, groups, eps, silu=True)
+        colp = getattr(self, "_gn_colpart", True)
+        if colp:
+            h, hp = ops.conv3x3_colpart(h, P[n + ".conv1.weight"], B, H, W, bias=P[n + ".conv1.bias"], rowvec=tp, rowvec_stride=tld)
+        else:
+            (h, _, _), hp = ops.conv3x3(h, P[n + ".conv1.weight"], B, H, W, bias=P[n + ".conv1.bias"], rowvec=tp, rowvec_stride=tld), None
+        h = ops.groupnorm(h, P[n + ".norm2.weight"], P[n + ".norm2.bias"], B, groups, eps, silu=True, colpart=hp)
         sc = x
         if (n + ".conv_shortcut.weight") in P:
             sc = ops.gemm(x, P[n + ".conv_shortcut.weight"], bias=P[n + ".conv_shortcut.bias"])
-        h, _, _ = ops.conv3x3(h, P[n + ".conv2.weight"], B, H, W, bias=P[n + ".conv2.bias"], residual=sc)
-        return h
+        if colp and want_part and out_cat is None:
+            return ops.conv3x3_colpart(h, P[n + ".conv2.weight"], B, H, W, bias=P[n + ".conv2.bias"], residual=sc)
+        h, _, _ = ops.conv3x3(h, P[n + ".conv2.weight"], B, H, W, bias=P[n + ".conv2.bias"], residual=sc, out=out_cat,
+                              out_left=out_cat is not None)
+        return h, None
 
     def enable_fp8(self, on=True):
         if bool(on) != getattr(self, "_fp8", False):
             self._fp8 = bool(on)
+            self._prep = None
+        return self
+
+    def enable_cat_inplace(self, on=True):
+        if bool(on) != getattr(self, "_cat_inplace", True):
+            self._cat_inplace = bool(on)
+            self._prep = None
+        return self
+
+    def enable_gn_colpart(self, on=True):
+        if bool(on) != getattr(self, "_gn_colpart", True):
+            self._gn_colpart = bool(on)
             self._prep = None
         return self
 
@@ -376,7 +398,10 @@
         return {"buf": b, "cur": None}
 
     def _transformer(self, P, n, x, B, HW, ctx2d, Lctx, heads, layers, groups):
-        h = ops.groupnorm(x, P[n + ".norm.weight"], P[n + ".norm.bias"], B, groups, 1e-6, silu=False)
+        return self._transformer_p(P, n, x, B, HW, ctx2d, Lctx, heads, layers, groups)[0]
+
+    def _transformer_p(self, P, n, x, B, HW, ctx2d, Lctx, heads, layers, groups, out_cat=None, x_part=None, want_part=False):
+        h = ops.groupnorm(x, P[n + ".norm.weight"], P[n + ".norm.bias"], B, groups, 1e-6, silu=False, colpart=x_part)
         rs = None
         if self._lnfold_on() and h.shape[0] > 128 and all(
                 (n + ".transformer_blocks.%d%s.lnf" % (k, w)) in P for k in range(layers)
@@ -407,7 +432,12 @@
                              bias=P[b + ".ff.net.0.proj.pairs.bias"], geglu=True, rowstat=rs)
             h = self._lin(P, b + ".ff.net.2.weight", u, bias=P[b + ".ff.net.2.bias"], residual=h,
                           rowstat=rs if k + 1 < layers else None)
-        return self._lin(P, n + ".proj_out.weight", h, bias=P[n + ".proj_out.bias"], residual=x)
+        f8 = getattr(self, "_fp8", False) and (n + ".proj_out.weight.fp8") in P
+        if out_cat is not None and not f8:
+            return ops.gemm(h, P[n + ".proj_out.weight"], bias=P[n + ".proj_out.bias"], residual=x, out=out_cat, out_left=True), None
+        if want_part and not f8 and getattr(self, "_gn_colpart", True):
+            return ops.gemm_colpart(h, P[n + ".proj_out.weight"], HW, bias=P[n + ".proj_out.bias"], residual=x)
+        return self._lin(P, n + ".proj_out.weight", h, bias=P[n + ".proj_out.bias"], residual=x), None
 
     @torch.no_grad()
     def forward(self, sample, timestep, encoder_hidden_states, added_cond_kwargs=None, return_dict=True, **kw):
@@ -444,34 +474,62 @@
         x = ops.nchw_to_nhwc(sample.contiguous(), 8)
         h, _, _ = ops.conv3x3(x, P["conv_in.weight"], B, H, W, bias=P["conv_in.bias"])
         skips = [(h, H, W)]
+        hp = None
         for i in range(len(boc)):
             for j in range(L):
-                h = self._resnet(P, "down_blocks.%d.resnets.%d" % (i, j), h, B, H, W, temb_act, G)
-                if c["transformer_layers"][i]:
-                    h = self._transformer(P, "down_blocks.%d.attentions.%d" % (i, j), h, B, H * W, ctx2d, Lctx,
-                                          c["num_heads"][i], c["transformer_layers"][i], G)
+                to_norm = not (j == L - 1 and i < len(boc) - 1)
+                has_tr = c["transformer_layers"][i]
+                h, hp = self._resnet_p(P, "down_blocks.%d.resnets.%d" % (i, j), h, B, H, W, temb_act, G, x_part=hp,
+                                     want_part=bool(has_tr) or to_norm)
+                if has_tr:
+                    h, hp = self._transformer_p(P, "down_blocks.%d.attentions.%d" % (i, j), h, B, H * W, ctx2d, Lctx,
+                                              c["num_heads"][i], has_tr, G, x_part=hp, want_part=to_norm)
                 skips.append((h, H, W))
             if i < len(boc) - 1:
                 n = "down_blocks.%d.downsamplers.0.conv" % i
                 h, H, W = ops.conv3x3(h, P[n + ".weight"], B, H, W, stride=2, bias=P[n + ".bias"])
+                hp = None
                 skips.append((h, H, W))
-        h = self._resnet(P, "mid_block.resnets.0", h, B, H, W, temb_act, G)
-        h = self._transformer(P, "mid_block.attentions.0", h, B, H * W, ctx2d, Lctx, c["num_heads"][-1],
-                              c["transformer_layers"][-1], G)
-        h = self._resnet(P, "mid_block.resnets.1", h, B, H, W, temb_act, G)
+        h, hp = self._resnet_p(P, "mid_block.resnets.0", h, B, H, W, temb_act, G, x_part=hp, want_part=True)
+        h, hp = self._transformer_p(P, "mid_block.attentions.0", h, B, H * W, ctx2d, Lctx, c["num_heads"][-1],
+                                  c["transformer_layers"][-1], G, x_part=hp, want_part=True)
+        def cat_for(cout):
+            if not getattr(self, "_cat_inplace", True):
+                return None
+            sk = skips[-1][0]
+            return torch.empty(sk.shape[0], cout + sk.shape[1], dtype=dt, device=dev)
+        n = "mid_block.resnets.1"
+        oc = cat_for(P[n + ".conv2.weight"].shape[0])
+        h, hp = self._resnet_p(P, n, h, B, H, W, temb_act, G, out_cat=oc, x_part=hp, want_part=oc is None)
+        hc1 = P[n + ".conv2.weight"].shape[0] if oc is not None else None
         for i in range(len(boc)):
             ri = len(boc) - 1 - i
             for j in range(L + 1):
                 sk, _, _ = skips.pop()
-                h = ops.concat_channels(h, sk)
-                h = self._resnet(P, "up_blocks.%d.resnets.%d" % (i, j), h, B, H, W, temb_act, G)
-                if c["transformer_layers"][ri]:
-                    h = self._transformer(P, "up_blocks.%d.attentions.%d" % (i, j), h, B, H * W, ctx2d, Lctx,
-                                          c["num_heads"][ri], c["transformer_layers"][ri], G)
+                if hc1 is not None:
+                    cat = (hc1, ops.concat_skip_(h, hc1, sk, B))
+                else:
+                    cat = None
+                    h = ops.concat_channels(h, sk)
+                hp = None
+                n = "up_blocks.%d.resnets.%d" % (i, j)
+                cout = P[n + ".conv2.weight"].shape[0]
+                has_tr, again = c["transformer_layers"][ri], j < L
+                oc = cat_for(cout) if again and not has_tr else None
+                to_norm = has_tr or (not again and i == len(boc) - 1)
+                h, hp = self._resnet_p(P, n, h, B, H, W, temb_act, G, cat=cat, out_cat=oc, want_part=bool(to_norm))
+                hc1 = cout if oc is not None else None
+                if has_tr:
+                    oc = cat_for(cout) if again else None
+                    h, hp = self._transformer_p(P, "up_blocks.%d.attentions.%d" % (i, j), h, B, H * W, ctx2d, Lctx,
+                                              c["num_heads"][ri], c["transformer_layers"][ri], G, out_cat=oc, x_part=hp,
+                                              want_part=not again and i == len(boc) - 1)
+                    hc1 = cout if oc is not None and h is oc else None
             if i < len(boc) - 1:
                 n = "up_blocks.%d.upsamplers.0.conv" % i
                 h, H, W = ops.conv3x3(h, P[n + ".weight"], B, H, W, upsample=True, bias=P[n + ".bias"])
-        h = ops.groupnorm(h, P["conv_norm_out.weight"], P["conv_norm_out.bias"], B, G, 1e-5, silu=True)
+                hp = None
+        h = ops.groupnorm(h, P["conv_norm_out.weight"], P["conv_norm_out.bias"], B, G, 1e-5, silu=True, colpart=hp)
         o, _, _ = ops.conv3x3(h, P["conv_out.weight"], B, H, W, bias=P["conv_out.bias"])
         out = ops.nhwc_to_nchw(o, B, c["out_channels"], H, W)
         return _Sample(out) if return_dict else (out,)
diff --git a/seed-story_amd/seedstory/ops.py b/seed-story_amd/seedstory/ops.py
--- a/seed-story_amd/seedstory/ops.py
+++ b/seed-story_amd/seedstory/ops.py
@@ -182,10 +182,26 @@
     return out
 
 
-def gemm(a, w, bias=None, residual=None, gelu=False, out=None, rowstat=None, rowpart=None):
+def _out_left(out, rows, n, like, name):
+    _req(out, name + "(out=)")
+    if out.dim() != 2 or out.shape[0] != rows or out.shape[1] < n or out.dtype != like.dtype or out.device != like.device:
+        raise _lib.SSError("%s(out=, out_left=True): expected [%d, >= %d] %s on %s, got %s %s on %s"
+                           % (name, rows, n, like.dtype, like.device, tuple(out.shape), out.dtype, out.device))
+    return out.shape[1]
+
+
+def gemm(a, w, bias=None, residual=None, gelu=False, out=None, rowstat=None, rowpart=None, out_left=False):
     _req(a); _req(w)
     M, K = a.shape
     N = w.shape[0]
+    if out_left:
+        assert rowstat is None and rowpart is None
+        ld = _out_left(out, M, N, a, "gemm")
+        epi = (EPI_BIAS if bias is not None else 0) | (EPI_GELU if gelu else 0) | (EPI_RESIDUAL if residual is not None else 0)
+        tune.ensure_gemm(M, N, K, dt(a), epi, a.device)
+        check(lib().ss_gemm(p(a), p(w), p(out), M, N, K, K, w.stride(0), ld, p(bias), p(residual), N, epi, dt(a), stream()),
+              "ss_gemm")
+        return out
     out = _out(out, (M, N), a, "gemm")
     epi = (EPI_BIAS if bias is not None else 0) | (EPI_GELU if gelu else 0) | (EPI_RESIDUAL if residual is not None else 0)
     tune.ensure_gemm(M, N, K, dt(a), epi, a.device)
@@ -335,12 +351,19 @@
     return tok
 
 
-def conv3x3(x, w, B, H, W, stride=1, upsample=False, bias=None, rowvec=None, residual=None, rowvec_stride=0, out=None):
+def conv3x3(x, w, B, H, W, stride=1, upsample=False, bias=None, rowvec=None, residual=None, rowvec_stride=0, out=None,
+            out_left=False):
     _req(x); _req(w)
     Cin = x.shape[-1]
     Cout = w.shape[0]
     Hin, Win = (2 * H, 2 * W) if upsample else (H, W)
     Ho, Wo = (Hin + 2 - 3) // stride + 1, (Win + 2 - 3) // stride + 1
+    if out_left:
+        ld = _out_left(out, B * Ho * Wo, Cout, x, "conv3x3")
+        tune.ensure_conv(B, H, W, Cin, Cout, stride, upsample, dt(x), x.device)
+        check(lib().ss_conv3x3_ld(p(x), p(w), p(out), ld, B, H, W, Cin, Cout, stride, int(upsample), p(bias), p(rowvec),
+                                  rowvec_stride, p(residual), dt(x), stream()), "ss_conv3x3_ld")
+        return out, Ho, Wo
     y = _out(out, (B * Ho * Wo, Cout), x, "conv3x3")
     tune.ensure_conv(B, H, W, Cin, Cout, stride, upsample, dt(x), x.device)
     check(lib().ss_conv3x3(p(x), p(w), p(y), B, H, W, Cin, Cout, stride, int(upsample), p(bias), p(rowvec),
@@ -348,15 +371,68 @@
     return y, Ho, Wo
 
 
-def groupnorm(x, gamma, beta, B, groups, eps, silu=False):
+def colpart_buffer(rows, n, device):
+    return torch.empty(rows // 128, n, 2, dtype=torch.float32, device=device)
+
+
+def conv3x3_colpart(x, w, B, H, W, bias=None, rowvec=None, residual=None, rowvec_stride=0, out=None, out_left=False, force=False,
+                    colpart=None):
+    _req(x); _req(w)
+    Cin, Cout, rows = x.shape[-1], w.shape[0], B * H * W
+    if x.dtype in (torch.bfloat16, torch.float16) and (H * W) % 128 == 0:
+        ld = _out_left(out, rows, Cout, x, "conv3x3_colpart") if out_left else Cout
+        y = out if out_left else _out(out, (rows, Cout), x, "conv3x3_colpart")
+        tune.ensure_conv(B, H, W, Cin, Cout, 1, False, dt(x), x.device)
+        part = colpart if colpart is not None else colpart_buffer(rows, Cout, x.device)
+        rc = lib().ss_conv3x3_colpart(p(x), p(w), p(y), ld, B, H, W, Cin, Cout, p(bias), p(rowvec), rowvec_stride, p(residual),
+                                      p(part), int(force), dt(x), stream())
+        if rc == 0:
+            return y, part
+        if rc != 1:
+            check(rc, "ss_conv3x3_colpart")
+    y, _, _ = conv3x3(x, w, B, H, W, bias=bias, rowvec=rowvec, residual=residual, rowvec_stride=rowvec_stride, out=out,
+                      out_left=out_left)
+    return y, None
+
+
+def gemm_colpart(a, w, hw, bias=None, residual=None, out=None, out_left=False, force=False, colpart=None):
+    _req(a); _req(w)
+    M, K = a.shape
+    N = w.shape[0]
+    if a.dtype in (torch.bfloat16, torch.float16) and hw % 128 == 0 and w.stride(0) == K:
+        ld = _out_left(out, M, N, a, "gemm_colpart") if out_left else N
+        y = out if out_left else _out(out, (M, N), a, "gemm_colpart")
+        epi = (EPI_BIAS if bias is not None else 0) | (EPI_RESIDUAL if residual is not None else 0)
+        tune.ensure_gemm(M, N, K, dt(a), epi, a.device)
+        part = colpart if colpart is not None else colpart_buffer(M, N, a.device)
+        rc = lib().ss_gemm_colpart(p(a), p(w), p(y), M, N, K, ld, p(bias), p(residual), N, hw, p(part), int(force), dt(a), stream())
+        if rc == 0:
+            return y, part
+        if rc != 1:
+            check(rc, "ss_gemm_colpart")
+    return gemm(a, w, bias=bias, residual=residual, out=out, out_left=out_left), None
+
+
+def groupnorm(x, gamma, beta, B, groups, eps, silu=False, cat=None, return_stats=False, colpart=None):
     _req(x)
     C = x.shape[-1]
     HW = x.shape[0] // B
     y = torch.empty_like(x)
     nb = int(lib().ss_groupnorm_workspace_bytes(B, HW, C, groups, dt(x)))
     ws = torch.empty(max(nb // 8, 1), dtype=torch.float64, device=x.device)
-    check(lib().ss_groupnorm(p(x), p(gamma), p(beta), p(y), p(ws), B, HW, C, groups, eps, int(silu), dt(x), stream()),
-          "ss_groupnorm")
+    if colpart is not None:
+        assert cat is None and colpart.dtype == torch.float32 and colpart.numel() == (x.shape[0] // 128) * C * 2
+        check(lib().ss_groupnorm_colpart(p(x), p(gamma), p(beta), p(y), p(ws), p(colpart), B, HW, C, groups, eps, int(silu),
+                                         dt(x), stream()), "ss_groupnorm_colpart")
+    elif cat is not None:
+        c1, chpart = cat
+        check(lib().ss_groupnorm_cat(p(x), p(gamma), p(beta), p(y), p(ws), p(chpart), B, HW, C, c1, groups, eps, int(silu),
+                                     dt(x), stream()), "ss_groupnorm_cat")
+    else:
+        check(lib().ss_groupnorm(p(x), p(gamma), p(beta), p(y), p(ws), B, HW, C, groups, eps, int(silu), dt(x), stream()),
+              "ss_groupnorm")
+    if return_stats:
+        return y, ws[:B * groups * 2].view(B, groups, 2)
     return y
 
 
@@ -467,6 +543,17 @@
     return out
 
 
+def concat_skip_(cat, c1, skip, B):
+    _req(cat); _req(skip)
+    rows, c2 = skip.shape
+    if cat.shape != (rows, c1 + c2) or cat.dtype != skip.dtype or rows % B:
+        raise _lib.SSError("concat_skip_: cat %s does not fit c1 = %d + skip %s" % (tuple(cat.shape), c1, tuple(skip.shape)))
+    nb = int(lib().ss_concat_skip_part_bytes(B, rows // B, c1, c2, dt(cat)))
+    chpart = torch.empty(max(nb // 4, 1), dtype=torch.float32, device=cat.device)
+    check(lib().ss_concat_skip(p(skip), p(cat), p(chpart), B, rows // B, c1, c2, dt(cat), stream()), "ss_concat_skip")
+    return chpart
+
+
 def nchw_to_nhwc(x, cpad):
     _req(x)
     B, Cc = x.shape[0], x.shape[1]
```

Result: no change. 2.338 (median of 6 runs) (+0.5%).
